# rubengooj/pl-svo

Measured on AMD Instinct MI355X. Metric: sparse-align+pose-opt frames/sec, 640×480, ~200 pts+80 lines; 1/2/4/8 GPU, higher is better.
Workload: dtype f64

## Files before the change

include/plsvo_hip.h:

```cpp
#ifndef PLSVO_HIP_H_
#define PLSVO_HIP_H_

#include <stddef.h>
#include <stdint.h>

#ifdef __cplusplus
extern "C" {
#endif

#define PLSVO_MAX_LEVELS 8
#define PLSVO_PATCH_SIZE 4
#define PLSVO_PATCH_AREA 16

#define PLSVO_OK              0
#define PLSVO_E_INVALID      -1
#define PLSVO_E_NODEVICE     -2
#define PLSVO_E_HIP          -3
#define PLSVO_E_CAPACITY     -4
#define PLSVO_E_STATE        -5
#define PLSVO_E_RCCL         -6

typedef struct plsvo_ctx plsvo_ctx;

typedef struct plsvo_pinhole {
  double fx, fy, cx, cy;
  int32_t width, height;
} plsvo_pinhole;


int plsvo_hip_create(int device_id, void* stream, plsvo_ctx** out);
int plsvo_hip_create_on_stream(int device_id, void* stream, plsvo_ctx** out);
void plsvo_hip_destroy(plsvo_ctx* ctx);
#define PLSVO_OPT_LDLT_FLAVOUR 1
#define PLSVO_OPT_ALIGN_THREADS 2
#define PLSVO_OPT_POSEOPT_THREADS 3
#define PLSVO_OPT_ALIGN_REORDER 4
#define PLSVO_OPT_POSEOPT_REORDER 5
int plsvo_hip_set_option(plsvo_ctx* ctx, int option, int value);
const char* plsvo_hip_last_error(const plsvo_ctx* ctx);
void* plsvo_hip_stream(plsvo_ctx* ctx);
int plsvo_hip_synchronize(plsvo_ctx* ctx);


int plsvo_hip_config_pyramids(plsvo_ctx* ctx, int n_slots, int width, int height, int n_levels);

int plsvo_hip_upload_pyramid(plsvo_ctx* ctx, int slot, int n_levels,
                             const uint8_t* const* level_ptr, const int* width, const int* height,
                             const int* stride_bytes);

int plsvo_hip_build_pyramid(plsvo_ctx* ctx, int slot, const uint8_t* level0, int stride_bytes,
                            int rounding);
int plsvo_hip_build_pyramids_dev(plsvo_ctx* ctx, int first_slot, int n, const void* d_level0,
                                 int stride_bytes, size_t image_pitch_bytes, int rounding);
int plsvo_hip_copy_slots(plsvo_ctx* ctx, int dst_first, int src_first, int n);
int plsvo_hip_download_level(plsvo_ctx* ctx, int slot, int level, uint8_t* out);


typedef struct plsvo_pinhole_radtan {
  plsvo_pinhole cam;
  double d[5];
} plsvo_pinhole_radtan;

#define PLSVO_MAX_RECTIFY_MAPS 8

int plsvo_rectify_map(const plsvo_pinhole_radtan* cam, int16_t* xy, uint16_t* frac);
int plsvo_hip_config_rectify(plsvo_ctx* ctx, const plsvo_pinhole_radtan* cam, int flip_vertical, int* map_id);
int plsvo_hip_rectify_build_pyramid(plsvo_ctx* ctx, int map_id, int slot, const uint8_t* raw, int stride_bytes, int rounding);
int plsvo_hip_rectify_build_pyramids_dev(plsvo_ctx* ctx, int map_id, int first_slot, int n, const void* d_raw,
                                         int stride_bytes, size_t image_pitch_bytes, int rounding);


typedef struct plsvo_corner { int32_t x, y; float score; int32_t level; } plsvo_corner;

typedef struct plsvo_detect_params {
  int32_t cell_size;
  int32_t n_levels;
  int32_t fast_threshold;
  int32_t reserved0;
  double  detection_threshold;
} plsvo_detect_params;

int plsvo_detect_grid(int width, int height, int cell_size, int* cols, int* rows);
int plsvo_detect_cell(int cols, int cell_size, double px_x, double px_y);
int plsvo_hip_detect_fast(plsvo_ctx* ctx, int first_slot, int n, const plsvo_detect_params* params, const uint8_t* occupancy,
                          plsvo_corner* corners, int32_t* counts);
int plsvo_hip_detect_fast_dev(plsvo_ctx* ctx, int first_slot, int n, const plsvo_detect_params* params, const uint8_t* d_occupancy,
                              plsvo_corner* d_corners, int32_t* d_counts);
int plsvo_hip_detect_stages(plsvo_ctx* ctx, int slot, int level, int fast_threshold, uint8_t* score, uint8_t* survives);


typedef struct plsvo_align_in {
  int32_t ref_slot, cur_slot;
  plsvo_pinhole cam;
  int32_t max_level, min_level;
  int32_t n_iter;
  int32_t reserved0;
  double eps;
  double T_cur_from_ref[7];
  int32_t n_pts, n_seg;
  const double* pt_px;
  const double* pt_xyz_ref;
  const double* seg_spx;
  const double* seg_epx;
  const double* seg_len;
  const double* seg_p_ref;
  const double* seg_q_ref;
  const uint8_t* seg_alive_in;
} plsvo_align_in;

typedef struct plsvo_align_out {
  double T_cur_from_ref[7];
  uint64_t n_meas;
  uint64_t n_tracked;
  double H[36];
  double chi2;
  uint8_t* seg_alive_out;
  int32_t iters_per_level[PLSVO_MAX_LEVELS];
  int32_t status;
  int32_t reserved0;
} plsvo_align_out;

typedef struct plsvo_align_iterlog {
  int32_t level, iter;
  int32_t accepted;
  int32_t stop;
  uint64_t n_meas;
  double new_chi2;
  double H[36], Jres[6], x[6];
  double T_after[7];
} plsvo_align_iterlog;

int plsvo_sparse_align(plsvo_ctx* ctx, const plsvo_align_in* in, plsvo_align_out* out);
int plsvo_sparse_align_batch(plsvo_ctx* ctx, int n, const plsvo_align_in* in, plsvo_align_out* out);

int plsvo_align_stage(plsvo_ctx* ctx, int n, const plsvo_align_in* in);
int plsvo_align_run(plsvo_ctx* ctx);
int plsvo_align_fetch(plsvo_ctx* ctx, int n, plsvo_align_out* out);

int plsvo_align_slot_layout(const plsvo_align_in* in, int level, int32_t* seg_code, int32_t* n_slots, int32_t* long_lines,
                            long long* n_patches);

int plsvo_align_set_trace(plsvo_ctx* ctx, int max_records_per_job);
int plsvo_align_fetch_trace(plsvo_ctx* ctx, int job, plsvo_align_iterlog* out, int max_records,
                            int* n_records);

const double* plsvo_align_poses_dev(plsvo_ctx* ctx);
int plsvo_align_copy_poses(plsvo_ctx* ctx, double* d_dst);

int plsvo_align_work(plsvo_ctx* ctx, uint64_t* patch_levels, uint64_t* patch_iters);
int plsvo_align_launch_order(plsvo_ctx* ctx, int n, int32_t* order);
int plsvo_align_work_points(plsvo_ctx* ctx, uint64_t* point_patch_iters);

int plsvo_align_chi2_ties(plsvo_ctx* ctx, uint64_t* iterations, uint64_t* ties, uint64_t* near_ties_without_terms);


typedef struct plsvo_poseopt_in {
  double T_f_w[7];
  double fx;
  double reproj_thresh;
  int32_t n_iter;
  int32_t n_iter_ref;
  int32_t n_pts, n_seg;
  const double* pt_f;
  const double* pt_pos;
  const int32_t* pt_level;
  const double* seg_line;
  const double* seg_spos;
  const double* seg_epos;
  const int32_t* seg_level;
} plsvo_poseopt_in;

typedef struct plsvo_poseopt_out {
  double T_f_w[7];
  double cov[36];
  double estimated_scale, error_init, error_final;
  uint64_t num_obs_pt, num_obs_ls;
  uint8_t* pt_keep;
  uint8_t* seg_keep;
  int32_t iters;
  int32_t iters_ref;
  int32_t status;
  int32_t reserved0;
} plsvo_poseopt_out;

typedef struct plsvo_poseopt_iterlog {
  int32_t phase;
  int32_t iter;
  int32_t accepted;
  int32_t reserved0;
  double new_chi2;
  double A[36], b[6], dT[6];
  double T_after[7];
} plsvo_poseopt_iterlog;

int plsvo_pose_optimize(plsvo_ctx* ctx, const plsvo_poseopt_in* in, plsvo_poseopt_out* out);
int plsvo_pose_optimize_batch(plsvo_ctx* ctx, int n, const plsvo_poseopt_in* in, plsvo_poseopt_out* out);
int plsvo_poseopt_stage(plsvo_ctx* ctx, int n, const plsvo_poseopt_in* in);
int plsvo_poseopt_run(plsvo_ctx* ctx);
int plsvo_poseopt_fetch(plsvo_ctx* ctx, int n, plsvo_poseopt_out* out);
int plsvo_poseopt_set_trace(plsvo_ctx* ctx, int max_records_per_job);
int plsvo_poseopt_fetch_trace(plsvo_ctx* ctx, int job, plsvo_poseopt_iterlog* out, int max_records,
                              int* n_records);
const double* plsvo_poseopt_poses_dev(plsvo_ctx* ctx);
int plsvo_poseopt_copy_poses(plsvo_ctx* ctx, double* d_dst);
int plsvo_poseopt_work(plsvo_ctx* ctx, uint64_t* pt_iters, uint64_t* seg_iters);


typedef struct plsvo_structopt_in {
  int32_t n_frames;
  int32_t n_iter_pts;
  int32_t n_iter_segs;
  int32_t n_pts, n_seg;
  int32_t reserved0;
  const double* frame_T;
  const double* pt_pos;
  const int32_t* pt_obs_off;
  const int32_t* pt_obs_frame;
  const double* pt_obs_f;
  const double* seg_spos;
  const double* seg_epos;
  const int32_t* seg_obs_off;
  const int32_t* seg_obs_frame;
  const double* seg_obs_sf;
  const double* seg_obs_ef;
} plsvo_structopt_in;

typedef struct plsvo_structopt_out {
  double* pt_pos;
  double* seg_spos;
  double* seg_epos;
  int32_t* pt_iters;
  int32_t* seg_iters;
} plsvo_structopt_out;

int plsvo_structure_optimize(plsvo_ctx* ctx, const plsvo_structopt_in* in, plsvo_structopt_out* out);


#define PLSVO_FTR_CORNER  0
#define PLSVO_FTR_EDGELET 1

typedef struct plsvo_match_in {
  plsvo_pinhole cam;
  int32_t n_pyr_levels;
  int32_t align_max_iter;
  int32_t n_frames;
  int32_t n;
  const double* frame_T;
  const int32_t* frame_slot;
  const int32_t* cur_frame;
  const int32_t* ref_frame;
  const double* ref_px;
  const double* ref_f;
  const int32_t* ref_level;
  const uint8_t* ref_type;
  const double* ref_grad;
  const double* pos;
  const double* px_cur;
} plsvo_match_in;

typedef struct plsvo_match_out {
  double* px_cur;
  uint8_t* found;
  int32_t* search_level;
  int32_t* n_iter;
} plsvo_match_out;

int plsvo_match_direct(plsvo_ctx* ctx, const plsvo_match_in* in, plsvo_match_out* out);

typedef struct plsvo_reproject_in {
  plsvo_pinhole cam;
  int32_t n_frames;
  int32_t n;
  int32_t cell_size;
  int32_t grid_n_cols;
  int32_t boundary;
  int32_t reserved0;
  const double* frame_T;
  const int32_t* frame;
  const double* pos;
} plsvo_reproject_in;

typedef struct plsvo_reproject_out {
  double* px;
  int32_t* cell;
} plsvo_reproject_out;

int plsvo_reproject(plsvo_ctx* ctx, const plsvo_reproject_in* in, plsvo_reproject_out* out);


typedef struct plsvo_chain_in {
  plsvo_align_in align;
  double T_prev_w[7];
  double T_kf_w[7];
  int32_t kf_slot;
  int32_t n_cand_pt, n_cand_seg;
  int32_t reserved0;
  const double* pos;
  const double* ref_px;
  const double* ref_f;
  const int32_t* ref_level;
  const uint8_t* ref_type;
  const double* ref_grad;
  const uint8_t* active;
// ... 134 lines not shown
```

pl-svo_amd/capi.py:

```python
import ctypes as C
import os
import sys

import numpy as np

from . import abi

_HERE = os.path.dirname(os.path.abspath(__file__))
LIB_PATH = os.environ.get("PLSVO_HIP_LIB", os.path.join(_HERE, "libplsvo_hip.so"))

SYMBOLS = [
    "plsvo_hip_create", "plsvo_hip_create_on_stream", "plsvo_hip_set_option", "plsvo_align_slot_layout", "plsvo_hip_destroy", "plsvo_hip_last_error", "plsvo_hip_stream", "plsvo_hip_synchronize",
    "plsvo_hip_config_pyramids", "plsvo_hip_upload_pyramid", "plsvo_hip_build_pyramid", "plsvo_hip_build_pyramids_dev",
    "plsvo_hip_download_level", "plsvo_hip_copy_slots",
    "plsvo_rectify_map", "plsvo_hip_config_rectify", "plsvo_hip_rectify_build_pyramid", "plsvo_hip_rectify_build_pyramids_dev",
    "plsvo_detect_grid", "plsvo_detect_cell", "plsvo_hip_detect_fast", "plsvo_hip_detect_fast_dev", "plsvo_hip_detect_stages",
    "plsvo_sparse_align", "plsvo_sparse_align_batch", "plsvo_align_stage", "plsvo_align_run", "plsvo_align_fetch",
    "plsvo_align_set_trace", "plsvo_align_fetch_trace", "plsvo_align_poses_dev", "plsvo_align_copy_poses", "plsvo_align_work", "plsvo_align_work_points", "plsvo_align_chi2_ties", "plsvo_align_launch_order",
    "plsvo_pose_optimize", "plsvo_pose_optimize_batch", "plsvo_poseopt_stage", "plsvo_poseopt_run", "plsvo_poseopt_fetch",
    "plsvo_poseopt_set_trace", "plsvo_poseopt_fetch_trace", "plsvo_poseopt_poses_dev", "plsvo_poseopt_copy_poses", "plsvo_poseopt_work",
    "plsvo_structure_optimize", "plsvo_match_direct", "plsvo_reproject", "plsvo_trajectory_record", "plsvo_update_seeds",
    "plsvo_chain_stage", "plsvo_chain_run", "plsvo_chain_fetch", "plsvo_frame_step_batch", "plsvo_chain_poses_dev",
    "plsvo_pack_pose_records", "plsvo_fetch_pose_records", "plsvo_gather_poses",
    "plsvo_hip_set_profiling", "plsvo_hip_kernel_time", "plsvo_hip_reset_profiling",
    "plsvo_hip_version", "plsvo_hip_build_flags", "plsvo_hip_device_info",
]


def rectify_map(cam):
    w, h = cam.cam.width, cam.cam.height
    xy = np.zeros((max(h, 0), max(w, 0), 2), dtype=np.int16)
    fr = np.zeros((max(h, 0), max(w, 0)), dtype=np.uint16)
    rc = lib().plsvo_rectify_map(C.byref(cam), xy.ctypes.data_as(C.POINTER(C.c_int16)), fr.ctypes.data_as(C.POINTER(C.c_uint16)))
    if rc != 0:
        raise PlsvoError(rc, "rectify_map: bad camera (non-finite or zero focal length, size outside 1..2046)")
    return xy, fr


def detect_grid(width, height, cell_size):
    cols, rows = C.c_int(0), C.c_int(0)
    rc = lib().plsvo_detect_grid(int(width), int(height), int(cell_size), C.byref(cols), C.byref(rows))
    if rc != 0:
        raise PlsvoError(rc, "detect_grid: width, height and cell_size must be >= 1")
    return cols.value, rows.value


def detect_cell(cols, cell_size, px_x, px_y):
    k = lib().plsvo_detect_cell(int(cols), int(cell_size), float(px_x), float(px_y))
    if k < 0:
        raise PlsvoError(k, "detect_cell: cols and cell_size must be >= 1, the pixel finite and not negative")
    return k


class PlsvoError(RuntimeError):
    def __init__(self, code, msg):
        super().__init__(f"plsvo_hip error {code}: {msg}")
        self.code = code


_lib = None


def lib():
    global _lib
    if _lib is not None:
        return _lib
    if not os.path.exists(LIB_PATH):
        raise ImportError(f"{LIB_PATH} not found: build it with `make -C pl-svo_amd/csrc` "
                          f"(or __graft_entry__.build()); plsvo_hip has no CPU fallback")
    L = C.CDLL(LIB_PATH)
    if hasattr(L, "plsvo_emu_build"):
        sys.stderr.write(f"pl-svo_amd: {LIB_PATH} is a HOST EMULATION build of the kernels (test infrastructure), not the gfx950 library\n")
    ctxp = C.c_void_p
    vp = C.c_void_p
    sig = {
        "plsvo_hip_create": (C.c_int, [C.c_int, vp, C.POINTER(ctxp)]),
        "plsvo_hip_create_on_stream": (C.c_int, [C.c_int, vp, C.POINTER(ctxp)]),
        "plsvo_hip_destroy": (None, [ctxp]),
        "plsvo_hip_set_option": (C.c_int, [ctxp, C.c_int, C.c_int]),
        "plsvo_hip_last_error": (C.c_char_p, [ctxp]),
        "plsvo_hip_stream": (vp, [ctxp]),
        "plsvo_hip_synchronize": (C.c_int, [ctxp]),
        "plsvo_hip_config_pyramids": (C.c_int, [ctxp, C.c_int, C.c_int, C.c_int, C.c_int]),
        "plsvo_hip_upload_pyramid": (C.c_int, [ctxp, C.c_int, C.c_int, C.POINTER(abi.c_u8_p), abi.c_i32_p, abi.c_i32_p, abi.c_i32_p]),
        "plsvo_hip_build_pyramid": (C.c_int, [ctxp, C.c_int, abi.c_u8_p, C.c_int, C.c_int]),
        "plsvo_hip_build_pyramids_dev": (C.c_int, [ctxp, C.c_int, C.c_int, vp, C.c_int, C.c_size_t, C.c_int]),
        "plsvo_hip_download_level": (C.c_int, [ctxp, C.c_int, C.c_int, abi.c_u8_p]),
        "plsvo_hip_copy_slots": (C.c_int, [ctxp, C.c_int, C.c_int, C.c_int]),
        "plsvo_rectify_map": (C.c_int, [C.POINTER(abi.PinholeRadtan), C.POINTER(C.c_int16), C.POINTER(C.c_uint16)]),
        "plsvo_hip_config_rectify": (C.c_int, [ctxp, C.POINTER(abi.PinholeRadtan), C.c_int, C.POINTER(C.c_int)]),
        "plsvo_hip_rectify_build_pyramid": (C.c_int, [ctxp, C.c_int, C.c_int, abi.c_u8_p, C.c_int, C.c_int]),
        "plsvo_hip_rectify_build_pyramids_dev": (C.c_int, [ctxp, C.c_int, C.c_int, C.c_int, vp, C.c_int, C.c_size_t, C.c_int]),
        "plsvo_detect_grid": (C.c_int, [C.c_int, C.c_int, C.c_int, C.POINTER(C.c_int), C.POINTER(C.c_int)]),
        "plsvo_detect_cell": (C.c_int, [C.c_int, C.c_int, C.c_double, C.c_double]),
        "plsvo_hip_detect_fast": (C.c_int, [ctxp, C.c_int, C.c_int, C.POINTER(abi.DetectParams), abi.c_u8_p, C.POINTER(abi.Corner), abi.c_i32_p]),
        "plsvo_hip_detect_fast_dev": (C.c_int, [ctxp, C.c_int, C.c_int, C.POINTER(abi.DetectParams), vp, vp, vp]),
        "plsvo_hip_detect_stages": (C.c_int, [ctxp, C.c_int, C.c_int, C.c_int, abi.c_u8_p, abi.c_u8_p]),
        "plsvo_sparse_align": (C.c_int, [ctxp, C.POINTER(abi.AlignIn), C.POINTER(abi.AlignOut)]),
        "plsvo_sparse_align_batch": (C.c_int, [ctxp, C.c_int, C.POINTER(abi.AlignIn), C.POINTER(abi.AlignOut)]),
        "plsvo_align_stage": (C.c_int, [ctxp, C.c_int, C.POINTER(abi.AlignIn)]),
        "plsvo_align_run": (C.c_int, [ctxp]),
        "plsvo_align_fetch": (C.c_int, [ctxp, C.c_int, C.POINTER(abi.AlignOut)]),
        "plsvo_align_set_trace": (C.c_int, [ctxp, C.c_int]),
        "plsvo_align_fetch_trace": (C.c_int, [ctxp, C.c_int, C.POINTER(abi.AlignIterLog), C.c_int, C.POINTER(C.c_int)]),
        "plsvo_align_poses_dev": (vp, [ctxp]),
        "plsvo_align_copy_poses": (C.c_int, [ctxp, vp]),
        "plsvo_poseopt_copy_poses": (C.c_int, [ctxp, vp]),
        "plsvo_align_work": (C.c_int, [ctxp, C.POINTER(C.c_uint64), C.POINTER(C.c_uint64)]),
        "plsvo_align_chi2_ties": (C.c_int, [ctxp, C.POINTER(C.c_uint64), C.POINTER(C.c_uint64), C.POINTER(C.c_uint64)]),
        "plsvo_align_work_points": (C.c_int, [ctxp, C.POINTER(C.c_uint64)]),
        "plsvo_align_launch_order": (C.c_int, [ctxp, C.c_int, C.POINTER(C.c_int32)]),
        "plsvo_pose_optimize": (C.c_int, [ctxp, C.POINTER(abi.PoseOptIn), C.POINTER(abi.PoseOptOut)]),
        "plsvo_pose_optimize_batch": (C.c_int, [ctxp, C.c_int, C.POINTER(abi.PoseOptIn), C.POINTER(abi.PoseOptOut)]),
        "plsvo_poseopt_stage": (C.c_int, [ctxp, C.c_int, C.POINTER(abi.PoseOptIn)]),
        "plsvo_poseopt_run": (C.c_int, [ctxp]),
        "plsvo_poseopt_fetch": (C.c_int, [ctxp, C.c_int, C.POINTER(abi.PoseOptOut)]),
        "plsvo_poseopt_set_trace": (C.c_int, [ctxp, C.c_int]),
        "plsvo_poseopt_fetch_trace": (C.c_int, [ctxp, C.c_int, C.POINTER(abi.PoseOptIterLog), C.c_int, C.POINTER(C.c_int)]),
        "plsvo_poseopt_poses_dev": (vp, [ctxp]),
        "plsvo_poseopt_work": (C.c_int, [ctxp, C.POINTER(C.c_uint64), C.POINTER(C.c_uint64)]),
        "plsvo_structure_optimize": (C.c_int, [ctxp, C.POINTER(abi.StructOptIn), C.POINTER(abi.StructOptOut)]),
        "plsvo_match_direct": (C.c_int, [ctxp, C.POINTER(abi.MatchIn), C.POINTER(abi.MatchOut)]),
        "plsvo_reproject": (C.c_int, [ctxp, C.POINTER(abi.ReprojectIn), C.POINTER(abi.ReprojectOut)]),
        "plsvo_update_seeds": (C.c_int, [ctxp, C.POINTER(abi.SeedsIn), C.POINTER(abi.SeedsOut)]),
        "plsvo_trajectory_record": (C.c_int, [abi.c_double_p, abi.c_double_p, abi.c_double_p]),
        "plsvo_chain_stage": (C.c_int, [ctxp, C.c_int, C.POINTER(abi.ChainIn), C.POINTER(abi.ChainParams)]),
        "plsvo_chain_run": (C.c_int, [ctxp]),
        "plsvo_chain_fetch": (C.c_int, [ctxp, C.c_int, C.POINTER(abi.ChainOut)]),
        "plsvo_frame_step_batch": (C.c_int, [ctxp, C.c_int, C.POINTER(abi.ChainIn), C.POINTER(abi.ChainParams), C.POINTER(abi.ChainOut)]),
        "plsvo_chain_poses_dev": (vp, [ctxp]),
        "plsvo_align_slot_layout": (C.c_int, [C.POINTER(abi.AlignIn), C.c_int, C.POINTER(C.c_int32), C.POINTER(C.c_int32), C.POINTER(C.c_int32),
                                              C.POINTER(C.c_longlong)]),
        "plsvo_pack_pose_records": (C.c_int, [ctxp, vp, C.POINTER(C.c_int)]),
        "plsvo_fetch_pose_records": (C.c_int, [ctxp, C.c_int, C.POINTER(abi.PoseRecord)]),
        "plsvo_gather_poses": (C.c_int, [ctxp, vp, vp, C.c_int, vp]),
        "plsvo_hip_set_profiling": (C.c_int, [ctxp, C.c_int]),
        "plsvo_hip_kernel_time": (C.c_int, [ctxp, C.c_int, C.POINTER(C.c_double), C.POINTER(C.c_int64)]),
        "plsvo_hip_reset_profiling": (C.c_int, [ctxp]),
        "plsvo_hip_version": (C.c_char_p, []),
        "plsvo_hip_build_flags": (C.c_char_p, []),
        "plsvo_hip_device_info": (C.c_int, [ctxp, C.c_char_p, C.c_int, C.POINTER(C.c_int), C.POINTER(C.c_size_t)]),
    }
    for name, (res, args) in sig.items():
        if "PLSVO_HIP_LIB" in os.environ and not hasattr(L, name):
            continue
        f = getattr(L, name)
        f.restype = res
        f.argtypes = args
    _lib = L
    return L


class Context:

    def __init__(self, device=0, stream=None):
        self.L = lib()
        h = C.c_void_p()
        if stream is None:
            rc = self.L.plsvo_hip_create(int(device), None, C.byref(h))
        else:
            rc = self.L.plsvo_hip_create_on_stream(int(device), C.c_void_p(int(stream)), C.byref(h))
        if rc != 0:
            raise PlsvoError(rc, (self.L.plsvo_hip_last_error(None) or b"").decode())
        self.h = h
        self._keep = None

    def set_ldlt_flavour(self, flavour):
        self._chk(self.L.plsvo_hip_set_option(self.h, 1, int(flavour)))

    def set_launch_shapes(self, align_threads=None, poseopt_threads=None):
        if align_threads is not None:
            self._chk(self.L.plsvo_hip_set_option(self.h, 2, int(align_threads)))
        if poseopt_threads is not None:
            self._chk(self.L.plsvo_hip_set_option(self.h, 3, int(poseopt_threads)))

    def set_launch_order_refresh(self, align=None, poseopt=None):
        if align is not None:
            self._chk(self.L.plsvo_hip_set_option(self.h, 4, 1 if align else 0))
        if poseopt is not None:
            self._chk(self.L.plsvo_hip_set_option(self.h, 5, 1 if poseopt else 0))

    def close(self):
        if getattr(self, "h", None):
            self.L.plsvo_hip_destroy(self.h)
            self.h = None

    def __del__(self):
        try:
            self.close()
        except Exception:
            pass

    def _chk(self, rc):
        if rc != 0:
            raise PlsvoError(rc, (self.L.plsvo_hip_last_error(self.h) or b"").decode())

    def device_info(self):
        name = C.create_string_buffer(256)
        cu = C.c_int(0)
        mem = C.c_size_t(0)
        self._chk(self.L.plsvo_hip_device_info(self.h, name, 256, C.byref(cu), C.byref(mem)))
        return name.value.decode(), cu.value, mem.value

    def stream(self):
        return self.L.plsvo_hip_stream(self.h)

    def synchronize(self):
        self._chk(self.L.plsvo_hip_synchronize(self.h))

    def set_profiling(self, on):
        self._chk(self.L.plsvo_hip_set_profiling(self.h, 1 if on else 0))

    def reset_profiling(self):
        self._chk(self.L.plsvo_hip_reset_profiling(self.h))

    def kernel_time(self, k):
        ms = C.c_double(0)
        n = C.c_int64(0)
        self._chk(self.L.plsvo_hip_kernel_time(self.h, k, C.byref(ms), C.byref(n)))
        return ms.value, n.value

    def config_pyramids(self, n_slots, width, height, n_levels):
        self._chk(self.L.plsvo_hip_config_pyramids(self.h, n_slots, width, height, n_levels))
        self.n_levels = n_levels
        self.width, self.height = width, height

    def upload_pyramid(self, slot, levels):
        keep = [np.ascontiguousarray(l, dtype=np.uint8) for l in levels]
        n = len(keep)
        ptrs = (abi.c_u8_p * n)(*[l.ctypes.data_as(abi.c_u8_p) for l in keep])
        w = (C.c_int32 * n)(*[l.shape[1] for l in keep])
        h = (C.c_int32 * n)(*[l.shape[0] for l in keep])
        s = (C.c_int32 * n)(*[l.strides[0] for l in keep])
        self._chk(self.L.plsvo_hip_upload_pyramid(self.h, slot, n, ptrs, w, h, s))

    def build_pyramid(self, slot, img0, rounding=0):
        img0 = np.ascontiguousarray(img0, dtype=np.uint8)
        self._chk(self.L.plsvo_hip_build_pyramid(self.h, slot, img0.ctypes.data_as(abi.c_u8_p), img0.strides[0], rounding))

    def build_pyramids_dev(self, first_slot, n, d_ptr, stride_bytes, image_pitch_bytes, rounding=0):
        self._chk(self.L.plsvo_hip_build_pyramids_dev(self.h, first_slot, n, C.c_void_p(d_ptr), stride_bytes,
                                                      image_pitch_bytes, rounding))

    def download_level(self, slot, level):
        w, h = self.width >> level, self.height >> level
        out = np.empty((h, w), dtype=np.uint8)
        self._chk(self.L.plsvo_hip_download_level(self.h, slot, level, out.ctypes.data_as(abi.c_u8_p)))
        return out

    def copy_slots(self, dst_first, src_first, n):
        self._chk(self.L.plsvo_hip_copy_slots(self.h, int(dst_first), int(src_first), int(n)))

    def download_pyramid(self, slot):
        return [self.download_level(slot, l) for l in range(self.n_levels)]

    def config_rectify(self, cam, flip_vertical=False):
        mid = C.c_int(-1)
        self._chk(self.L.plsvo_hip_config_rectify(self.h, C.byref(cam), 1 if flip_vertical else 0, C.byref(mid)))
        return mid.value

    def rectify_build_pyramid(self, map_id, slot, raw, rounding=0):
        raw = np.asarray(raw, dtype=np.uint8)
        if raw.ndim != 2 or raw.strides[1] != 1:
            raw = np.ascontiguousarray(raw)
        self._chk(self.L.plsvo_hip_rectify_build_pyramid(self.h, int(map_id), int(slot), raw.ctypes.data_as(abi.c_u8_p), raw.strides[0],
                                                         int(rounding)))

    def rectify_build_pyramids_dev(self, map_id, first_slot, n, d_ptr, stride_bytes, image_pitch_bytes, rounding=0):
        self._chk(self.L.plsvo_hip_rectify_build_pyramids_dev(self.h, int(map_id), int(first_slot), int(n), C.c_void_p(d_ptr),
                                                              int(stride_bytes), int(image_pitch_bytes), int(rounding)))

    def detect_fast(self, first_slot, n, cell_size=25, n_levels=3, fast_threshold=20, detection_threshold=20.0, occupancy=None):
        cols, rows = detect_grid(self.width, self.height, cell_size)
        cells = cols * rows
        pr = abi.detect_params(cell_size, n_levels, fast_threshold, detection_threshold)
        occ = None
        if occupancy is not None:
            occ = np.ascontiguousarray(np.asarray(occupancy).reshape(int(n), cells) != 0, dtype=np.uint8)
        out = np.zeros((max(int(n), 1), cells), dtype=abi.CORNER_DTYPE)
        counts = np.zeros(max(int(n), 1), dtype=np.int32)
        self._chk(self.L.plsvo_hip_detect_fast(self.h, int(first_slot), int(n), C.byref(pr), None if occ is None else occ.ctypes.data_as(abi.c_u8_p),
                                               out.ctypes.data_as(C.POINTER(abi.Corner)), counts.ctypes.data_as(abi.c_i32_p)))
        return [out[i, :counts[i]].copy() for i in range(int(n))]

    def detect_fast_dev(self, first_slot, n, d_corners, d_counts, cell_size=25, n_levels=3, fast_threshold=20, detection_threshold=20.0,
                        d_occupancy=None):
        pr = abi.detect_params(cell_size, n_levels, fast_threshold, detection_threshold)
        self._chk(self.L.plsvo_hip_detect_fast_dev(self.h, int(first_slot), int(n), C.byref(pr), C.c_void_p(d_occupancy), C.c_void_p(d_corners),
                                                   C.c_void_p(d_counts)))

    def detect_stages(self, slot, level, fast_threshold=20):
        w, h = self.width >> level, self.height >> level
        score = np.zeros((max(h, 0), max(w, 0)), dtype=np.uint8)
        surv = np.zeros_like(score)
        self._chk(self.L.plsvo_hip_detect_stages(self.h, int(slot), int(level), int(fast_threshold), score.ctypes.data_as(abi.c_u8_p),
                                                 surv.ctypes.data_as(abi.c_u8_p)))
        return score, surv

    def align_set_trace(self, max_records):
        self._chk(self.L.plsvo_align_set_trace(self.h, max_records))
        self._align_trace = max_records

    def align_stage(self, jobs):
        arr = (abi.AlignIn * len(jobs))(*[j.c for j in jobs])
        self._chk(self.L.plsvo_align_stage(self.h, len(jobs), arr))
        self._align_jobs = jobs

    def align_run(self):
        self._chk(self.L.plsvo_align_run(self.h))

    def align_fetch(self):
        jobs = self._align_jobs
        n = len(jobs)
        outs = (abi.AlignOut * n)()
        alive = [np.ones(max(j.n_seg, 1), dtype=np.uint8) for j in jobs]
        for o, a in zip(outs, alive):
            o.seg_alive_out = a.ctypes.data_as(abi.c_u8_p)
        self._chk(self.L.plsvo_align_fetch(self.h, n, outs))
        return [abi.AlignResult(o, a[:j.n_seg].copy()) for o, a, j in zip(outs, alive, jobs)]

    def align_fetch_trace(self, job):
        cap = getattr(self, "_align_trace", 0)
        log = (abi.AlignIterLog * max(cap, 1))()
        n = C.c_int(0)
        self._chk(self.L.plsvo_align_fetch_trace(self.h, job, log, cap, C.byref(n)))
        return abi.align_log_to_dicts(log, n.value)

    def sparse_align_batch(self, jobs):
        self.align_stage(jobs)
        self.align_run()
        return self.align_fetch()

    def sparse_align(self, job):
        return self.sparse_align_batch([job])[0]

    def align_work(self):
        a = C.c_uint64(0)
        b = C.c_uint64(0)
        self._chk(self.L.plsvo_align_work(self.h, C.byref(a), C.byref(b)))
        return a.value, b.value

    def align_work_points(self):
        a = C.c_uint64(0)
        self._chk(self.L.plsvo_align_work_points(self.h, C.byref(a)))
        return a.value

    def align_launch_order(self, n):
        out = np.zeros(n, dtype=np.int32)
        self._chk(self.L.plsvo_align_launch_order(self.h, n, out.ctypes.data_as(C.POINTER(C.c_int32))))
        return out

    def align_chi2_ties(self):
        a = C.c_uint64(0)
        b = C.c_uint64(0)
        c = C.c_uint64(0)
        self._chk(self.L.plsvo_align_chi2_ties(self.h, C.byref(a), C.byref(b), C.byref(c)))
        return a.value, b.value, c.value

    def align_poses_dev(self):
        return self.L.plsvo_align_poses_dev(self.h)

    def align_copy_poses(self, d_dst):
        self._chk(self.L.plsvo_align_copy_poses(self.h, C.c_void_p(d_dst)))

    def poseopt_copy_poses(self, d_dst):
        self._chk(self.L.plsvo_poseopt_copy_poses(self.h, C.c_void_p(d_dst)))

    def poseopt_set_trace(self, max_records):
        self._chk(self.L.plsvo_poseopt_set_trace(self.h, max_records))
        self._pose_trace = max_records

    def poseopt_stage(self, jobs):
        arr = (abi.PoseOptIn * len(jobs))(*[j.c for j in jobs])
        self._chk(self.L.plsvo_poseopt_stage(self.h, len(jobs), arr))
        self._pose_jobs = jobs

    def poseopt_run(self):
        self._chk(self.L.plsvo_poseopt_run(self.h))

    def poseopt_fetch(self):
        jobs = self._pose_jobs
        n = len(jobs)
        outs = (abi.PoseOptOut * n)()
        pk = [np.ones(max(j.n_pts, 1), dtype=np.uint8) for j in jobs]
        sk = [np.ones(max(j.n_seg, 1), dtype=np.uint8) for j in jobs]
        for o, a, b in zip(outs, pk, sk):
            o.pt_keep = a.ctypes.data_as(abi.c_u8_p)
            o.seg_keep = b.ctypes.data_as(abi.c_u8_p)
        self._chk(self.L.plsvo_poseopt_fetch(self.h, n, outs))
        return [abi.PoseOptResult(o, a[:j.n_pts].copy(), b[:j.n_seg].copy()) for o, a, b, j in zip(outs, pk, sk, jobs)]

    def poseopt_fetch_trace(self, job):
        cap = getattr(self, "_pose_trace", 0)
        log = (abi.PoseOptIterLog * max(cap, 1))()
        n = C.c_int(0)
        self._chk(self.L.plsvo_poseopt_fetch_trace(self.h, job, log, cap, C.byref(n)))
        return abi.poseopt_log_to_dicts(log, n.value)

    def pose_optimize_batch(self, jobs):
        self.poseopt_stage(jobs)
        self.poseopt_run()
        return self.poseopt_fetch()

    def pose_optimize(self, job):
        return self.pose_optimize_batch([job])[0]

    def poseopt_work(self):
        a = C.c_uint64(0)
        b = C.c_uint64(0)
        self._chk(self.L.plsvo_poseopt_work(self.h, C.byref(a), C.byref(b)))
        return a.value, b.value

    def poseopt_poses_dev(self):
        return self.L.plsvo_poseopt_poses_dev(self.h)

    def chain_stage(self, jobs, cam, n_pyr_levels=3, align_max_iter=10, cell_size=30, cell_rule=False, max_fts=120, cell_order=None,
                    reproj_thresh=2.0, poseopt_n_iter=10, seg_cell_size=0, max_fts_segs=100, seg_cell_order=None):
        n = len(jobs)
        arr = (abi.ChainIn * n)(*[j.c for j in jobs])
        pr = abi.ChainParams()
        pr.cam = cam if isinstance(cam, abi.Pinhole) else abi.Pinhole(*cam)
        pr.n_pyr_levels, pr.align_max_iter, pr.cell_size, pr.cell_rule = int(n_pyr_levels), int(align_max_iter), int(cell_size), int(bool(cell_rule))
        pr.max_fts, pr.poseopt_n_iter, pr.reproj_thresh = int(max_fts), int(poseopt_n_iter), float(reproj_thresh)
        self._chain_order = None if cell_order is None else np.ascontiguousarray(cell_order, dtype=np.int32)
        pr.cell_order = C.cast(None, abi.c_i32_p) if self._chain_order is None else self._chain_order.ctypes.data_as(abi.c_i32_p)
        pr.seg_cell_size, pr.max_fts_segs = int(seg_cell_size), int(max_fts_segs)
        self._chain_seg_order = None if seg_cell_order is None else np.ascontiguousarray(seg_cell_order, dtype=np.int32)
        pr.seg_cell_order = C.cast(None, abi.c_i32_p) if self._chain_seg_order is None else self._chain_seg_order.ctypes.data_as(abi.c_i32_p)
        self._chain_seg_mult = 2 if (cell_rule and seg_cell_size > 0) else 1
        self._chk(self.L.plsvo_chain_stage(self.h, n, arr, C.byref(pr)))
        self._chain_jobs = list(jobs)
        self._align_jobs = [j.align_job for j in jobs]

    def chain_run(self):
        self._chk(self.L.plsvo_chain_run(self.h))

    def chain_fetch(self):
        jobs = self._chain_jobs
        n = len(jobs)
        outs = (abi.ChainOut * n)()
        bufs = []
        for o, j in zip(outs, jobs):
            b = dict(alive=np.ones(max(j.align_job.n_seg, 1), np.uint8), pk=np.zeros(max(j.n_cand_pt, 1), np.uint8), sk=np.zeros(max(self._chain_seg_mult * j.n_cand_seg, 1), np.uint8),
                     found=np.zeros(max(j.n_cand, 1), np.uint8), px=np.zeros((max(j.n_cand, 1), 2)), level=np.zeros(max(j.n_cand, 1), np.int32),
                     sel_pt=np.zeros(max(j.n_cand_pt, 1), np.int32), sel_seg=np.zeros(max(self._chain_seg_mult * j.n_cand_seg, 1), np.int32))
            o.align.seg_alive_out = b["alive"].ctypes.data_as(abi.c_u8_p)
            o.pose.pt_keep = b["pk"].ctypes.data_as(abi.c_u8_p)
            o.pose.seg_keep = b["sk"].ctypes.data_as(abi.c_u8_p)
            o.found = b["found"].ctypes.data_as(abi.c_u8_p)
            o.px = b["px"].ctypes.data_as(abi.c_double_p)
            o.search_level = b["level"].ctypes.data_as(abi.c_i32_p)
            o.sel_pt = b["sel_pt"].ctypes.data_as(abi.c_i32_p)
            o.sel_seg = b["sel_seg"].ctypes.data_as(abi.c_i32_p)
            bufs.append(b)
        self._chk(self.L.plsvo_chain_fetch(self.h, n, outs))
        return [abi.ChainResult(o, j, b["alive"][:j.align_job.n_seg].copy(), b["pk"], b["sk"], b["found"], b["px"], b["level"], b["sel_pt"], b["sel_seg"])
                for o, j, b in zip(outs, jobs, bufs)]

    def frame_step_batch(self, jobs, cam, **params):
        self.chain_stage(jobs, cam, **params)
        self.chain_run()
        return self.chain_fetch()

    def chain_poses_dev(self):
        return self.L.plsvo_chain_poses_dev(self.h)

    def structure_optimize(self, job):
        out, bufs = job.make_out()
        self._chk(self.L.plsvo_structure_optimize(self.h, C.byref(job.c), C.byref(out)))
        return job.trim(bufs)

    def match_direct(self, job):
        out, bufs = job.make_out()
        self._chk(self.L.plsvo_match_direct(self.h, C.byref(job.c), C.byref(out)))
        return job.trim(bufs)

    def reproject(self, job):
        out, bufs = job.make_out()
        self._chk(self.L.plsvo_reproject(self.h, C.byref(job.c), C.byref(out)))
        return job.trim(bufs)

    def update_seeds(self, job):
        out, bufs = job.make_out()
        self._chk(self.L.plsvo_update_seeds(self.h, C.byref(job.c), C.byref(out)))
        return job.trim(bufs)

    def pack_pose_records(self, d_dst):
        n = C.c_int(0)
        self._chk(self.L.plsvo_pack_pose_records(self.h, C.c_void_p(d_dst), C.byref(n)))
        return int(n.value)

    def fetch_pose_records(self, n):
        out = np.zeros(n, dtype=abi.POSE_RECORD_DTYPE)
        self._chk(self.L.plsvo_fetch_pose_records(self.h, n, out.ctypes.data_as(C.POINTER(abi.PoseRecord))))
        return out

    def gather_poses(self, rccl_comm, d_local, n_local, d_all):
        self._chk(self.L.plsvo_gather_poses(self.h, C.c_void_p(rccl_comm), C.c_void_p(d_local), n_local, C.c_void_p(d_all)))


def trajectory_record(T_f_w, cov):
    T = np.ascontiguousarray(T_f_w, dtype=np.float64)
    Cv = np.ascontiguousarray(cov, dtype=np.float64).reshape(36)
# ... 18 lines not shown
```

pl-svo_amd/csrc/align_kernels.hip:

```cpp
#include <hip/hip_runtime.h>

#include <type_traits>

#include "plsvo_dev.hpp"
#include "plsvo_math.hpp"
#include "plsvo_wave.hpp"
#include "align_refpatch.hpp"
#include "robust_weight.hpp"

namespace plsvo_hip {

__device__ __forceinline__ float robust_weight(float a) { return robust_weight_f64(a); }

template <bool TILED>
__device__ __forceinline__ uint2 load_row8_raw(const uint8_t* img, int pitch, int x, int y) {
  uint32_t d0, d1, d2, sh;
  if constexpr (TILED) {
    const int a = x & ~3;
    sh = (uint32_t)(x & 3);
    const int row = tiled_row_offset(pitch, y);
    d0 = *reinterpret_cast<const uint32_t*>(img + (row + tiled_col_offset(a)));
    d1 = *reinterpret_cast<const uint32_t*>(img + (row + tiled_col_offset(a + 4)));
    d2 = *reinterpret_cast<const uint32_t*>(img + (row + tiled_col_offset(a + 8)));
  } else {
    const int off = y * pitch + x, a = off & ~3;
    sh = (uint32_t)(off & 3);
    d0 = *reinterpret_cast<const uint32_t*>(img + a);
    d1 = *reinterpret_cast<const uint32_t*>(img + a + 4);
    d2 = *reinterpret_cast<const uint32_t*>(img + a + 8);
  }
  return make_uint2(__builtin_amdgcn_alignbyte(d1, d0, sh), __builtin_amdgcn_alignbyte(d2, d1, sh));
}
#ifdef PLSVO_TIMING
#define TICK_RAW(slot) do { if (tid == 0) { const unsigned long long t__ = __builtin_amdgcn_s_memtime(); s_time[slot] += t__ - s_tlast; s_tlast = t__; } } while (0)
#if PLSVO_TIMING == 3
#define TICK(slot) do { if ((slot) == 0) TICK_RAW(5); } while (0)
#define TICKS(slot) TICK_RAW(slot)
#else
#define TICK(slot) TICK_RAW(slot)
#define TICKS(slot) do { } while (0)
#endif
#else
#define TICK(slot) do { } while (0)
#define TICKS(slot) do { } while (0)
#endif

#define SLOT_HOLE ((int)0x80000000)

template <int T>
__device__ __forceinline__ void block_sync() {
  if constexpr (T == 64) wave_lds_fence(); else __syncthreads();
}

constexpr int kTiledMaxThreads = 64;
constexpr float kChiBand = 1.5f;

__host__ __device__ inline size_t align_chi_window_offset(int threads, int cap, int scap) {
  size_t o = sizeof(double) * 32 * (threads / 16) + sizeof(double) * 64 + sizeof(int) * 32;
  o += (size_t)cap * (sizeof(int2) + sizeof(float)) + (size_t)scap * sizeof(int) + ((size_t)2 * scap + 2) * sizeof(float);
  return (o + 15) & ~(size_t)15;
}
__host__ __device__ inline size_t align_quad_offset(int threads, int cap, int scap, int chi_lds_pts) {
  const size_t window = 1024 * sizeof(float), planes = (size_t)2 * chi_lds_pts * 16 * sizeof(float);
  return (align_chi_window_offset(threads, cap, scap) + (planes > window ? planes : window) + 15) & ~(size_t)15;
}
__host__ __device__ inline size_t align_lds_used(int threads, int cap, int scap, int chi_lds_pts) {
  const size_t quad = threads >= kQuadMinThreads ? (size_t)cap * 32 : 0;
  return align_quad_offset(threads, cap, scap, chi_lds_pts) + quad + 16;
}
#define PLSVO_LDS __attribute__((address_space(3)))
#define PLSVO_GLOBAL __attribute__((address_space(1)))
typedef float plsvo_v4f __attribute__((ext_vector_type(4)));
__device__ __forceinline__ float chain4(float s, plsvo_v4f v) {
  s = __fadd_rn(s, v.x); s = __fadd_rn(s, v.y); s = __fadd_rn(s, v.z); return __fadd_rn(s, v.w);
}
__device__ __forceinline__ double half_scan_incl(double v) {
  v += dpp_bcast_f64<DPP_ROW_SHR(1), 0xF>(v);
  v += dpp_bcast_f64<DPP_ROW_SHR(2), 0xF>(v);
  v += dpp_bcast_f64<DPP_ROW_SHR(4), 0xF>(v);
  v += dpp_bcast_f64<DPP_ROW_SHR(8), 0xF>(v);
  v += dpp_bcast_f64<DPP_ROW_BCAST15, 0xA>(v);
  return v;
}
__device__ __forceinline__ double half_readlane(double v, int la, int lb) {
  const double a = readlane_f64(v, la), b = readlane_f64(v, 32 + lb);
  return (threadIdx.x & 32) ? b : a;
}
__device__ __forceinline__ float half_readlane(float v, int la, int lb) {
  const float a = __int_as_float(__builtin_amdgcn_readlane(__float_as_int(v), la)), b = __int_as_float(__builtin_amdgcn_readlane(__float_as_int(v), 32 + lb));
  return (threadIdx.x & 32) ? b : a;
}

__device__ __forceinline__ void exact_round32(const float (&t)[16], float& s, double& base) {
  const int lane = threadIdx.x & 63, l32 = lane & 31;
  double d = 0.0;
#pragma unroll
  for (int i = 0; i < 16; ++i) d += (double)t[i];
  const double inc = half_scan_incl(d);
  const double excl = inc - d;
  const double tot = half_readlane(inc, 31, 31);
  const double lo = base + excl, hi = lo + d;
  int e = (int)((__double2hiint(lo) >> 20) & 0x7ff) - 1023;
  bool safe = lo > 0.0 && hi < 1.7976931348623157e308 && e - 24 >= -126 && e <= 126;
  e = min(max(e, -100), 126);
  const double two_e = __hiloint2double((e + 1023) << 20, 0), two_e1 = __hiloint2double((e + 1024) << 20, 0);
  safe = safe && lo * (1.0 - 0.0009765625) >= two_e && hi * (1.0 + 0.0009765625) < two_e1;
  const int e_top = (int)((__double2hiint(base + tot) >> 20) & 0x7ff) - 1023;
  safe = safe && e >= e_top - 26;
  const float C = __int_as_float((e + 127) << 23), half_q = __int_as_float((e - 24 + 127) << 23);
  double delta = 0.0;
  bool half_hit = false;
#pragma unroll
  for (int i = 0; i < 16; ++i) {
    const float r = __fsub_rn(__fadd_rn(C, t[i]), C);
    half_hit = half_hit || fabsf(__fsub_rn(t[i], r)) == half_q;
    delta += (double)r;
  }
  safe = safe && !half_hit;
  if (!safe) delta = 0.0;
  const double dinc = half_scan_incl(delta);
  const double dex = dinc - delta;
  const double dlast = half_readlane(dinc, 31, 31);
  int start = 0;
  double s0 = (double)s, off = 0.0;
  bool done = false;
  for (;;) {
    const double sl = s0 + (dex - off);
    bool ok = safe && sl > 0.0 && two_e <= sl && sl + delta < two_e1;
    if (l32 < start || done) ok = true;
    const unsigned long long m = __ballot(!ok);
    const unsigned ba = (unsigned)m, bb = (unsigned)(m >> 32);
    const int fa = ba ? __builtin_ctz(ba) : 32, fb = bb ? __builtin_ctz(bb) : 32;
    const int f = (lane & 32) ? fb : fa;
    const double dex_f = half_readlane(dex, fa & 31, fb & 31), delta_f = half_readlane(delta, fa & 31, fb & 31);
    float sf = (float)(s0 + (dex_f - off));
    if (!done && l32 == f) {
#pragma unroll
      for (int i = 0; i < 16; ++i) sf = __fadd_rn(sf, t[i]);
    }
    sf = half_readlane(sf, fa & 31, fb & 31);
    if (!done) {
      if (f == 32) { s0 = s0 + (dlast - off); done = true; }
      else { s0 = (double)sf; start = f + 1; off = dex_f + delta_f; if (start == 32) done = true; }
    }
    if (!__any(!done)) break;
  }
  s = (float)s0;
  base += tot;
}

__device__ __noinline__ void exact_chi2_pair(const PLSVO_GLOBAL float* bufA, const PLSVO_GLOBAL float* bufB, int n_pts, int n_seg, int iter,
                                             const PLSVO_LDS int* s_dead, PLSVO_LDS float* s_win, const PLSVO_LDS float* s_lterm, int scap,
                                             PLSVO_LDS float* s_out) {
  const int lane = threadIdx.x & 63;
  const plsvo_v4f z4 = { 0.f, 0.f, 0.f, 0.f };
  auto load_win = [&](int r, plsvo_v4f* v) {
    const size_t f0 = (size_t)r * 512;
#pragma unroll
    for (int h = 0; h < 2; ++h) {
      const int q = lane + 64 * h;
      const bool ok = 32 * r + (q >> 2) < n_pts;
      v[h] = ok ? reinterpret_cast<const PLSVO_GLOBAL plsvo_v4f*>(bufA + f0)[q] : z4;
      v[2 + h] = ok ? reinterpret_cast<const PLSVO_GLOBAL plsvo_v4f*>(bufB + f0)[q] : z4;
    }
  };
  float sum = 0.0f;
  double base = 0.0;
  const int n_rounds = (n_pts + 31) >> 5;
  plsvo_v4f nxt[4] = { z4, z4, z4, z4 };
  if (n_rounds > 0) load_win(0, nxt);
  for (int r = 0; r < n_rounds; ++r) {
    const plsvo_v4f c0 = nxt[0], c1 = nxt[1], c2 = nxt[2], c3 = nxt[3];
    if (r + 1 < n_rounds) load_win(r + 1, nxt);
    wave_lds_fence();
    PLSVO_LDS plsvo_v4f* const w4 = reinterpret_cast<PLSVO_LDS plsvo_v4f*>(s_win);
    w4[lane] = c0; w4[lane + 64] = c1; w4[128 + lane] = c2; w4[128 + lane + 64] = c3;
    wave_lds_fence();
    {
      const PLSVO_LDS plsvo_v4f* w = w4 + 128 * (lane >> 5) + 4 * (lane & 31);
      const plsvo_v4f q0 = w[0], q1 = w[1], q2 = w[2], q3 = w[3];
      const float t[16] = { q0.x, q0.y, q0.z, q0.w, q1.x, q1.y, q1.z, q1.w, q2.x, q2.y, q2.z, q2.w, q3.x, q3.y, q3.z, q3.w };
      exact_round32(t, sum, base);
    }
  }
  if ((lane & 31) == 0) {
    const int h = lane >> 5;
    float seg_sum = 0.0f;
    for (int sg = 0; sg < n_seg; ++sg) {
      const int dead = s_dead[sg];
      const float t = s_lterm[((iter - h) & 1) * scap + sg];
      seg_sum = __fadd_rn(seg_sum, (dead == 0 || dead > iter - h + 1) ? t : 0.0f);
    }
    s_out[h] = __fadd_rn(sum, seg_sum);
  }
  wave_lds_fence();
}

__device__ __noinline__ void exact_chi2_pair_lds(const PLSVO_LDS float* planeA, const PLSVO_LDS float* planeB, int n_pts, int n_seg, int iter,
                                                 const PLSVO_LDS int* s_dead, const PLSVO_LDS float* s_lterm, int scap, PLSVO_LDS float* s_out) {
  const int lane = threadIdx.x & 63, h = lane >> 5, l32 = lane & 31;
  const PLSVO_LDS plsvo_v4f* plane = reinterpret_cast<const PLSVO_LDS plsvo_v4f*>(h ? planeB : planeA);
  float sum = 0.0f;
  double base = 0.0;
  for (int p0 = 0; p0 < n_pts; p0 += 32) {
    const int p = p0 + l32;
    const plsvo_v4f z4 = { 0.f, 0.f, 0.f, 0.f };
    plsvo_v4f q0 = z4, q1 = z4, q2 = z4, q3 = z4;
    if (p < n_pts) { q0 = plane[4 * p]; q1 = plane[4 * p + 1]; q2 = plane[4 * p + 2]; q3 = plane[4 * p + 3]; }
    const float t[16] = { q0.x, q0.y, q0.z, q0.w, q1.x, q1.y, q1.z, q1.w, q2.x, q2.y, q2.z, q2.w, q3.x, q3.y, q3.z, q3.w };
    exact_round32(t, sum, base);
  }
  if (l32 == 0) {
    float seg_sum = 0.0f;
    for (int sg = 0; sg < n_seg; ++sg) {
      const int dead = s_dead[sg];
      const float t = s_lterm[((iter - h) & 1) * scap + sg];
      seg_sum = __fadd_rn(seg_sum, (dead == 0 || dead > iter - h + 1) ? t : 0.0f);
    }
    s_out[h] = __fadd_rn(sum, seg_sum);
  }
  wave_lds_fence();
}

constexpr int kMinWavesPerSimd = 2;
template <int T>
__global__ __launch_bounds__(T, kMinWavesPerSimd) void align_fused_kernel(AlignBatchDev b, int cap, int scap, int level_hi, int level_lo, int do_init) {
  const bool pair = T >= kQuadMinThreads && b.pair != 0;
  const int rank = pair ? (int)((blockIdx.x >> 3) & 1u) : 0;
  const int wg_index = pair ? (int)((blockIdx.x >> 4) * 8u + (blockIdx.x & 7u)) : (int)blockIdx.x;
  if (wg_index >= b.n_jobs) return;
  const bool lead = rank == 0;
  const bool own_pts = !pair || rank == 0, own_segs = !pair || rank == 1;
  const int job_id = b.order ? b.order[wg_index] : wg_index;
  const AlignJobDev job = b.jobs[job_id];
  AlignStateDev* st = b.state + job_id;
  const int tid = threadIdx.x, lane = tid & 63, wave = tid >> 6;
  const int grp = tid >> 2, row = tid & 3;
  constexpr int ROWS = T / 16;

  extern __shared__ __align__(16) unsigned char smem[];
  double* s_red = reinterpret_cast<double*>(smem);
  double* s_pose = s_red + ROWS * 32;
  double* s_tot = s_pose + 32;
  int* s_ctl = reinterpret_cast<int*>(s_tot + 32);
  int2* s_meta = reinterpret_cast<int2*>(s_ctl + 32);
  float* s_abs = reinterpret_cast<float*>(s_meta + cap);
  int* s_dead = reinterpret_cast<int*>(s_abs + cap);
  float* s_lterm = reinterpret_cast<float*>(s_dead + scap);
  float* s_win = reinterpret_cast<float*>(smem + align_chi_window_offset(T, cap, scap));
  constexpr bool kQuad = T >= kQuadMinThreads;
  double* const s_xyz = reinterpret_cast<double*>(kQuad ? smem + align_quad_offset(T, cap, scap, b.chi_lds_pts) : smem);
  float* const s_uvr = reinterpret_cast<float*>(s_xyz + 3 * (kQuad ? cap : 0));

#ifdef PLSVO_TIMING
  __shared__ unsigned long long s_time[8];
  __shared__ unsigned long long s_tlast;
  if (tid == 0) { for (int k = 0; k < 8; ++k) s_time[k] = 0; s_tlast = __builtin_amdgcn_s_memtime(); }
#endif
  const int lv_first = min(job.max_level, level_hi), lv_last = max(job.min_level, level_lo);
  const bool nothing = job.skip || lv_first < lv_last;
  if (do_init && own_segs) {
    for (int s = tid; s < job.n_seg; s += T)
      b.seg_alive[job.seg_off + s] = b.seg_alive_in ? (b.seg_alive_in[job.seg_off + s] != 0) : 1;
  }
  if (tid == 0) {
    double T_in[7], chi_in = 1e10; int stop_in = 0;
    if (do_init) {
#pragma unroll
      for (int k = 0; k < 7; ++k) T_in[k] = b.T0[7 * job_id + k];
      if (lead) {
#pragma unroll
      for (int k = 0; k < 7; ++k) st->T[k] = T_in[k];
      st->chi2 = 1e10; st->n_meas = 0; st->stop = 0; st->log_count = 0; st->error = 0;
      for (int k = 0; k < 36; ++k) st->H[k] = 0.0;
      for (int k = 0; k < PLSVO_MAX_LEVELS; ++k) st->iters[k] = 0;
      st->patch_levels = 0; st->patch_iters = 0; st->patch_iters_pt = 0; st->chi2_ties = 0; st->chi2_unarmed = 0;
      for (int k = 0; k < 8; ++k) st->phase_ticks[k] = 0;
      if (nothing && b.poses) for (int k = 0; k < 7; ++k) b.poses[7 * job_id + k] = T_in[k];
      if (nothing && b.work_key) b.work_key[job_id] = 0;
      }
    } else if (!nothing) {
#pragma unroll
      for (int k = 0; k < 7; ++k) T_in[k] = st->T[k];
      chi_in = st->chi2; stop_in = st->stop;
    }
    if (!nothing) {
#pragma unroll
      for (int k = 0; k < 7; ++k) { s_pose[12 + k] = T_in[k]; s_pose[19 + k] = T_in[k]; }
      s_pose[26] = chi_in; s_pose[28] = 0.0; s_pose[29] = 0.0; s_pose[31] = 0.0;
      for (int k = 0; k < 32; ++k) s_tot[k] = 0.0;
      s_ctl[1] = stop_in; s_ctl[3] = 0; s_ctl[6] = 0; s_ctl[9] = 0;
      s_ctl[10] = 0;
    }
  }
  if (nothing) return;
  block_sync<T>();
  if (b.chi_lds_pts > 0) {
    const int tail0 = job.n_pts * 16, tail1 = ((job.n_pts + 3) & ~3) * 16;
    for (int k = tail0 + tid; k < tail1; k += T) { s_win[k] = 0.0f; s_win[b.chi_lds_pts * 16 + k] = 0.0f; }
  }
  const size_t pbase = (size_t)job.patch_off;
  const int nfeat = job.n_pts + job.n_seg;
  double* const pxyz = b.patch_xyz + 3 * pbase;
  const int line0 = pair ? ((job.n_pts + 63) & ~63) : 0;
  unsigned long long* const xb = pair ? b.xbuf + (size_t)job_id * 256 : nullptr;
  unsigned xseq = b.xseq0;
  bool x_lost = false;

  for (int level = lv_first; level >= lv_last; --level) {
    const int W = job.width >> level, Hh = job.height >> level;
    constexpr bool kTiled = T <= kTiledMaxThreads;
    const unsigned int lvl_off = kTiled ? pyr_tiled_level_offset(job.width, job.height, level) : pyr_level_offset(job.width, job.height, level);
    const uint8_t* const pyr_base = kTiled ? b.pyr.tbase : b.pyr.base;
    const unsigned long long pyr_slot = kTiled ? b.pyr.tslot_bytes : b.pyr.slot_bytes;
    const uint8_t* ref_img = pyr_base + (size_t)job.ref_slot * pyr_slot + lvl_off;
    const uint8_t* cur_img = pyr_base + (size_t)job.cur_slot * pyr_slot + lvl_off;
    const int pitch = kTiled ? (W + 15) >> 4 : W;
    int n_slots = 0; bool long_lines = false;
#pragma unroll
    for (int l = 0; l < PLSVO_MAX_LEVELS; ++l) if (l == level) { n_slots = job.n_slots[l]; long_lines = ((job.long_mask >> l) & 1) != 0; }
    if (n_slots > cap || n_slots > job.patch_cap) {
      if (tid == 0 && lead) { st->error = 1; if (b.work_key) b.work_key[job_id] = 0; }
      return;
    }
    const int slot_lo = (pair && rank == 1) ? min(line0, n_slots) : 0, slot_hi = (pair && rank == 0) ? min(line0, n_slots) : n_slots;
    block_sync<T>();
    TICKS(0);

    if (tid == 0) { s_ctl[0] = 0; s_ctl[2] = 0; s_ctl[5] = 0; s_ctl[7] = 0; s_ctl[8] = 0; s_pose[27] = 0.0; }
    for (int p = tid; p < n_slots; p += T) s_meta[p] = make_int2(SLOT_HOLE, 0);
    block_sync<T>();
    TICKS(1);

    const double scale = 1.0 / (double)(1 << level);
    int my_patches = 0;
    for (int f = (own_pts ? 0 : job.n_pts) + tid; f < (own_segs ? nfeat : job.n_pts); f += T) {
      if (f < job.n_pts) {
        const int i = job.pt_off + f;
        if constexpr (kQuad) {
          s_xyz[3 * f] = b.pt_xyz[3 * i]; s_xyz[3 * f + 1] = b.pt_xyz[3 * i + 1]; s_xyz[3 * f + 2] = b.pt_xyz[3 * i + 2];
        }
        const float u = (float)(b.pt_px[2 * i] * scale), v = (float)(b.pt_px[2 * i + 1] * scale);
        if constexpr (kQuad) { s_uvr[2 * f] = u; s_uvr[2 * f + 1] = v; }
        if (u >= 3.0f && v >= 3.0f && u < (float)(W - 3) && v < (float)(Hh - 3)) {
          s_meta[f] = make_int2(f, f | (1 << 20));
          if constexpr (kQuad) {
          } else {
          b.patch_uvref[2 * (pbase + f)] = u;
          b.patch_uvref[2 * (pbase + f) + 1] = v;
          pxyz[3 * f] = b.pt_xyz[3 * i];
          pxyz[3 * f + 1] = b.pt_xyz[3 * i + 1];
          pxyz[3 * f + 2] = b.pt_xyz[3 * i + 2];
          }
          ++my_patches;
        }
      } else {
        const int sl = f - job.n_pts, s = job.seg_off + sl;
        s_dead[sl] = 0; s_lterm[sl] = 0.0f; s_lterm[scap + sl] = 0.0f;
        double g_s[2] = { 0.0, 0.0 }, g_e[2] = { 0.0, 0.0 }, g_p[3] = { 0.0, 0.0, 0.0 }, g_q[3] = { 0.0, 0.0, 0.0 };
        if constexpr (kQuad) {
          g_s[0] = b.seg_spx[2 * s]; g_s[1] = b.seg_spx[2 * s + 1]; g_e[0] = b.seg_epx[2 * s]; g_e[1] = b.seg_epx[2 * s + 1];
#pragma unroll
          for (int c = 0; c < 3; ++c) { g_p[c] = b.seg_p[3 * s + c]; g_q[c] = b.seg_q[3 * s + c]; }
        }
        const int code = b.seg_slot[(size_t)(level - b.slot_level0) * b.slot_stride + s];
        if (code >= 0 && b.seg_alive[s]) {
          const int p0 = code & 0xfffff, N = code >> 20;
          const double sx = kQuad ? g_s[0] : b.seg_spx[2 * s], sy = kQuad ? g_s[1] : b.seg_spx[2 * s + 1];
          double inc2x = ((kQuad ? g_e[0] : b.seg_epx[2 * s]) - sx) * scale / (double)(N - 1);
          double inc2y = ((kQuad ? g_e[1] : b.seg_epx[2 * s + 1]) - sy) * scale / (double)(N - 1);
          double px = sx * scale, py = sy * scale;
          double xr[3], inc3[3];
          for (int c = 0; c < 3; ++c) {
            const double pr = kQuad ? g_p[c] : b.seg_p[3 * s + c];
            inc3[c] = ((kQuad ? g_q[c] : b.seg_q[3 * s + c]) - pr) / (double)(N - 1);
            xr[c] = pr;
          }
          for (int n = 0; n < N; ++n) {
            const int p = p0 + n;
            s_meta[p] = make_int2(-1 - sl, p0 | (N << 20));
            if constexpr (kQuad) {
              s_uvr[2 * p] = (float)px; s_uvr[2 * p + 1] = (float)py;
              s_xyz[3 * p] = xr[0]; s_xyz[3 * p + 1] = xr[1]; s_xyz[3 * p + 2] = xr[2];
            } else {
            b.patch_uvref[2 * (pbase + p)] = (float)px;
            b.patch_uvref[2 * (pbase + p) + 1] = (float)py;
            pxyz[3 * p] = xr[0];
            pxyz[3 * p + 1] = xr[1];
            pxyz[3 * p + 2] = xr[2];
            }
            px += inc2x; py += inc2y;
            xr[0] += inc3[0]; xr[1] += inc3[1]; xr[2] += inc3[2];
          }
          my_patches += N;
        }
      }
    }
    if constexpr (kQuad) {
      const int wave_patches = wave_sum_i32_to_lane63(my_patches);
      if (lane == 63 && wave_patches) atomicAdd(&s_ctl[5], wave_patches);
    } else {
    if (my_patches) atomicAdd(&s_ctl[5], my_patches);
    }
    TICKS(2);
    block_sync<T>();
    TICKS(3);

    if constexpr (kQuad) {
      for (int pb = slot_lo + wave * 64; pb < slot_hi; pb += T) {
        const int p = pb + lane;
        if (p < slot_hi && s_meta[p].x != SLOT_HOLE) {
          const float u = s_uvr[2 * p], v = s_uvr[2 * p + 1];
          const PatchW pw = patch_weights(u, v);
          uint32_t d[7][3]; int shf[7];
#pragma unroll
          for (int k = 0; k < 7; ++k) {
            const int off = (pw.vi - 3 + k) * pitch + (pw.ui - 3), a = off & ~3;
            shf[k] = off & 3;
            d[k][0] = *reinterpret_cast<const uint32_t*>(ref_img + a);
            d[k][1] = *reinterpret_cast<const uint32_t*>(ref_img + a + 4);
            d[k][2] = *reinterpret_cast<const uint32_t*>(ref_img + a + 8);
          }
          uint32_t lo[7], hi[7];
#pragma unroll
          for (int k = 0; k < 7; ++k) {
            lo[k] = __builtin_amdgcn_alignbyte(d[k][1], d[k][0], (uint32_t)shf[k]);
            hi[k] = __builtin_amdgcn_alignbyte(d[k][2], d[k][1], (uint32_t)shf[k]);
          }
          uint4 q[4];
          q[0] = make_uint4(lo[0], hi[0], lo[1], hi[1]); q[1] = make_uint4(lo[2], hi[2], lo[3], hi[3]); q[2] = make_uint4(lo[4], hi[4], lo[5], hi[5]);
          q[3] = make_uint4(lo[6], hi[6], __float_as_uint(u - floorf(u)), __float_as_uint(v - floorf(v)));
          float4* const dst = reinterpret_cast<float4*>(b.cache_ref) + (pbase + p) * 12;
          RecordRows rec;
          rec.start(q);
          float4 vr, vx, vy;
          rec.template row<0>(vr, vx, vy); dst[0] = vr; dst[1] = vx; dst[2] = vy;
          rec.template row<1>(vr, vx, vy); dst[3] = vr; dst[4] = vx; dst[5] = vy;
          rec.template row<2>(vr, vx, vy); dst[6] = vr; dst[7] = vx; dst[8] = vy;
          rec.template row<3>(vr, vx, vy); dst[9] = vr; dst[10] = vx; dst[11] = vy;
        }
      }
    } else {
    for (int pb = 0; pb < n_slots; pb += T / 4) {
      const int p = pb + grp;
      if (p < n_slots && s_meta[p].x != SLOT_HOLE) {
        const float u = b.patch_uvref[2 * (pbase + p)], v = b.patch_uvref[2 * (pbase + p) + 1];
        const PatchW pw = patch_weights(u, v);
        unsigned char* const rec = reinterpret_cast<unsigned char*>(b.cache_ref) + ((pbase + p) << 6);
        const int cx = pw.ui - 3, ry = pw.vi - 3 + row;
        *reinterpret_cast<uint2*>(rec + 8 * row) = load_row8_raw<kTiled>(ref_img, pitch, cx, ry);
        if (row < 3) *reinterpret_cast<uint2*>(rec + 8 * (row + 4)) = load_row8_raw<kTiled>(ref_img, pitch, cx, ry + 4);
        else *reinterpret_cast<float2*>(rec + 56) = make_float2(u - floorf(u), v - floorf(v));
      }
    }
    }
    TICKS(4);
    if (tid == 0) { SE3d m = se3_load(s_pose + 12); quat_to_matrix(m.q, s_pose); s_pose[9] = m.t[0]; s_pose[10] = m.t[1]; s_pose[11] = m.t[2]; }
    block_sync<T>();
    TICK(0);

    const double fs = fabs(job.fx) / (double)(1 << level);
    const float colmax = (float)(W - 2), rowmax = (float)(Hh - 2);

    for (int iter = 0; iter < job.n_iter; ++iter) {
     int redo_mask = 0;
     for (int stage = 0; stage < 3; ++stage) {
      if (stage > 0 && !(redo_mask & stage)) continue;
      const bool terms_only = stage > 0;
      const int last_stage = (redo_mask & 2) ? 2 : ((redo_mask & 1) ? 1 : 0);
      const double* const pose_rt = (stage == 2) ? s_red : s_pose;

      const bool store_chi = terms_only || b.chi_lds_pts > 0 || s_ctl[7] != 0;
      const int chi_par = (stage == 2) ? ((iter & 1) ^ 1) : (iter & 1);
      float* const chi_it = b.chi_terms + (size_t)chi_par * b.chi_plane + (size_t)job.pt_off * 16;

      double acc[32];
#pragma unroll
      for (int k = 0; k < 32; ++k) acc[k] = 0.0;

      for (int pass = (long_lines && !terms_only) ? 0 : 1; pass < 2; ++pass) {
        const bool write_abs = (!long_lines || pass == 0) && !terms_only;
        const bool accumulate = pass == 1 && !terms_only;
        const int n_rounds_slots = terms_only ? min(n_slots, job.n_pts) : (kQuad ? slot_hi : n_slots);

        if constexpr (kQuad) {
        struct PixSums { double A, B, C, D, E, Chi; float Abs; };
        auto unpack5 = [](uint32_t lo, uint32_t hi, int sh, float* o) {
          const uint32_t w0 = __builtin_amdgcn_alignbyte(hi, lo, (uint32_t)sh);
          o[0] = (float)(w0 & 0xffu); o[1] = (float)((w0 >> 8) & 0xffu); o[2] = (float)((w0 >> 16) & 0xffu); o[3] = (float)(w0 >> 24);
          o[4] = (float)((hi >> (8 * sh)) & 0xffu);
        };
        auto row4 = [&](auto WEIGHTED, bool is_point, const PatchW& pw, const float* top, const float* bot, const float4& r4, const float4& x4,
                        const float4& y4, float4& tv4, PixSums& ps) {
          constexpr bool weighted = decltype(WEIGHTED)::value;
          const float* pr = reinterpret_cast<const float*>(&r4);
          const float* pxp = reinterpret_cast<const float*>(&x4);
          const float* pyp = reinterpret_cast<const float*>(&y4);
          float* tv = reinterpret_cast<float*>(&tv4);
#pragma unroll
          for (int x = 0; x < 4; ++x) {
            const float c = bilinear(pw.wTL, pw.wTR, pw.wBL, pw.wBR, top[x], top[x + 1], bot[x], bot[x + 1]);
            const float res = __fsub_rn(c, pr[x]);
            const float ares = fabsf(res);
            const double rd = (double)res, dx = (double)pxp[x], dy = (double)pyp[x];
            if (weighted) {
              const float w = is_point ? robust_weight(ares) : 1.0f;
              const double wd = (double)w;
              const double wdx = wd * dx, wdy = wd * dy;
              ps.A += wdx * dx; ps.B += wdx * dy; ps.C += wdy * dy;
              ps.D += wdx * rd; ps.E += wdy * rd;
              const float term = __fmul_rn(__fmul_rn(res, res), w);
              ps.Chi += (double)term;
              tv[x] = is_point ? term : ares;
            } else {
              ps.A += dx * dx; ps.B += dx * dy; ps.C += dy * dy;
              ps.D += dx * rd; ps.E += dy * rd;
              tv[x] = ares;
            }
            ps.Abs += ares;
          }
        };
        auto chi_store = [&](int p_, int r, const float4& t) {
          const plsvo_v4f t4 = { t.x, t.y, t.z, t.w };
          if (b.chi_lds_pts > 0) ((PLSVO_LDS plsvo_v4f*)(s_win + (iter & 1) * b.chi_lds_pts * 16 + p_ * 16))[r] = t4;
          else ((PLSVO_GLOBAL plsvo_v4f*)(chi_it + (unsigned)(p_ * 16)))[r] = t4;
        };
        auto slot_finish = [&](int p, const int2& meta, bool is_line, bool cand, bool live, double X, double Y, double Z, double z_inv, const PixSums& ps) {
          double wh = 0.0, wj = 0.0;
          if (__any(is_line && cand)) {
            if (write_abs) {
              if (is_line && cand) s_abs[p] = live ? ps.Abs : -1.0f;
              wave_lds_fence();
            }
            if (accumulate && is_line && cand) {
              const int first = meta.y & 0xfffff, N = meta.y >> 20;
              bool good = true; float sum = 0.0f;
              for (int n = 0; n < N; ++n) { const float a = s_abs[first + n]; good = good && (a >= 0.0f); sum += a; }
              const float res_ = (float)((double)sum / (double)N);
              if (good && (double)res_ < 200.0) {
                const float w = (float)(1.0 / (1.0 + (double)res_));
                wh = (double)w / (double)res_;
                wj = (double)w;
                if (p == first) {
                  const float term = __fmul_rn(__fmul_rn(res_, res_), w);
                  acc[27] += (double)term; acc[28] += 1.0;
                  s_lterm[(iter & 1) * scap + (-1 - meta.x)] = term;
                }
              } else if (p == first) {
                s_dead[-1 - meta.x] = iter + 1;
                b.seg_alive[job.seg_off + (-1 - meta.x)] = 0;
              }
            }
          }
          if (accumulate) {
            if (!is_line && live) {
              wh = 1.0; wj = 1.0;
              acc[27] += ps.Chi; acc[28] += (double)PLSVO_PATCH_AREA;
            }
            if (live) { acc[29] += 1.0; if (!is_line && store_chi && b.chi_lds_pts == 0) acc[30] += 1.0; }
            if (wh != 0.0 || wj != 0.0) {
              double J[12];
              {
                const double z_inv_2 = z_inv * z_inv;
                J[0] = -z_inv; J[1] = 0.0; J[2] = X * z_inv_2; J[3] = Y * J[2]; J[4] = -(1.0 + X * J[2]); J[5] = Y * z_inv;
                J[6] = 0.0; J[7] = -z_inv; J[8] = Y * z_inv_2; J[9] = 1.0 + Y * J[8]; J[10] = -J[3]; J[11] = -X * z_inv;
              }
              const double hs = wh * fs * fs, js = wj * fs;
              const double hA = ps.A * hs, hB = ps.B * hs, hC = ps.C * hs, jD = ps.D * js, jE = ps.E * js;
              double v0[6], v1[6];
#pragma unroll
              for (int k = 0; k < 6; ++k) { v0[k] = hA * J[k] + hB * J[6 + k]; v1[k] = hB * J[k] + hC * J[6 + k]; }
              int k = 0;
#pragma unroll
              for (int i = 0; i < 6; ++i)
#pragma unroll
                for (int jj = i; jj < 6; ++jj) { acc[k] += J[i] * v0[jj] + J[6 + i] * v1[jj]; ++k; }
#pragma unroll
              for (int i = 0; i < 6; ++i) acc[21 + i] -= jD * J[i] + jE * J[6 + i];
            }
          }
        };
        auto project = [&](bool cand_, double X, double Y, double Z, float& u, float& v) -> bool {
          const PLSVO_LDS double* const pq = (const PLSVO_LDS double*)pose_rt;
          const double x_cam = pq[0] * X + pq[1] * Y + pq[2] * Z + pq[9];
          const double y_cam = pq[3] * X + pq[4] * Y + pq[5] * Z + pq[10];
          const double z_cam = pq[6] * X + pq[7] * Y + pq[8] * Z + pq[11];
          u = (float)((job.fx * (x_cam / z_cam) + job.cx) * scale);
          v = (float)((job.fy * (y_cam / z_cam) + job.cy) * scale);
          return cand_ && (u >= 2.0f) && (v >= 2.0f) && (u < colmax) && (v < rowmax);
        };

          const float4* const cache_f = reinterpret_cast<const float4*>(b.cache_ref);
          for (int pb = (terms_only ? 0 : slot_lo) + wave * 64; pb < n_rounds_slots; pb += T) {
            const int p = pb + lane;
            struct Rows3 { float4 r4, x4, y4; };
            auto load_row = [&](int r) -> Rows3 {
              Rows3 c;
              c.r4 = make_float4(0.f, 0.f, 0.f, 0.f); c.x4 = c.r4; c.y4 = c.r4;
              if (p < n_rounds_slots) {
                const float4* const cf = cache_f + ((pbase + p) * 4 + r) * 3;
                c.r4 = cf[0]; c.x4 = cf[1]; c.y4 = cf[2];
              }
              return c;
            };
            Rows3 row_cur = load_row(0);
            int2 meta = make_int2(SLOT_HOLE, 0);
            if (p < n_slots) meta = s_meta[p];
            const bool hole = meta.x == SLOT_HOLE;
            const bool is_line = !hole && meta.x < 0;
            bool cand = !hole && p < n_rounds_slots;
            if (cand && is_line && s_dead[-1 - meta.x]) cand = false;
            double X = 0.0, Y = 0.0, Z = 1.0;
            if (cand) { X = s_xyz[3 * p]; Y = s_xyz[3 * p + 1]; Z = s_xyz[3 * p + 2]; }
            float u, v;
            const bool live = project(cand, X, Y, Z, u, v);
            uint32_t wlo[5], whi[5]; int wsh[5];
#pragma unroll
            for (int r = 0; r < 5; ++r) { wlo[r] = 0u; whi[r] = 0u; wsh[r] = 0; }
            PatchW pw = { 0, 0, 0.f, 0.f, 0.f, 0.f };
            if (live) {
              pw = patch_weights(u, v);
#pragma unroll
              for (int r = 0; r < 5; ++r) {
                const int off = (pw.vi - 2 + r) * pitch + (pw.ui - 2);
                wsh[r] = off & 3;
                wlo[r] = *reinterpret_cast<const uint32_t*>(cur_img + (off & ~3)); whi[r] = *reinterpret_cast<const uint32_t*>(cur_img + (off & ~3) + 4);
              }
            }
            const double z_inv = 1.0 / Z;
            PixSums ps = { 0.0, 0.0, 0.0, 0.0, 0.0, 0.0, 0.0f };
            const bool any_point = __any(live && !is_line) != 0;
            const bool chi_out = (accumulate || terms_only) && store_chi && p < job.n_pts;
            if (chi_out && !live) {
#pragma unroll
              for (int r = 0; r < 4; ++r) chi_store(p, r, make_float4(0.f, 0.f, 0.f, 0.f));
            }
            if (__any(live)) {
              float ra[5], rb[5];
              unpack5(wlo[0], whi[0], wsh[0], ra);
#pragma unroll
              for (int r = 0; r < 4; ++r) {
                const Rows3 c = row_cur;
                if (r < 3) row_cur = load_row(r + 1);
                float* const top = (r & 1) ? rb : ra;
                float* const bot = (r & 1) ? ra : rb;
                unpack5(wlo[r + 1], whi[r + 1], wsh[r + 1], bot);
                if (live) {
                  float4 chi_t = make_float4(0.f, 0.f, 0.f, 0.f);
                  if (any_point) row4(std::true_type{}, !is_line, pw, top, bot, c.r4, c.x4, c.y4, chi_t, ps);
                  else row4(std::false_type{}, !is_line, pw, top, bot, c.r4, c.x4, c.y4, chi_t, ps);
                  if (chi_out) chi_store(p, r, chi_t);
                }
              }
            }
            if (!terms_only) slot_finish(p, meta, is_line, cand, live, X, Y, Z, z_inv, ps);
          }
        } else {
        struct SlotA { int2 meta; bool cand; double X, Y, Z; };
        auto stage_a = [&](int pb_) -> SlotA {
          SlotA f;
          const int p_ = pb_ + tid;
          f.meta = make_int2(SLOT_HOLE, 0);
          if (p_ < n_slots) f.meta = s_meta[p_];
          f.cand = f.meta.x != SLOT_HOLE;
          if (f.cand && f.meta.x < 0 && s_dead[-1 - f.meta.x]) f.cand = false;
          f.X = 0.0; f.Y = 0.0; f.Z = 1.0;
          if (f.cand) { f.X = pxyz[3 * p_]; f.Y = pxyz[3 * p_ + 1]; f.Z = pxyz[3 * p_ + 2]; }
          return f;
        };
        struct SlotC { uint4 q[4]; };
        auto stage_c = [&](int pb_, bool cand_) -> SlotC {
          SlotC c;
#pragma unroll
          for (int r = 0; r < 4; ++r) c.q[r] = make_uint4(0u, 0u, 0u, 0u);
          if (cand_) {
            const uint4* const rec = reinterpret_cast<const uint4*>(b.cache_ref) + (pbase + pb_ + tid) * 4;
#pragma unroll
            for (int r = 0; r < 4; ++r) c.q[r] = rec[r];
          }
          return c;
        };
        struct SlotB { bool live; float u, v; uint32_t wlo[5], whi[5]; int wsh[5]; };
        auto stage_b = [&](const SlotA& a_) -> SlotB {
          SlotB g;
          const PLSVO_LDS double* const pq = (const PLSVO_LDS double*)pose_rt;
          const double x_cam = pq[0] * a_.X + pq[1] * a_.Y + pq[2] * a_.Z + pq[9];
          const double y_cam = pq[3] * a_.X + pq[4] * a_.Y + pq[5] * a_.Z + pq[10];
          const double z_cam = pq[6] * a_.X + pq[7] * a_.Y + pq[8] * a_.Z + pq[11];
          g.u = (float)((job.fx * (x_cam / z_cam) + job.cx) * scale);
          g.v = (float)((job.fy * (y_cam / z_cam) + job.cy) * scale);
          g.live = a_.cand && (g.u >= 2.0f) && (g.v >= 2.0f) && (g.u < colmax) && (g.v < rowmax);
#pragma unroll
          for (int r = 0; r < 5; ++r) { g.wlo[r] = 0u; g.whi[r] = 0u; g.wsh[r] = 0; }
          if (g.live) {
            const int ui = (int)floorf(g.u), vi = (int)floorf(g.v);
            const int x0 = ui - 2, y0 = vi - 2;
            if constexpr (kTiled) {
              const int ca = tiled_col_offset(x0 & ~3), cb = tiled_col_offset((x0 & ~3) + 4);
#pragma unroll
              for (int r = 0; r < 5; ++r) {
                const int q = tiled_row_offset(pitch, y0 + r);
                g.wsh[r] = x0 & 3;
                g.wlo[r] = *reinterpret_cast<const uint32_t*>(cur_img + (q + ca)); g.whi[r] = *reinterpret_cast<const uint32_t*>(cur_img + (q + cb));
              }
            } else {
#pragma unroll
              for (int r = 0; r < 5; ++r) {
                const int off = (y0 + r) * pitch + x0;
                g.wsh[r] = off & 3;
                g.wlo[r] = *reinterpret_cast<const uint32_t*>(cur_img + (off & ~3)); g.whi[r] = *reinterpret_cast<const uint32_t*>(cur_img + (off & ~3) + 4);
              }
            }
          }
          return g;
        };
        SlotA a_nxt = stage_a(0);
        SlotC c_nxt = stage_c(0, a_nxt.cand);
        for (int pb = 0; pb < n_rounds_slots; pb += T) {
          const int p = pb + tid;
          const SlotA sa = a_nxt;
          const SlotC sc = c_nxt;
          const SlotB sb = stage_b(sa);
          a_nxt = stage_a(pb + T);
          const bool next_cand = a_nxt.cand;
          const int2 meta = sa.meta;
          const bool hole = meta.x == SLOT_HOLE;
          const bool is_line = !hole && meta.x < 0;
          const bool cand = sa.cand;
          const double X = sa.X, Y = sa.Y, Z = sa.Z;
          const float u = sb.u, v = sb.v;
          const bool live = sb.live;
          const uint32_t* const wlo = sb.wlo; const uint32_t* const whi = sb.whi; const int* const wsh = sb.wsh;

          double sA = 0, sB = 0, sC = 0, sD = 0, sE = 0, sChi = 0;
          float sAbs = 0.0f;
          const bool any_point = __any(live && !is_line) != 0;
          const bool chi_out = (accumulate || terms_only) && store_chi && p < job.n_pts;
          PLSVO_LDS plsvo_v4f* const chi_lds = (PLSVO_LDS plsvo_v4f*)(s_win + (iter & 1) * b.chi_lds_pts * 16 + p * 16);
          PLSVO_GLOBAL plsvo_v4f* const chi_glb = (PLSVO_GLOBAL plsvo_v4f*)(chi_it + (unsigned)(p * 16));
          auto chi_store = [&](int r, const float4& t) {
            const plsvo_v4f t4 = { t.x, t.y, t.z, t.w };
            if (b.chi_lds_pts > 0) chi_lds[r] = t4; else chi_glb[r] = t4;
          };
          if (chi_out && !live) {
#pragma unroll
            for (int r = 0; r < 4; ++r) chi_store(r, make_float4(0.f, 0.f, 0.f, 0.f));
          }
          if (live) {
            const PatchW pw = patch_weights(u, v);
            auto unpack5 = [](uint32_t lo, uint32_t hi, int sh, float* o) {
              const uint32_t w0 = __builtin_amdgcn_alignbyte(hi, lo, (uint32_t)sh);
              o[0] = (float)(w0 & 0xffu); o[1] = (float)((w0 >> 8) & 0xffu); o[2] = (float)((w0 >> 16) & 0xffu); o[3] = (float)(w0 >> 24);
              o[4] = (float)((hi >> (8 * sh)) & 0xffu);
            };
            const bool is_point = !is_line;
            auto row4 = [&](auto WEIGHTED, const float* top, const float* bot, const float4& r4, const float4& x4, const float4& y4, float4& tv4) {
              constexpr bool weighted = decltype(WEIGHTED)::value;
              const float* pr = reinterpret_cast<const float*>(&r4);
              const float* pxp = reinterpret_cast<const float*>(&x4);
              const float* pyp = reinterpret_cast<const float*>(&y4);
              float* tv = reinterpret_cast<float*>(&tv4);
#pragma unroll
              for (int x = 0; x < 4; ++x) {
                const float c = bilinear(pw.wTL, pw.wTR, pw.wBL, pw.wBR, top[x], top[x + 1], bot[x], bot[x + 1]);
                const float res = __fsub_rn(c, pr[x]);
                const float ares = fabsf(res);
                const double rd = (double)res, dx = (double)pxp[x], dy = (double)pyp[x];
                if (weighted) {
                  const float w = is_point ? robust_weight(ares) : 1.0f;
                  const double wd = (double)w;
                  const double wdx = wd * dx, wdy = wd * dy;
                  sA += wdx * dx; sB += wdx * dy; sC += wdy * dy;
                  sD += wdx * rd; sE += wdy * rd;
                  const float term = __fmul_rn(__fmul_rn(res, res), w);
                  sChi += (double)term;
                  tv[x] = is_point ? term : ares;
                } else {
                  sA += dx * dx; sB += dx * dy; sC += dy * dy;
                  sD += dx * rd; sE += dy * rd;
                  tv[x] = ares;
                }
                sAbs += ares;
              }
            };
            float ra[5], rb[5];
            unpack5(wlo[0], whi[0], wsh[0], ra);
            RecordRows rec;
            rec.start(sc.q);
            auto patch_row = [&](auto RI) {
              constexpr int r = decltype(RI)::value;
              float* const top = (r & 1) ? rb : ra;
              float* const bot = (r & 1) ? ra : rb;
              unpack5(wlo[r + 1], whi[r + 1], wsh[r + 1], bot);
              float4 chi_t = make_float4(0.f, 0.f, 0.f, 0.f);
              float4 r4, x4, y4;
              rec.template row<r>(r4, x4, y4);
              if (any_point) row4(std::true_type{}, top, bot, r4, x4, y4, chi_t);
              else row4(std::false_type{}, top, bot, r4, x4, y4, chi_t);
              if (chi_out) chi_store(r, chi_t);
            };
            patch_row(std::integral_constant<int, 0>{}); patch_row(std::integral_constant<int, 1>{});
            patch_row(std::integral_constant<int, 2>{}); patch_row(std::integral_constant<int, 3>{});
          }
          c_nxt = stage_c(pb + T, next_cand);

          double wh = 0.0, wj = 0.0;
          if (__any(is_line && cand)) {
            if (write_abs) {
              if (is_line && cand) s_abs[p] = live ? sAbs : -1.0f;
              wave_lds_fence();
            }
            if (accumulate && is_line && cand) {
              const int first = meta.y & 0xfffff, N = meta.y >> 20;
              bool good = true; float sum = 0.0f;
              for (int n = 0; n < N; ++n) { const float a = s_abs[first + n]; good = good && (a >= 0.0f); sum += a; }
              const float res_ = (float)((double)sum / (double)N);
              if (good && (double)res_ < 200.0) {
                const float w = (float)(1.0 / (1.0 + (double)res_));
                wh = (double)w / (double)res_;
                wj = (double)w;
                if (p == first) {
                  const float term = __fmul_rn(__fmul_rn(res_, res_), w);
                  acc[27] += (double)term; acc[28] += 1.0;
                  s_lterm[(iter & 1) * scap + (-1 - meta.x)] = term;
                }
              } else if (p == first) {
                s_dead[-1 - meta.x] = iter + 1;
                b.seg_alive[job.seg_off + (-1 - meta.x)] = 0;
              }
            }
          }
          if (accumulate) {
            if (!is_line && live) {
              wh = 1.0; wj = 1.0;
              acc[27] += sChi; acc[28] += (double)PLSVO_PATCH_AREA;
            }
            if (live) { acc[29] += 1.0; if (!is_line && store_chi && b.chi_lds_pts == 0) acc[30] += 1.0; }
            if (wh != 0.0 || wj != 0.0) {
              const double xyz[3] = { X, Y, Z };
              double J[12];
              jacobian_xyz2uv(xyz, J);
              const double hs = wh * fs * fs, js = wj * fs;
              const double hA = sA * hs, hB = sB * hs, hC = sC * hs, jD = sD * js, jE = sE * js;
              double v0[6], v1[6];
#pragma unroll
              for (int k = 0; k < 6; ++k) { v0[k] = hA * J[k] + hB * J[6 + k]; v1[k] = hB * J[k] + hC * J[6 + k]; }
              int k = 0;
#pragma unroll
              for (int i = 0; i < 6; ++i)
#pragma unroll
                for (int jj = i; jj < 6; ++jj) { acc[k] += J[i] * v0[jj] + J[6 + i] * v1[jj]; ++k; }
#pragma unroll
              for (int i = 0; i < 6; ++i) acc[21 + i] -= jD * J[i] + jE * J[6 + i];
            }
          }
        }
        }
        if (long_lines && pass == 0) block_sync<T>();
      }
      TICK(1);

      if (!terms_only) {
        double out2[2];
        row_reduce_scatter32(acc, out2);
        const int k0 = row_reduce_scatter32_index(lane);
        *reinterpret_cast<double2*>(s_red + (tid >> 4) * 32 + k0) = make_double2(out2[0], out2[1]);
      }
      block_sync<T>();
      TICK(2);

      if (wave == 0 && stage == last_stage) {
        double tot = terms_only ? s_tot[lane & 31] : reduce_rows_finish<ROWS>(s_red);
        if constexpr (kQuad) {
          if (pair) {
            if ((lane & 31) == 31) tot = (double)s_ctl[5];
            const double theirs = pair_allgather32(xb, rank, xseq, tot, x_lost);
            ++xseq;
            tot = rank == 0 ? tot + theirs : theirs + tot;
          }
        }
        if (lane < 32 && !terms_only) s_tot[lane] = tot;
        TICK(3);
        double x[6];
        wave_solve6_reg(tot, x, job.ldlt_flavour, kQuad);
        TICK(4);
        const double chi_sum = readlane_f64(tot, 27), nm_d = readlane_f64(tot, 28), ev_d = readlane_f64(tot, 29), ev_pt = readlane_f64(tot, 30);
        const unsigned long long nm = (unsigned long long)(nm_d + 0.5);
        double new_chi2 = (double)((float)chi_sum / (float)nm);
        double old_chi2 = s_pose[26];
        const float band = kChiBand * __fsqrt_rn((float)nm_d) * 5.9604644775390625e-8f;
        const bool near = iter > 0 && !s_ctl[1] && !isnan(x[0]) && fabs(new_chi2 - old_chi2) <= (double)band * old_chi2;
        const bool have_terms = terms_only || b.chi_lds_pts > 0 || (s_ctl[7] != 0 && s_ctl[8] != 0);
        const bool tie = near && have_terms;
        const bool defer = near && !have_terms;
        if (defer && lane == 0) {
          s_ctl[10] = (s_ctl[7] != 0 ? 0 : 1) | (s_ctl[8] != 0 ? 0 : 2);
          if (s_ctl[8] == 0) {
            const SE3d om = se3_load(s_pose + 19);
            quat_to_matrix(om.q, s_red); s_red[9] = om.t[0]; s_red[10] = om.t[1]; s_red[11] = om.t[2];
          }
        }
        if (tie) {
          if (b.chi_lds_pts > 0)
            exact_chi2_pair_lds((const PLSVO_LDS float*)(s_win + (iter & 1) * b.chi_lds_pts * 16), (const PLSVO_LDS float*)(s_win + ((iter & 1) ^ 1) * b.chi_lds_pts * 16),
                                own_pts ? job.n_pts : 0, own_segs ? job.n_seg : 0, iter, (const PLSVO_LDS int*)s_dead, (const PLSVO_LDS float*)s_lterm, scap, (PLSVO_LDS float*)s_lterm + 2 * scap);
          else
            exact_chi2_pair((const PLSVO_GLOBAL float*)(b.chi_terms + (size_t)(iter & 1) * b.chi_plane + (size_t)job.pt_off * 16),
                            (const PLSVO_GLOBAL float*)(b.chi_terms + (size_t)((iter & 1) ^ 1) * b.chi_plane + (size_t)job.pt_off * 16),
                            job.n_pts, job.n_seg, iter, (const PLSVO_LDS int*)s_dead, (PLSVO_LDS float*)s_win, (const PLSVO_LDS float*)s_lterm, scap,
                            (PLSVO_LDS float*)s_lterm + 2 * scap);
          float FA = s_lterm[2 * scap], FB = s_lterm[2 * scap + 1];
          if constexpr (kQuad) {
            if (pair) {
              const double mine = (lane & 31) == 0 ? (double)FA : ((lane & 31) == 1 ? (double)FB : 0.0);
              const double theirs = pair_allgather32(xb, rank, xseq, mine, x_lost);
              ++xseq;
              const float TA = (float)readlane_f64(theirs, 0), TB = (float)readlane_f64(theirs, 1);
              FA = rank == 0 ? __fadd_rn(FA, TA) : __fadd_rn(TA, FA);
              FB = rank == 0 ? __fadd_rn(FB, TB) : __fadd_rn(TB, FB);
            }
          }
          new_chi2 = (double)(FA / (float)nm);
          old_chi2 = (double)(FB / (float)(unsigned long long)(s_pose[30] + 0.5));
        }
        TICK(7);
        if (x_lost && lane == 0) s_ctl[3] = 2;
        if (lane == 0 && !defer) {
          s_ctl[10] = 0;
          s_pose[27] += ev_d;
          s_pose[31] += ev_pt;
          s_pose[30] = nm_d;
          s_ctl[2] += 1;
          if (tie) s_ctl[6] += 1;
          if (near && !have_terms) s_ctl[9] += 1;
          int stop = s_ctl[1];
          if (isnan(x[0]) || x_lost) stop = 1;
          SE3d model = se3_load(s_pose + 12);
          int accepted, brk = 0;
          if ((iter > 0 && new_chi2 > old_chi2) || stop) {
            model = se3_load(s_pose + 19);
            accepted = 0; brk = 1;
          } else {
            double mx[6];
            for (int k = 0; k < 6; ++k) mx[k] = -x[k];
            const SE3d nm_ = se3_mul_dev(model, se3_exp_dev(mx));
            se3_store(model, s_pose + 19);
            model = nm_;
            s_pose[26] = new_chi2;
            accepted = 1;
            if (norm_max6(x) <= job.eps) brk = 1;
          }
          s_ctl[8] = s_ctl[7];
          s_ctl[7] = (accepted && norm_max6(x) < 1e-3) ? 1 : 0;
          se3_store(model, s_pose + 12);
          quat_to_matrix(model.q, s_pose); s_pose[9] = model.t[0]; s_pose[10] = model.t[1]; s_pose[11] = model.t[2];
          s_ctl[1] = stop; s_ctl[0] = brk;
          if (b.log && lead) {
            const int lc = st->log_count;
            if (lc < b.log_cap) {
              plsvo_align_iterlog* r = b.log + (size_t)job_id * b.log_cap + lc;
              r->level = level; r->iter = iter; r->accepted = accepted; r->stop = stop; r->n_meas = nm; r->new_chi2 = new_chi2;
              for (int k = 0; k < 6; ++k) r->x[k] = x[k];
              se3_store(model, r->T_after);
            }
            st->log_count = lc + 1;
          }
        }
      }
      TICK(5);
      block_sync<T>();
      if (stage == 0) redo_mask = s_ctl[10];
     }
      if (b.log && tid == 0 && lead) {
        const int lc = st->log_count - 1;
        if (lc >= 0 && lc < b.log_cap) {
          plsvo_align_iterlog* r = b.log + (size_t)job_id * b.log_cap + lc;
          for (int i = 0; i < 6; ++i) for (int jj = 0; jj < 6; ++jj) r->H[i * 6 + jj] = s_tot[sym6_index(i, jj)];
          for (int k = 0; k < 6; ++k) r->Jres[k] = s_tot[21 + k];
        }
      }
#if defined(PLSVO_TIMING) && PLSVO_TIMING == 3
      if (iter == 0) TICK_RAW(7); else TICK_RAW(6);
#endif
      TICK(6);
      if (s_ctl[0]) break;
    }

    if (tid == 0) {
      if (lead) st->iters[level] = s_ctl[2];
      s_pose[28] += pair ? s_tot[31] : (double)s_ctl[5];
      s_pose[29] += s_pose[27];
    }
  }

  block_sync<T>();
  if (tid == 0 && lead) {
    for (int k = 0; k < 7; ++k) st->T[k] = s_pose[12 + k];
    if (b.poses) for (int k = 0; k < 7; ++k) b.poses[7 * job_id + k] = s_pose[12 + k];
    st->chi2 = s_pose[26];
    st->patch_levels += (unsigned long long)(s_pose[28] + 0.5);
    st->patch_iters += (unsigned long long)(s_pose[29] + 0.5);
    if (b.work_key) b.work_key[job_id] = (int)fmin(s_pose[29] + 0.5, 2147483647.0);
    st->patch_iters_pt += (unsigned long long)(s_pose[31] + 0.5);
    st->stop = s_ctl[1];
    if (s_ctl[3]) st->error = s_ctl[3];
    st->chi2_ties += s_ctl[6];
    st->chi2_unarmed += s_ctl[9];
    st->n_meas = (unsigned long long)(s_tot[28] + 0.5);
    for (int i = 0; i < 6; ++i) for (int jj = 0; jj < 6; ++jj) st->H[i * 6 + jj] = s_tot[sym6_index(i, jj)];
#ifdef PLSVO_TIMING
    for (int k = 0; k < 8; ++k) st->phase_ticks[k] += s_time[k];
#endif
  }
}


size_t align_level_lds_bytes(int threads, int cap, int scap, int chi_lds_pts) { return align_lds_used(threads, cap, scap, chi_lds_pts); }

}
extern "C" const char* plsvo_hip_build_flags(void) { return ""; }
namespace plsvo_hip {

template <int T>
static hipError_t launch_fused_T(const AlignBatchDev& b, int cap, int scap, int level_hi, int level_lo, int do_init, size_t lds, hipStream_t stream) {
  hipError_t e = hipFuncSetAttribute(reinterpret_cast<const void*>(align_fused_kernel<T>), hipFuncAttributeMaxDynamicSharedMemorySize, (int)lds);
  if (e != hipSuccess) return e;
  const unsigned grid = (T >= kQuadMinThreads && b.pair) ? (unsigned)((b.n_jobs + 7) / 8) * 16u : (unsigned)b.n_jobs;
#ifdef PLSVO_WAVE_EMU
  wave_emu::pair_stride() = (T >= kQuadMinThreads && b.pair) ? 8 : 0;
#endif
  hipLaunchKernelGGL((align_fused_kernel<T>), dim3(grid), dim3(T), lds, stream, b, cap, scap, level_hi, level_lo, do_init);
#ifdef PLSVO_WAVE_EMU
  wave_emu::pair_stride() = 0;
#endif
  return hipGetLastError();
}

__global__ __launch_bounds__(1024) void align_reorder_kernel(const int* work_key, int n, int* order_out, int shift) {
  __shared__ int s_hist[1024];
  __shared__ int s_scan[1024];
  const int tid = threadIdx.x;
  auto bin_of = [&](int j) -> int {
    const int b_ = work_key[j] >> shift;
    return 1023 - (b_ > 1023 ? 1023 : (b_ < 0 ? 0 : b_));
  };
  s_hist[tid] = 0;
  __syncthreads();
  for (int j = tid; j < n; j += 1024) atomicAdd(&s_hist[bin_of(j)], 1);
  __syncthreads();
  int v = s_hist[tid];
  s_scan[tid] = v;
  __syncthreads();
  for (int d = 1; d < 1024; d <<= 1) {
    const int add = tid >= d ? s_scan[tid - d] : 0;
    __syncthreads();
    s_scan[tid] += add;
    __syncthreads();
  }
  s_hist[tid] = s_scan[tid] - v;
  __syncthreads();
  for (int j = tid; j < n; j += 1024) order_out[atomicAdd(&s_hist[bin_of(j)], 1)] = j;
}
hipError_t launch_align_reorder(const int* work_key, int n, int* order_out, int shift, hipStream_t stream) {
  hipLaunchKernelGGL(align_reorder_kernel, dim3(1), dim3(1024), 0, stream, work_key, n, order_out, shift);
  return hipGetLastError();
}

hipError_t launch_align_levels(const AlignBatchDev& b, int cap, int scap, int level_hi, int level_lo, int do_init, int threads, size_t lds,
                               hipStream_t stream) {
  switch (threads) {
    case 64: return launch_fused_T<64>(b, cap, scap, level_hi, level_lo, do_init, lds, stream);
    case 128: return launch_fused_T<128>(b, cap, scap, level_hi, level_lo, do_init, lds, stream);
    case 256: return launch_fused_T<256>(b, cap, scap, level_hi, level_lo, do_init, lds, stream);
    case 512: return launch_fused_T<512>(b, cap, scap, level_hi, level_lo, do_init, lds, stream);
    default: return hipErrorInvalidValue;
  }
}

}
```

pl-svo_amd/csrc/plsvo_capi.hip:

```cpp
#include <hip/hip_runtime.h>
#include <dlfcn.h>
#include <rccl/rccl.h>

#include <algorithm>
#include <chrono>
#include <cmath>
#include <cstdio>
#include <cstdlib>
#include <cstring>
#include <string>
#include <vector>

#include "../../include/plsvo_hip.h"
#include "plsvo_dev.hpp"
#include "plsvo_math.hpp"

namespace plsvo_hip {
size_t align_level_lds_bytes(int threads, int cap, int scap, int chi_lds_pts);
hipError_t launch_align_reorder(const int* work_key, int n, int* order_out, int shift, hipStream_t stream);
hipError_t launch_align_levels(const AlignBatchDev& b, int cap, int scap, int level_hi, int level_lo, int do_init, int threads, size_t lds,
                               hipStream_t stream);
hipError_t launch_pose_opt(const PoseBatchDev& b, double* d_poses, int threads, hipStream_t stream);
hipError_t launch_structopt(const StructBatchDev& s, hipStream_t stream);
hipError_t launch_match_direct(const MatchBatchDev& b, hipStream_t stream);
hipError_t launch_reproject(const ReprojBatchDev& b, hipStream_t stream);
hipError_t launch_update_seeds(const SeedsBatchDev& b, hipStream_t stream);
hipError_t launch_halfsample(const uint8_t* src, size_t src_pitch, int in_w, int in_h, int in_stride, uint8_t* dst,
                             size_t dst_pitch, int n_slots, int rounding, hipStream_t stream);
hipError_t launch_copy_level0(const uint8_t* src, size_t src_pitch, int w, int h, int stride, uint8_t* dst, size_t dst_pitch,
                              int n_slots, hipStream_t stream);
hipError_t launch_chain_pose(const ChainBatchDev& b, hipStream_t stream);
hipError_t launch_pack_pose_records(const AlignStateDev* ast, const PoseStateDev* pst, int n, plsvo_pose_record* dst, hipStream_t stream);
hipError_t launch_chain_active(const ChainBatchDev& b, hipStream_t stream);
hipError_t launch_chain_select(const ChainBatchDev& b, hipStream_t stream);
hipError_t launch_tile_level(const uint8_t* src, size_t src_pitch, int w, int h, uint8_t* dst, size_t dst_pitch, int n_slots, hipStream_t stream);
hipError_t launch_rectify(const uint8_t* raw, size_t raw_pitch, int stride, int flip, const uint32_t* map, int w, int h, uint8_t* dst,
                          size_t dst_pitch, int n_slots, hipStream_t stream);
hipError_t launch_detect_fast(const DetectLaunch& a, int n_slots, hipStream_t stream);
hipError_t launch_detect_stages(const DetectLaunch& a, hipStream_t stream);
hipError_t launch_detect_compact(unsigned long long* keys, int n_cells, plsvo_corner* corners, int32_t* counts, int n_slots, hipStream_t stream);
}

using namespace plsvo_hip;

static thread_local std::string g_create_error;

namespace {

struct DevBuf {
  void* p = nullptr;
  size_t cap = 0;
  hipError_t ensure(size_t bytes) {
    if (bytes <= cap) return hipSuccess;
    if (p) { hipError_t e = hipFree(p); p = nullptr; cap = 0; if (e != hipSuccess) return e; }
    size_t want = std::max(bytes, (size_t)256);
    hipError_t e = hipMalloc(&p, want);
    if (e == hipSuccess) cap = want;
    return e;
  }
  void release() { if (p) (void)hipFree(p); p = nullptr; cap = 0; }
  template <typename T> T* as() const { return reinterpret_cast<T*>(p); }
};

struct EventPair { hipEvent_t a, b; };

struct Blob {
  std::vector<uint8_t> host;
  template <typename T> size_t add(const std::vector<T>& v) {
    const size_t off = (host.size() + 255) & ~(size_t)255;
    host.resize(off + std::max(v.size() * sizeof(T), (size_t)16));
    if (!v.empty()) memcpy(host.data() + off, v.data(), v.size() * sizeof(T));
    return off;
  }
};

}

struct plsvo_ctx {
  int device = 0;
  hipStream_t stream = nullptr;
  bool own_stream = false;
  std::string err;
  int cu_count = 0;
  size_t lds_per_block = 65536;
  int env_align_threads = 0, env_align_lds_pad = 0, env_poseopt_threads = 0;
  bool env_align_per_level = false, env_align_no_lpt = false, env_host_timing = false;
  int ldlt_flavour = 320;

  DevBuf pyr_tiled;
  DevBuf pyr_slab;
  PyrDesc pyr{};
  DevBuf pyr_upload;
  struct RectifyMap { DevBuf map; int w = 0, h = 0; bool identity = false, flip = false; };
  RectifyMap rect[PLSVO_MAX_RECTIFY_MAPS];
  int rect_n = 0;
  DevBuf det_keys, det_occ, det_corners, det_counts, det_stage;

  int a_n = 0;
  bool a_staged = false;
  std::vector<AlignJobDev> a_jobs;
  std::vector<int> a_nseg_off;
  int a_total_seg = 0;
  int a_gmax = -1, a_gmin = 99;
  int a_cap[PLSVO_MAX_LEVELS]{};
  int a_scap = 4;
  int a_trace_cap = 0;
  DevBuf a_d_state, a_d_alive;
  DevBuf a_d_pxyz, a_d_puv, a_d_cref, a_d_chi, a_d_log, a_d_poses;
  size_t a_patch_total = 0;
  int a_seg_align = 32;
  DevBuf a_d_workkey;
  DevBuf a_d_order[2];
  int a_order_next = 0;
  bool env_align_no_reorder = false;
  const int* a_stage_order = nullptr;
  bool a_one_shot = false, p_one_shot = false;
  int env_align_reorder_min = 0;
  DevBuf a_d_xbuf;
  unsigned int x_launch = 0;
  bool env_align_no_pair = false;
  AlignBatchDev a_b{};

  int p_n = 0;
  bool p_staged = false;
  std::vector<PoseJobDev> p_jobs;
  int p_total_pt = 0, p_total_seg = 0;
  int p_trace_cap = 0;
  DevBuf p_d_state, p_d_ptkeep, p_d_segkeep;
  DevBuf p_d_s32, p_d_s64, p_d_log, p_d_poses;
  PoseBatchDev p_b{};
  DevBuf p_d_workkey, p_d_order[2];
  int p_order_next = 0, p_key_shift = 0;
  bool env_poseopt_no_reorder = false;
  int env_poseopt_reorder_min = 0;

  bool ch_staged = false;
  int ch_n = 0, ch_ncand = 0, ch_npt_cap = 0, ch_nseg_cap = 0;
  std::vector<ChainJobDev> ch_jobs;
  DevBuf ch_d_blob, ch_d_work, ch_d_po;
  ChainBatchDev ch_b{};
  MatchBatchDev ch_match{};
  ReprojBatchDev ch_reproj{};
  PoseBatchDev ch_pose{};
  DevBuf ch_d_state, ch_d_ptkeep, ch_d_segkeep, ch_d_s32, ch_d_s64, ch_d_poses;
  DevBuf rec_d;
  unsigned long long run_seq = 0, a_run_seq = 0, p_run_seq = 0, ch_run_seq = 0;

  DevBuf s_d_in, s_d_out;

  DevBuf a_d_blob, p_d_blob;
  void* pinned[2] = { nullptr, nullptr };
  size_t pinned_cap[2] = { 0, 0 };
  hipEvent_t pinned_done[2] = { nullptr, nullptr };
  int pinned_next = 0;
  void* pyr_pinned[2] = { nullptr, nullptr };
  size_t pyr_pinned_cap[2] = { 0, 0 };
  hipEvent_t pyr_pinned_done[2] = { nullptr, nullptr };
  int pyr_pinned_next = 0;
  std::vector<uint8_t> tiled_stale;
  int tiled_stale_count = 0;
  void* dl_pinned = nullptr;
  size_t dl_pinned_cap = 0;

  bool profiling = false;
  std::vector<EventPair> ev[PLSVO_K_COUNT];
  std::vector<EventPair> ev_pool;
  double ev_ms[PLSVO_K_COUNT]{};
  int64_t ev_launches[PLSVO_K_COUNT]{};
};

#define CTX_CHECK(ctx) do { if (!(ctx)) return PLSVO_E_INVALID; } while (0)
#define HIP_TRY(ctx, expr)                                                                      \
  do {                                                                                          \
    hipError_t e__ = (expr);                                                                    \
    if (e__ != hipSuccess) {                                                                    \
      (ctx)->err = std::string(#expr) + ": " + hipGetErrorString(e__);                          \
      return PLSVO_E_HIP;                                                                       \
    }                                                                                           \
  } while (0)
static int fail(plsvo_ctx* ctx, int code, const std::string& msg) { ctx->err = msg; return code; }

static void prof_begin(plsvo_ctx* c, int k, EventPair* ep) {
  if (!c->profiling) return;
  if (!c->ev_pool.empty()) { *ep = c->ev_pool.back(); c->ev_pool.pop_back(); }
  else { (void)hipEventCreate(&ep->a); (void)hipEventCreate(&ep->b); }
  (void)hipEventRecord(ep->a, c->stream);
  (void)k;
}
static void prof_end(plsvo_ctx* c, int k, EventPair* ep) {
  if (!c->profiling) return;
  (void)hipEventRecord(ep->b, c->stream);
  c->ev[k].push_back(*ep);
}
static void prof_collect(plsvo_ctx* c) {
  for (int k = 0; k < PLSVO_K_COUNT; ++k) {
    for (auto& ep : c->ev[k]) {
      float ms = 0.f;
      if (hipEventSynchronize(ep.b) == hipSuccess && hipEventElapsedTime(&ms, ep.a, ep.b) == hipSuccess) {
        c->ev_ms[k] += (double)ms; c->ev_launches[k] += 1;
      }
      c->ev_pool.push_back(ep);
    }
    c->ev[k].clear();
  }
}

extern "C" const char* plsvo_hip_version(void) { return "plsvo_hip 0.1 (gfx950)"; }

static int create_ctx(int device_id, void* stream, bool use_given_stream, plsvo_ctx** out);
static bool env_flag(const char* name) { const char* s = getenv(name); return s && *s && strcmp(s, "0") != 0; }
extern "C" int plsvo_hip_create(int device_id, void* stream, plsvo_ctx** out) { return create_ctx(device_id, stream, stream != nullptr, out); }
extern "C" int plsvo_hip_create_on_stream(int device_id, void* stream, plsvo_ctx** out) { return create_ctx(device_id, stream, true, out); }

static int create_ctx(int device_id, void* stream, bool use_given_stream, plsvo_ctx** out) {
  if (!out) return PLSVO_E_INVALID;
  *out = nullptr;
  int n = 0;
  hipError_t e = hipGetDeviceCount(&n);
  if (e != hipSuccess || n <= 0) {
    g_create_error = std::string("no HIP device available (") + (e != hipSuccess ? hipGetErrorString(e) : "count=0") +
                     "); plsvo_hip has no CPU fallback";
    return PLSVO_E_NODEVICE;
  }
  if (device_id < 0 || device_id >= n) { g_create_error = "device_id out of range"; return PLSVO_E_INVALID; }
  if ((e = hipSetDevice(device_id)) != hipSuccess) { g_create_error = hipGetErrorString(e); return PLSVO_E_HIP; }
  plsvo_ctx* c = new plsvo_ctx();
  c->device = device_id;
  hipDeviceProp_t prop;
  if (hipGetDeviceProperties(&prop, device_id) == hipSuccess) {
    c->cu_count = prop.multiProcessorCount;
    c->lds_per_block = prop.sharedMemPerBlock;
    int optin = 0;
    if (hipDeviceGetAttribute(&optin, hipDeviceAttributeMaxSharedMemoryPerBlock, device_id) == hipSuccess && optin > 0)
      c->lds_per_block = std::max(c->lds_per_block, (size_t)optin);
  }
  if (use_given_stream) { c->stream = reinterpret_cast<hipStream_t>(stream); c->own_stream = false; }
  else {
    if ((e = hipStreamCreateWithFlags(&c->stream, hipStreamNonBlocking)) != hipSuccess) {
      g_create_error = hipGetErrorString(e); delete c; return PLSVO_E_HIP;
    }
    c->own_stream = true;
  }
  if (const char* s = getenv("PLSVO_LDS_LIMIT")) c->lds_per_block = (size_t)atol(s);
  if (const char* s = getenv("PLSVO_ALIGN_THREADS")) { const int v = atoi(s); if (v == 64 || v == 128 || v == 256 || v == 512) c->env_align_threads = v; }
  if (const char* s = getenv("PLSVO_ALIGN_LDS_PAD")) c->env_align_lds_pad = std::max(0, atoi(s));
  if (const char* s = getenv("PLSVO_POSEOPT_THREADS")) { const int v = atoi(s); if (v == 16 || v == 64 || v == 256 || v == 512) c->env_poseopt_threads = v; }
  if (const char* s = getenv("PLSVO_ALIGN_PER_LEVEL")) c->env_align_per_level = atoi(s) != 0;
  c->env_align_no_lpt = env_flag("PLSVO_ALIGN_NO_LPT");
  c->env_align_no_pair = env_flag("PLSVO_ALIGN_NO_PAIR");
  c->env_align_no_reorder = env_flag("PLSVO_ALIGN_NO_REORDER");
  if (const char* s = getenv("PLSVO_ALIGN_REORDER_MIN")) c->env_align_reorder_min = atoi(s);
  c->env_poseopt_no_reorder = env_flag("PLSVO_POSEOPT_NO_REORDER");
  if (const char* s = getenv("PLSVO_POSEOPT_REORDER_MIN")) c->env_poseopt_reorder_min = atoi(s);
  c->env_host_timing = getenv("PLSVO_HOST_TIMING") != nullptr;
  *out = c;
  return PLSVO_OK;
}

extern "C" void plsvo_hip_destroy(plsvo_ctx* c) {
  if (!c) return;
  (void)hipSetDevice(c->device);
  (void)hipStreamSynchronize(c->stream);
  prof_collect(c);
  for (auto& ep : c->ev_pool) { (void)hipEventDestroy(ep.a); (void)hipEventDestroy(ep.b); }
  c->a_d_xbuf.release(); c->a_d_order[0].release(); c->a_d_order[1].release(); c->a_d_workkey.release(); c->p_d_workkey.release(); c->p_d_order[0].release(); c->p_d_order[1].release();
  DevBuf* bufs[] = { &c->pyr_slab, &c->pyr_tiled, &c->pyr_upload, &c->a_d_blob, &c->a_d_state, &c->a_d_alive, &c->a_d_pxyz, &c->a_d_puv, &c->a_d_cref,
                     &c->a_d_chi, &c->a_d_log, &c->a_d_poses, &c->p_d_blob, &c->p_d_state, &c->p_d_ptkeep, &c->p_d_segkeep, &c->p_d_s32, &c->p_d_s64,
                     &c->p_d_log, &c->p_d_poses, &c->s_d_in, &c->s_d_out, &c->ch_d_blob, &c->ch_d_work, &c->ch_d_po, &c->ch_d_state,
                     &c->ch_d_ptkeep, &c->ch_d_segkeep, &c->ch_d_s32, &c->ch_d_s64, &c->ch_d_poses, &c->rec_d };
  for (DevBuf* b : bufs) b->release();
  for (auto& r : c->rect) r.map.release();
  c->det_keys.release(); c->det_occ.release(); c->det_corners.release(); c->det_counts.release(); c->det_stage.release();
  for (int k = 0; k < 2; ++k) { if (c->pinned[k]) (void)hipHostFree(c->pinned[k]); if (c->pinned_done[k]) (void)hipEventDestroy(c->pinned_done[k]); }
  for (int k = 0; k < 2; ++k) { if (c->pyr_pinned[k]) (void)hipHostFree(c->pyr_pinned[k]); if (c->pyr_pinned_done[k]) (void)hipEventDestroy(c->pyr_pinned_done[k]); }
  if (c->dl_pinned) (void)hipHostFree(c->dl_pinned);
  if (c->own_stream) (void)hipStreamDestroy(c->stream);
  delete c;
}

extern "C" int plsvo_hip_set_option(plsvo_ctx* c, int option, int value) {
  CTX_CHECK(c);
  if (option == PLSVO_OPT_LDLT_FLAVOUR) {
    if (value != 320 && value != 330) return fail(c, PLSVO_E_INVALID, "set_option: the LDLT flavour is 320 (Eigen 3.1 ... 3.2.1) or 330 (Eigen 3.2.2 and later)");
    c->ldlt_flavour = value;
    c->a_staged = false; c->p_staged = false;
    return PLSVO_OK;
  }
  if (option == PLSVO_OPT_ALIGN_THREADS) {
    if (value != 0 && value != 64 && value != 128 && value != 256 && value != 512) return fail(c, PLSVO_E_INVALID, "set_option: alignment launch shape is 0 (automatic), 64, 128, 256 or 512 threads per frame");
    c->env_align_threads = value;
    return PLSVO_OK;
  }
  if (option == PLSVO_OPT_POSEOPT_THREADS) {
    if (value != 0 && value != 16 && value != 64 && value != 256 && value != 512) return fail(c, PLSVO_E_INVALID, "set_option: pose-optimiser launch shape is 0 (automatic), 16 (a 16-lane row per frame, four frames per wave), 64, 256 or 512 threads per frame");
    c->env_poseopt_threads = value;
    return PLSVO_OK;
  }
  if (option == PLSVO_OPT_ALIGN_REORDER || option == PLSVO_OPT_POSEOPT_REORDER) {
    if (value != 0 && value != 1) return fail(c, PLSVO_E_INVALID, "set_option: the launch-order refresh is 0 (keep the stage order) or 1 (refresh from the last launch's measured work)");
    if (option == PLSVO_OPT_ALIGN_REORDER) {
      c->env_align_no_reorder = value == 0;
      if (value == 0 && c->a_staged && c->a_d_blob.p) c->a_b.order = c->a_stage_order;
    } else {
      c->env_poseopt_no_reorder = value == 0;
    }
    return PLSVO_OK;
  }
  return fail(c, PLSVO_E_INVALID, "set_option: unknown option");
}

extern "C" const char* plsvo_hip_last_error(const plsvo_ctx* c) { return c ? c->err.c_str() : g_create_error.c_str(); }
extern "C" void* plsvo_hip_stream(plsvo_ctx* c) { return c ? reinterpret_cast<void*>(c->stream) : nullptr; }
extern "C" int plsvo_hip_synchronize(plsvo_ctx* c) { CTX_CHECK(c); HIP_TRY(c, hipStreamSynchronize(c->stream)); return PLSVO_OK; }

extern "C" int plsvo_hip_device_info(plsvo_ctx* c, char* name, int name_len, int* cu_count, size_t* hbm_bytes) {
  CTX_CHECK(c);
  hipDeviceProp_t prop;
  HIP_TRY(c, hipGetDeviceProperties(&prop, c->device));
  if (name && name_len > 0) { snprintf(name, (size_t)name_len, "%s (%s)", prop.name, prop.gcnArchName); }
  if (cu_count) *cu_count = prop.multiProcessorCount;
  if (hbm_bytes) *hbm_bytes = prop.totalGlobalMem;
  return PLSVO_OK;
}

extern "C" int plsvo_hip_config_pyramids(plsvo_ctx* c, int n_slots, int width, int height, int n_levels) {
  CTX_CHECK(c);
  if (n_slots <= 0 || width <= 0 || height <= 0 || n_levels <= 0 || n_levels > PLSVO_MAX_LEVELS) return fail(c, PLSVO_E_INVALID, "config_pyramids: bad arguments");
  HIP_TRY(c, hipSetDevice(c->device));
  PyrDesc d{};
  size_t off = 0;
  for (int l = 0; l < n_levels; ++l) {
    d.w[l] = width >> l; d.h[l] = height >> l;
    if (d.w[l] <= 0 || d.h[l] <= 0) return fail(c, PLSVO_E_INVALID, "config_pyramids: too many levels for this image size");
    d.off[l] = pyr_level_offset(width, height, l);
    off = (size_t)pyr_level_offset(width, height, l + 1);
  }
  d.slot_bytes = off; d.n_slots = n_slots; d.n_levels = n_levels;
  d.tslot_bytes = pyr_tiled_level_offset(width, height, n_levels);
  HIP_TRY(c, hipStreamSynchronize(c->stream));
  HIP_TRY(c, c->pyr_slab.ensure((size_t)n_slots * off + 256));
  HIP_TRY(c, hipMemsetAsync(c->pyr_slab.p, 0, (size_t)n_slots * off + 256, c->stream));
  HIP_TRY(c, c->pyr_tiled.ensure((size_t)n_slots * d.tslot_bytes + 256));
  HIP_TRY(c, hipMemsetAsync(c->pyr_tiled.p, 0, (size_t)n_slots * d.tslot_bytes + 256, c->stream));
  d.base = c->pyr_slab.as<uint8_t>();
  d.tbase = c->pyr_tiled.as<uint8_t>();
  c->pyr = d;
  c->tiled_stale.assign((size_t)n_slots, 0); c->tiled_stale_count = 0;
  c->a_staged = false;
  c->ch_staged = false;
  return PLSVO_OK;
}

static int check_slot(plsvo_ctx* c, int slot) {
  if (!c->pyr.base) return fail(c, PLSVO_E_STATE, "pyramids not configured");
  if (slot < 0 || slot >= c->pyr.n_slots) return fail(c, PLSVO_E_CAPACITY, "pyramid slot out of range");
  return PLSVO_OK;
}

static int retile(plsvo_ctx* c, int first_slot, int n, int n_levels) {
  const uint8_t* src = c->pyr_slab.as<uint8_t>() + (size_t)first_slot * c->pyr.slot_bytes;
  uint8_t* dst = c->pyr_tiled.as<uint8_t>() + (size_t)first_slot * c->pyr.tslot_bytes;
  for (int l = 0; l < n_levels; ++l)
    HIP_TRY(c, launch_tile_level(src + c->pyr.off[l], c->pyr.slot_bytes, c->pyr.w[l], c->pyr.h[l],
                                 dst + pyr_tiled_level_offset(c->pyr.w[0], c->pyr.h[0], l), c->pyr.tslot_bytes, n, c->stream));
  return PLSVO_OK;
}

static void mark_tiled_fresh(plsvo_ctx* c, int first, int n) {
  if (c->tiled_stale_count == 0) return;
  for (int s = first; s < first + n && s < (int)c->tiled_stale.size(); ++s)
    if (c->tiled_stale[(size_t)s]) { c->tiled_stale[(size_t)s] = 0; --c->tiled_stale_count; }
}
static int retile_stale(plsvo_ctx* c, const std::vector<int>& slots) {
  if (c->tiled_stale_count == 0) return PLSVO_OK;
  for (int sl : slots) {
    if (sl < 0 || sl >= (int)c->tiled_stale.size() || !c->tiled_stale[(size_t)sl]) continue;
    int rc = retile(c, sl, 1, c->pyr.n_levels); if (rc) return rc;
    c->tiled_stale[(size_t)sl] = 0; --c->tiled_stale_count;
    if (c->tiled_stale_count == 0) break;
  }
  return PLSVO_OK;
}

extern "C" int plsvo_hip_upload_pyramid(plsvo_ctx* c, int slot, int n_levels, const uint8_t* const* level_ptr, const int* width,
                                        const int* height, const int* stride_bytes) {
  CTX_CHECK(c);
  int rc = check_slot(c, slot); if (rc) return rc;
  if (!level_ptr || !width || !height || !stride_bytes || n_levels <= 0 || n_levels > c->pyr.n_levels) return fail(c, PLSVO_E_INVALID, "upload_pyramid: bad arguments");
  HIP_TRY(c, hipSetDevice(c->device));
  for (int l = 0; l < n_levels; ++l) {
    if (!level_ptr[l] || width[l] != c->pyr.w[l] || height[l] != c->pyr.h[l] || stride_bytes[l] < width[l])
      return fail(c, PLSVO_E_INVALID, "upload_pyramid: level size does not match the configured pyramid");
  }
  uint8_t* const slot_dst = c->pyr_slab.as<uint8_t>() + (size_t)slot * c->pyr.slot_bytes;
  const size_t image_bytes = (size_t)c->pyr.off[n_levels - 1] + (size_t)width[n_levels - 1] * (size_t)height[n_levels - 1];
  const int k = c->pyr_pinned_next;
  if (!c->pyr_pinned_done[k] && hipEventCreate(&c->pyr_pinned_done[k]) != hipSuccess) c->pyr_pinned_done[k] = nullptr;
  bool packed = false;
  if (c->pyr_pinned_done[k]) {
    HIP_TRY(c, hipEventSynchronize(c->pyr_pinned_done[k]));
    if (c->pyr_pinned_cap[k] < image_bytes) {
      if (c->pyr_pinned[k]) (void)hipHostFree(c->pyr_pinned[k]);
      c->pyr_pinned[k] = nullptr; c->pyr_pinned_cap[k] = 0;
      if (hipHostMalloc(&c->pyr_pinned[k], (size_t)c->pyr.slot_bytes, hipHostMallocDefault) == hipSuccess) {
        c->pyr_pinned_cap[k] = (size_t)c->pyr.slot_bytes;
        memset(c->pyr_pinned[k], 0, c->pyr_pinned_cap[k]);
      }
    }
    if (c->pyr_pinned[k]) {
      uint8_t* const img = static_cast<uint8_t*>(c->pyr_pinned[k]);
      for (int l = 0; l < n_levels; ++l) {
        uint8_t* d = img + c->pyr.off[l];
        const size_t w = (size_t)width[l];
        if ((size_t)stride_bytes[l] == w) memcpy(d, level_ptr[l], w * (size_t)height[l]);
        else for (int y = 0; y < height[l]; ++y) memcpy(d + (size_t)y * w, level_ptr[l] + (size_t)y * (size_t)stride_bytes[l], w);
      }
      HIP_TRY(c, hipMemcpyAsync(slot_dst, img, image_bytes, hipMemcpyHostToDevice, c->stream));
      HIP_TRY(c, hipEventRecord(c->pyr_pinned_done[k], c->stream));
      c->pyr_pinned_next = k ^ 1;
      packed = true;
    }
  }
  if (!packed) {
    for (int l = 0; l < n_levels; ++l)
      HIP_TRY(c, hipMemcpy2DAsync(slot_dst + c->pyr.off[l], (size_t)width[l], level_ptr[l], (size_t)stride_bytes[l], (size_t)width[l], (size_t)height[l],
                                  hipMemcpyHostToDevice, c->stream));
    HIP_TRY(c, hipStreamSynchronize(c->stream));
  }
  if (!c->tiled_stale[(size_t)slot]) { c->tiled_stale[(size_t)slot] = 1; ++c->tiled_stale_count; }
  return PLSVO_OK;
}

static int build_levels(plsvo_ctx* c, int first_slot, int n, int rounding) {
  uint8_t* base = c->pyr_slab.as<uint8_t>() + (size_t)first_slot * c->pyr.slot_bytes;
  for (int l = 1; l < c->pyr.n_levels; ++l) {
    EventPair ep{}; prof_begin(c, PLSVO_K_HALFSAMPLE, &ep);
    HIP_TRY(c, launch_halfsample(base + c->pyr.off[l - 1], c->pyr.slot_bytes, c->pyr.w[l - 1], c->pyr.h[l - 1], c->pyr.w[l - 1],
                                 base + c->pyr.off[l], c->pyr.slot_bytes, n, rounding, c->stream));
    prof_end(c, PLSVO_K_HALFSAMPLE, &ep);
  }
  const int rc_t = retile(c, first_slot, n, c->pyr.n_levels);
  if (rc_t) {
    for (int s = first_slot; s < first_slot + n && s < (int)c->tiled_stale.size(); ++s)
      if (!c->tiled_stale[(size_t)s]) { c->tiled_stale[(size_t)s] = 1; ++c->tiled_stale_count; }
    return rc_t;
  }
  mark_tiled_fresh(c, first_slot, n);
  return PLSVO_OK;
}

extern "C" int plsvo_hip_build_pyramid(plsvo_ctx* c, int slot, const uint8_t* level0, int stride_bytes, int rounding) {
  CTX_CHECK(c);
  int rc = check_slot(c, slot); if (rc) return rc;
  if (!level0 || stride_bytes < c->pyr.w[0]) return fail(c, PLSVO_E_INVALID, "build_pyramid: bad arguments");
  HIP_TRY(c, hipSetDevice(c->device));
  uint8_t* dst = c->pyr_slab.as<uint8_t>() + (size_t)slot * c->pyr.slot_bytes + c->pyr.off[0];
  HIP_TRY(c, hipMemcpy2DAsync(dst, (size_t)c->pyr.w[0], level0, (size_t)stride_bytes, (size_t)c->pyr.w[0], (size_t)c->pyr.h[0],
                              hipMemcpyHostToDevice, c->stream));
// ... 392 lines not shown
  if (!pinned) fallback.resize(std::max(total, (size_t)64));
  uint8_t* const base = pinned ? static_cast<uint8_t*>(c->dl_pinned) : fallback.data();
  for (int k = 0; k < n_ranges; ++k) {
    void* to = static_cast<void*>(base + off[k]);
    h[k] = static_cast<const uint8_t*>(to);
    if (bytes[k]) HIP_TRY(c, hipMemcpyAsync(to, src[k], bytes[k], hipMemcpyDeviceToHost, c->stream));
  }
  HIP_TRY(c, hipStreamSynchronize(c->stream));
  return PLSVO_OK;
}

static const size_t kPinnedMax = (size_t)8 << 20;
static int upload_blob(plsvo_ctx* c, DevBuf& buf, const Blob& blob) {
  const size_t bytes = std::max(blob.host.size(), (size_t)256);
  HIP_TRY(c, buf.ensure(bytes));
  if (blob.host.empty()) return PLSVO_OK;
  if (blob.host.size() <= kPinnedMax) {
    const int k = c->pinned_next;
    if (!c->pinned_done[k] && hipEventCreate(&c->pinned_done[k]) != hipSuccess) c->pinned_done[k] = nullptr;
    if (c->pinned_done[k]) {
      HIP_TRY(c, hipEventSynchronize(c->pinned_done[k]));
      if (c->pinned_cap[k] < blob.host.size()) {
        if (c->pinned[k]) (void)hipHostFree(c->pinned[k]);
        c->pinned[k] = nullptr; c->pinned_cap[k] = 0;
        const size_t want = std::max(blob.host.size() * 2, (size_t)1 << 20);
        if (hipHostMalloc(&c->pinned[k], want, hipHostMallocDefault) == hipSuccess) c->pinned_cap[k] = want; else c->pinned[k] = nullptr;
      }
      if (c->pinned[k]) {
        memcpy(c->pinned[k], blob.host.data(), blob.host.size());
        HIP_TRY(c, hipMemcpyAsync(buf.p, c->pinned[k], blob.host.size(), hipMemcpyHostToDevice, c->stream));
        HIP_TRY(c, hipEventRecord(c->pinned_done[k], c->stream));
        c->pinned_next = k ^ 1;
        return PLSVO_OK;
      }
    }
  }
  HIP_TRY(c, hipMemcpyAsync(buf.p, blob.host.data(), blob.host.size(), hipMemcpyHostToDevice, c->stream));
  HIP_TRY(c, hipStreamSynchronize(c->stream));
  return PLSVO_OK;
}

extern "C" int plsvo_align_stage(plsvo_ctx* c, int n, const plsvo_align_in* in) {
  CTX_CHECK(c);
  if (n <= 0 || !in) return fail(c, PLSVO_E_INVALID, "align_stage: bad arguments");
  if (!c->pyr.base) return fail(c, PLSVO_E_STATE, "align_stage: pyramids not configured");
  HIP_TRY(c, hipSetDevice(c->device));
  c->a_staged = false;
  c->ch_staged = false;
  std::vector<AlignJobDev> jobs((size_t)n);
  std::vector<double> T0((size_t)n * 7), ptpx, ptxyz, spx, epx, len, sp, sq;
  std::vector<uint8_t> alive;
  int gmax = -1, gmin = 99;
  const int cus_stage = c->cu_count > 0 ? c->cu_count : 256;
  const int seg_align = (2 * n <= cus_stage) ? 64 : 32;
  int caps[PLSVO_MAX_LEVELS] = { 0 };
  std::vector<long long> work((size_t)n, 0);
  std::vector<int> seg_slot[PLSVO_MAX_LEVELS];
  size_t patch_total = 0;
  for (int j = 0; j < n; ++j) {
    const plsvo_align_in& a = in[j];
    if (a.n_pts < 0 || a.n_seg < 0 || a.max_level < a.min_level || a.min_level < 0 || a.max_level >= c->pyr.n_levels || a.n_iter < 0)
      return fail(c, PLSVO_E_INVALID, "align_stage: bad job parameters (levels must exist in the configured pyramid)");
    if (a.ref_slot < 0 || a.ref_slot >= c->pyr.n_slots || a.cur_slot < 0 || a.cur_slot >= c->pyr.n_slots)
      return fail(c, PLSVO_E_CAPACITY, "align_stage: pyramid slot out of range");
    if (a.cam.width != c->pyr.w[0] || a.cam.height != c->pyr.h[0])
      return fail(c, PLSVO_E_INVALID, "align_stage: camera size does not match the configured pyramid");
    if ((a.n_pts > 0 && (!a.pt_px || !a.pt_xyz_ref)) || (a.n_seg > 0 && (!a.seg_spx || !a.seg_epx || !a.seg_len || !a.seg_p_ref || !a.seg_q_ref)))
      return fail(c, PLSVO_E_INVALID, "align_stage: null feature array");
    AlignJobDev& J = jobs[(size_t)j];
    J.ref_slot = a.ref_slot; J.cur_slot = a.cur_slot;
    J.fx = a.cam.fx; J.fy = a.cam.fy; J.cx = a.cam.cx; J.cy = a.cam.cy; J.width = a.cam.width; J.height = a.cam.height;
    J.max_level = a.max_level; J.min_level = a.min_level; J.n_iter = a.n_iter; J.eps = a.eps;
    J.skip = (a.n_pts == 0 && a.n_seg == 0) ? 1 : 0;
    J.pt_off = (int)(ptpx.size() / 2); J.n_pts = a.n_pts; J.seg_off = (int)len.size(); J.n_seg = a.n_seg;
    for (int k = 0; k < 7; ++k) T0[(size_t)j * 7 + k] = a.T_cur_from_ref[k];
    ptpx.insert(ptpx.end(), a.pt_px, a.pt_px + 2 * (size_t)a.n_pts);
    ptxyz.insert(ptxyz.end(), a.pt_xyz_ref, a.pt_xyz_ref + 3 * (size_t)a.n_pts);
    spx.insert(spx.end(), a.seg_spx, a.seg_spx + 2 * (size_t)a.n_seg);
    epx.insert(epx.end(), a.seg_epx, a.seg_epx + 2 * (size_t)a.n_seg);
    len.insert(len.end(), a.seg_len, a.seg_len + (size_t)a.n_seg);
    sp.insert(sp.end(), a.seg_p_ref, a.seg_p_ref + 3 * (size_t)a.n_seg);
    sq.insert(sq.end(), a.seg_q_ref, a.seg_q_ref + 3 * (size_t)a.n_seg);
    for (int s = 0; s < a.n_seg; ++s) alive.push_back(a.seg_alive_in ? (a.seg_alive_in[s] ? 1 : 0) : 1);
    int ub_max = 0;
    long long ub_sum = 0;
    J.long_mask = 0; J.ldlt_flavour = c->ldlt_flavour;
    for (int l = 0; l < PLSVO_MAX_LEVELS; ++l) J.n_slots[l] = 0;
    std::vector<int> codes((size_t)std::max(a.n_seg, 1));
    for (int l = a.max_level; l >= a.min_level; --l) {
      int n_slots = 0, long_lines = 0; long long n_real = 0;
      const int lrc = slot_layout(&a, l, seg_align, codes.data(), &n_slots, &long_lines, &n_real);
      if (lrc == PLSVO_E_CAPACITY) return fail(c, PLSVO_E_CAPACITY, "align_stage: a segment with more than 2047 samples or more than 2^20 patch slots in one job");
      if (lrc != PLSVO_OK) return fail(c, lrc, "align_stage: slot layout failed");
      seg_slot[(size_t)l].insert(seg_slot[(size_t)l].end(), codes.begin(), codes.begin() + a.n_seg);
      if (long_lines) J.long_mask |= 1 << l;
      const int slots4 = (n_slots + 3) & ~3;
      J.n_slots[l] = n_slots;
      ub_sum += n_real;
      if (!J.skip) caps[l] = std::max(caps[l], slots4);
      ub_max = std::max(ub_max, slots4);
    }
    J.patch_off = (int)patch_total; J.patch_cap = ub_max;
    work[(size_t)j] = J.skip ? 0 : ub_sum;
    patch_total += (size_t)ub_max;
    if (patch_total > (size_t)0x7fffffff / 16) return fail(c, PLSVO_E_CAPACITY, "align_stage: batch too large (patch index overflow)");
    if (!J.skip) { gmax = std::max(gmax, a.max_level); gmin = std::min(gmin, a.min_level); }
    for (int l = 0; l < PLSVO_MAX_LEVELS; ++l)
      if (l > a.max_level || l < a.min_level) seg_slot[(size_t)l].insert(seg_slot[(size_t)l].end(), (size_t)a.n_seg, -1);
  }
  std::vector<int> order((size_t)n);
  for (int j = 0; j < n; ++j) order[(size_t)j] = j;
  if (!c->env_align_no_lpt) std::stable_sort(order.begin(), order.end(), [&](int x, int y) { return work[(size_t)x] > work[(size_t)y]; });
  int rc;
  const int slot_level0 = (gmax >= gmin && gmax >= 0) ? gmin : 0;
  const size_t total_seg = len.size();
  std::vector<int> slot_table;
  for (int l = slot_level0; l <= std::max(gmax, slot_level0); ++l) slot_table.insert(slot_table.end(), seg_slot[(size_t)l].begin(), seg_slot[(size_t)l].end());
  if (slot_table.empty()) slot_table.push_back(-1);
  Blob blob;
  const size_t o_slot = blob.add(slot_table), o_order = blob.add(order), o_jobs = blob.add(jobs), o_T0 = blob.add(T0), o_ptpx = blob.add(ptpx),
               o_ptxyz = blob.add(ptxyz), o_spx = blob.add(spx), o_epx = blob.add(epx), o_len = blob.add(len), o_sp = blob.add(sp),
               o_sq = blob.add(sq), o_alive = blob.add(alive);
  if ((rc = upload_blob(c, c->a_d_blob, blob))) return rc;
  HIP_TRY(c, c->a_d_alive.ensure(std::max(alive.size(), (size_t)1)));
  HIP_TRY(c, c->a_d_state.ensure((size_t)n * sizeof(AlignStateDev)));
  HIP_TRY(c, c->a_d_poses.ensure((size_t)n * 7 * sizeof(double)));
  const size_t pt = std::max(patch_total, (size_t)4);
  HIP_TRY(c, c->a_d_pxyz.ensure(pt * 3 * sizeof(double)));
  HIP_TRY(c, c->a_d_puv.ensure(pt * 2 * sizeof(float)));
  HIP_TRY(c, c->a_d_cref.ensure(pt * 64));
  c->a_patch_total = pt;
  const size_t npt_total = ptpx.size() / 2 + 32;
  HIP_TRY(c, c->a_d_chi.ensure(2 * npt_total * 16 * sizeof(float)));
  if (c->a_trace_cap > 0) HIP_TRY(c, c->a_d_log.ensure((size_t)n * c->a_trace_cap * sizeof(plsvo_align_iterlog)));

  AlignBatchDev& b = c->a_b;
  uint8_t* const base = c->a_d_blob.as<uint8_t>();
  b.jobs = reinterpret_cast<const AlignJobDev*>(base + o_jobs); b.state = c->a_d_state.as<AlignStateDev>();
  b.T0 = reinterpret_cast<const double*>(base + o_T0);
  b.pt_px = reinterpret_cast<const double*>(base + o_ptpx); b.pt_xyz = reinterpret_cast<const double*>(base + o_ptxyz);
  b.seg_spx = reinterpret_cast<const double*>(base + o_spx); b.seg_epx = reinterpret_cast<const double*>(base + o_epx);
  b.seg_len = reinterpret_cast<const double*>(base + o_len);
  b.seg_p = reinterpret_cast<const double*>(base + o_sp); b.seg_q = reinterpret_cast<const double*>(base + o_sq);
  b.seg_alive_in = base + o_alive; b.seg_alive = c->a_d_alive.as<uint8_t>();
  b.patch_xyz = c->a_d_pxyz.as<double>(); b.patch_uvref = c->a_d_puv.as<float>();
  b.cache_ref = c->a_d_cref.as<float>();
  b.chi_terms = c->a_d_chi.as<float>(); b.chi_plane = (unsigned long long)npt_total * 16;
  b.seg_slot = reinterpret_cast<const int*>(base + o_slot); b.slot_level0 = slot_level0; b.slot_stride = (int)total_seg;
  b.poses = c->a_d_poses.as<double>();
  b.pyr = c->pyr;
  b.log = c->a_trace_cap > 0 ? c->a_d_log.as<plsvo_align_iterlog>() : nullptr;
  b.log_cap = c->a_trace_cap;
  b.n_jobs = n;
  b.pair = 0; b.xseq0 = 0; b.xbuf = nullptr; b.work_key = nullptr;
  b.order = reinterpret_cast<const int*>(base + o_order);
  c->a_stage_order = b.order;
  c->a_jobs.swap(jobs);
  c->a_n = n; c->a_total_seg = (int)alive.size(); c->a_gmax = gmax; c->a_gmin = gmin;
  for (int l = 0; l < PLSVO_MAX_LEVELS; ++l) c->a_cap[l] = caps[l];
  c->a_scap = 4;
  for (int j = 0; j < n; ++j) c->a_scap = std::max(c->a_scap, in[j].n_seg);
  c->a_seg_align = seg_align;
  c->a_staged = true; c->a_run_seq = 0;
  return PLSVO_OK;
}

static void pick_align_config(const plsvo_ctx* c, int n_jobs, int cap, int scap, int max_pts, int* threads, size_t* lds, int* chi_lds_pts) {
  const int cus = c->cu_count > 0 ? c->cu_count : 256;
  int t = 64;
  if (n_jobs <= cus) t = 512;
  else if (n_jobs <= 4 * cus) t = 256;
  else if (n_jobs < 64 * cus) t = 128;
  if (c->env_align_threads) t = c->env_align_threads;
  int pts = t >= 256 ? ((max_pts + 3) & ~3) : 0;
  if (pts > 0 && align_level_lds_bytes(t, cap, scap, pts) > c->lds_per_block) pts = 0;
  *chi_lds_pts = pts;
  *threads = t; *lds = align_level_lds_bytes(t, cap, scap, pts);
  *lds += (size_t)c->env_align_lds_pad;
}

namespace {
struct Roctx {
  int (*push)(const char*) = nullptr;
  int (*pop)() = nullptr;
  Roctx() {
    void* h = dlopen("librocprofiler-sdk-roctx.so", RTLD_LAZY | RTLD_GLOBAL);
    if (!h) h = dlopen("librocprofiler-sdk-roctx.so.1", RTLD_LAZY | RTLD_GLOBAL);
    if (!h) return;
    push = reinterpret_cast<int (*)(const char*)>(dlsym(h, "roctxRangePushA"));
    pop = reinterpret_cast<int (*)()>(dlsym(h, "roctxRangePop"));
    if (!push || !pop) { push = nullptr; pop = nullptr; }
  }
};
const Roctx& roctx() { static const Roctx r; return r; }
struct RoctxRange {
  explicit RoctxRange(const char* name) { if (roctx().push) roctx().push(name); }
  ~RoctxRange() { if (roctx().pop) roctx().pop(); }
};
}

extern "C" int plsvo_align_run(plsvo_ctx* c) {
  CTX_CHECK(c);
  RoctxRange range("sparse_img_align");
  if (!c->a_staged) return fail(c, PLSVO_E_STATE, "align_run: no staged batch");
  HIP_TRY(c, hipSetDevice(c->device));
  int cap = 4;
  const bool have_levels = c->a_gmax >= c->a_gmin && c->a_gmax >= 0;
  if (have_levels) for (int l = c->a_gmin; l <= c->a_gmax; ++l) cap = std::max(cap, c->a_cap[l]);
  int threads; size_t lds;
  const int scap = (c->a_scap + 3) & ~3;
  int max_pts = 0, chi_lds_pts = 0;
  for (const AlignJobDev& J : c->a_jobs) max_pts = std::max(max_pts, J.n_pts);
  pick_align_config(c, c->a_n, cap, scap, max_pts, &threads, &lds, &chi_lds_pts);
  c->a_b.chi_lds_pts = chi_lds_pts;
  if (lds > c->lds_per_block) return fail(c, PLSVO_E_CAPACITY, "align_run: slot tables do not fit in LDS (too many features in one job)");
  if (threads <= 64 && c->tiled_stale_count > 0) {
    std::vector<int> slots;
    slots.reserve(2 * c->a_jobs.size());
    for (const AlignJobDev& J : c->a_jobs) { slots.push_back(J.ref_slot); slots.push_back(J.cur_slot); }
    const int rc_t = retile_stale(c, slots); if (rc_t) return rc_t;
  }
  const int cus_run = c->cu_count > 0 ? c->cu_count : 256;
  int max_iter = 0;
  for (const AlignJobDev& J : c->a_jobs) max_iter = std::max(max_iter, J.n_iter);
  const long long max_exchanges = have_levels ? (long long)(c->a_gmax - c->a_gmin + 1) * (long long)max_iter * 2 : 0;
  const bool pair = threads >= kQuadMinThreads && chi_lds_pts > 0 && c->a_seg_align == 64 && 2 * c->a_n <= cus_run && !c->env_align_no_pair &&
                    !c->env_align_per_level && have_levels && max_exchanges < 1024;
  c->a_b.pair = pair ? 1 : 0;
  if (pair) {
    const size_t xbytes = (size_t)c->a_n * 256 * sizeof(unsigned long long);
    if (c->a_d_xbuf.cap < xbytes) {
      HIP_TRY(c, c->a_d_xbuf.ensure(std::max(xbytes, (size_t)128 * 2048)));
      HIP_TRY(c, hipMemsetAsync(c->a_d_xbuf.p, 0, c->a_d_xbuf.cap, c->stream));
    }
    c->a_b.xbuf = c->a_d_xbuf.as<unsigned long long>();
    c->x_launch = (c->x_launch + 1u) & 0x3fffffu;
    if (c->x_launch == 0) {
      HIP_TRY(c, hipMemsetAsync(c->a_d_xbuf.p, 0, c->a_d_xbuf.cap, c->stream));
      c->x_launch = 1;
    }
    c->a_b.xseq0 = c->x_launch << 10;
  }
  if (threads >= kQuadMinThreads) {
    HIP_TRY(c, c->a_d_cref.ensure(c->a_patch_total * 192));
    c->a_b.cache_ref = c->a_d_cref.as<float>();
  }
  const bool per_level = c->env_align_per_level;
  const bool reorder = have_levels && !per_level && c->a_n > (c->env_align_reorder_min > 0 ? c->env_align_reorder_min - 1 : cus_run * 512 / threads) &&
                       !c->env_align_no_reorder && !c->env_align_no_lpt && !c->a_one_shot;
  c->a_b.work_key = nullptr;
  if (reorder) {
    if (c->a_d_workkey.cap < (size_t)c->a_n * sizeof(int)) {
      HIP_TRY(c, c->a_d_workkey.ensure((size_t)c->a_n * sizeof(int)));
      HIP_TRY(c, hipMemsetAsync(c->a_d_workkey.p, 0, c->a_d_workkey.cap, c->stream));
    }
    c->a_b.work_key = c->a_d_workkey.as<int>();
  }
  if (!per_level || !have_levels) {
    EventPair ep{}; prof_begin(c, PLSVO_K_ALIGN_LEVEL, &ep);
    HIP_TRY(c, launch_align_levels(c->a_b, cap, scap, have_levels ? c->a_gmax : 0, have_levels ? c->a_gmin : 0, 1, threads, lds, c->stream));
    prof_end(c, PLSVO_K_ALIGN_LEVEL, &ep);
    if (reorder) {
      DevBuf& ob = c->a_d_order[c->a_order_next];
      HIP_TRY(c, ob.ensure((size_t)c->a_n * sizeof(int)));
      HIP_TRY(c, launch_align_reorder(c->a_b.work_key, c->a_n, ob.as<int>(), 7, c->stream));
      c->a_b.order = ob.as<int>();
      c->a_order_next ^= 1;
    }
  } else {
    for (int level = c->a_gmax; level >= c->a_gmin; --level) {
      EventPair ep{}; prof_begin(c, PLSVO_K_ALIGN_LEVEL, &ep);
      HIP_TRY(c, launch_align_levels(c->a_b, cap, scap, level, level, level == c->a_gmax ? 1 : 0, threads, lds, c->stream));
      prof_end(c, PLSVO_K_ALIGN_LEVEL, &ep);
    }
  }
  c->a_run_seq = ++c->run_seq;
  return PLSVO_OK;
}

extern "C" int plsvo_align_fetch(plsvo_ctx* c, int n, plsvo_align_out* out) {
  CTX_CHECK(c);
  if (!c->a_staged) return fail(c, PLSVO_E_STATE, "align_fetch: no staged batch");
  if (n != c->a_n || !out) return fail(c, PLSVO_E_INVALID, "align_fetch: n does not match the staged batch");
  HIP_TRY(c, hipSetDevice(c->device));
  std::vector<uint8_t> big;
  const size_t rb[2] = { (size_t)n * sizeof(AlignStateDev), (size_t)std::max(c->a_total_seg, 0) };
  const void* const rs[2] = { c->a_d_state.p, c->a_d_alive.p };
  const uint8_t* rh[2] = { nullptr, nullptr };
  { const int rc_d = download_ranges(c, 2, rs, rb, big, rh); if (rc_d) return rc_d; }
  const AlignStateDev* const st = reinterpret_cast<const AlignStateDev*>(rh[0]);
  const uint8_t* const alive = rh[1];
  int dev_err = 0;
  for (int j = 0; j < n; ++j) {
    const AlignStateDev& s = st[(size_t)j];
    plsvo_align_out& o = out[j];
    uint8_t* alive_out = o.seg_alive_out;
    memset(&o, 0, sizeof(o));
    o.seg_alive_out = alive_out;
    for (int k = 0; k < 7; ++k) o.T_cur_from_ref[k] = s.T[k];
    o.n_meas = s.n_meas; o.n_tracked = s.n_meas / PLSVO_PATCH_AREA;
    for (int k = 0; k < 36; ++k) o.H[k] = s.H[k];
    o.chi2 = s.chi2;
    for (int l = 0; l < PLSVO_MAX_LEVELS; ++l) o.iters_per_level[l] = s.iters[l];
    o.status = s.stop ? 1 : 0;
    if (alive_out && c->a_jobs[(size_t)j].n_seg > 0)
      memcpy(alive_out, alive + c->a_jobs[(size_t)j].seg_off, (size_t)c->a_jobs[(size_t)j].n_seg);
    if (s.error) dev_err = s.error;
  }
  if (dev_err) return fail(c, PLSVO_E_CAPACITY, "align: device-side capacity check failed (code " + std::to_string(dev_err) + ")");
  return PLSVO_OK;
}

extern "C" int plsvo_sparse_align_batch(plsvo_ctx* c, int n, const plsvo_align_in* in, plsvo_align_out* out) {
  const bool host_timing = c && c->env_host_timing;
  const auto t0 = std::chrono::steady_clock::now();
  int rc = plsvo_align_stage(c, n, in); if (rc) return rc;
  const auto t1 = std::chrono::steady_clock::now();
  c->a_one_shot = true;
  rc = plsvo_align_run(c);
  c->a_one_shot = false;
  if (rc) return rc;
  const auto t2 = std::chrono::steady_clock::now();
  rc = plsvo_align_fetch(c, n, out);
  if (host_timing) {
    const auto t3 = std::chrono::steady_clock::now();
    fprintf(stderr, "[plsvo_hip] sparse_align_batch n=%d: stage %.1f us, run (enqueue) %.1f us, fetch (incl. wait) %.1f us\n", n,
            std::chrono::duration<double, std::micro>(t1 - t0).count(), std::chrono::duration<double, std::micro>(t2 - t1).count(),
            std::chrono::duration<double, std::micro>(t3 - t2).count());
  }
  return rc;
}
extern "C" int plsvo_sparse_align(plsvo_ctx* c, const plsvo_align_in* in, plsvo_align_out* out) {
  return plsvo_sparse_align_batch(c, 1, in, out);
}

extern "C" int plsvo_align_set_trace(plsvo_ctx* c, int max_records_per_job) {
  CTX_CHECK(c);
  if (max_records_per_job < 0) return fail(c, PLSVO_E_INVALID, "set_trace: negative capacity");
  c->a_trace_cap = max_records_per_job;
  c->a_staged = false;
  return PLSVO_OK;
}

extern "C" int plsvo_align_fetch_trace(plsvo_ctx* c, int job, plsvo_align_iterlog* out, int max_records, int* n_records) {
  CTX_CHECK(c);
  if (!c->a_staged || c->a_trace_cap <= 0) return fail(c, PLSVO_E_STATE, "fetch_trace: tracing not enabled for the staged batch");
  if (job < 0 || job >= c->a_n || !out || !n_records) return fail(c, PLSVO_E_INVALID, "fetch_trace: bad arguments");
  HIP_TRY(c, hipSetDevice(c->device));
  AlignStateDev s;
  HIP_TRY(c, hipMemcpyAsync(&s, c->a_d_state.as<AlignStateDev>() + job, sizeof(s), hipMemcpyDeviceToHost, c->stream));
  HIP_TRY(c, hipStreamSynchronize(c->stream));
  const int have = std::min(s.log_count, c->a_trace_cap);
  const int nrec = std::min(have, max_records);
  if (nrec > 0) {
    HIP_TRY(c, hipMemcpyAsync(out, c->a_d_log.as<plsvo_align_iterlog>() + (size_t)job * c->a_trace_cap, (size_t)nrec * sizeof(plsvo_align_iterlog),
                              hipMemcpyDeviceToHost, c->stream));
    HIP_TRY(c, hipStreamSynchronize(c->stream));
  }
  *n_records = nrec;
  return PLSVO_OK;
}

extern "C" const double* plsvo_align_poses_dev(plsvo_ctx* c) { return (c && c->a_staged) ? c->a_d_poses.as<double>() : nullptr; }

extern "C" int plsvo_align_phase_ticks(plsvo_ctx* c, unsigned long long* out8) {
  CTX_CHECK(c);
  if (!c->a_staged || !out8) return fail(c, PLSVO_E_STATE, "phase_ticks: no staged batch");
  std::vector<AlignStateDev> st((size_t)c->a_n);
  HIP_TRY(c, hipMemcpyAsync(st.data(), c->a_d_state.p, (size_t)c->a_n * sizeof(AlignStateDev), hipMemcpyDeviceToHost, c->stream));
  HIP_TRY(c, hipStreamSynchronize(c->stream));
  for (int k = 0; k < 8; ++k) { out8[k] = 0; for (auto& s : st) out8[k] += s.phase_ticks[k]; }
  return PLSVO_OK;
}

extern "C" int plsvo_poseopt_phase_ticks(plsvo_ctx* c, unsigned long long* out8) {
  CTX_CHECK(c);
  if (!c->p_staged || !out8) return fail(c, PLSVO_E_STATE, "phase_ticks: no staged batch");
  std::vector<PoseStateDev> st((size_t)c->p_n);
  HIP_TRY(c, hipMemcpyAsync(st.data(), c->p_d_state.p, (size_t)c->p_n * sizeof(PoseStateDev), hipMemcpyDeviceToHost, c->stream));
  HIP_TRY(c, hipStreamSynchronize(c->stream));
  for (int k = 0; k < 8; ++k) { out8[k] = 0; for (auto& s : st) out8[k] += s.phase_ticks[k]; }
  return PLSVO_OK;
}

extern "C" int plsvo_align_copy_poses(plsvo_ctx* c, double* d_dst) {
  CTX_CHECK(c);
  if (!c->a_staged || !d_dst) return fail(c, PLSVO_E_STATE, "align_copy_poses: no staged batch / null destination");
  HIP_TRY(c, hipSetDevice(c->device));
  HIP_TRY(c, hipMemcpyAsync(d_dst, c->a_d_poses.p, (size_t)c->a_n * 7 * sizeof(double), hipMemcpyDeviceToDevice, c->stream));
  return PLSVO_OK;
}

extern "C" int plsvo_align_work(plsvo_ctx* c, uint64_t* patch_levels, uint64_t* patch_iters) {
  CTX_CHECK(c);
  if (!c->a_staged) return fail(c, PLSVO_E_STATE, "align_work: no staged batch");
  HIP_TRY(c, hipSetDevice(c->device));
  std::vector<AlignStateDev> st((size_t)c->a_n);
  HIP_TRY(c, hipMemcpyAsync(st.data(), c->a_d_state.p, (size_t)c->a_n * sizeof(AlignStateDev), hipMemcpyDeviceToHost, c->stream));
  HIP_TRY(c, hipStreamSynchronize(c->stream));
  uint64_t pl = 0, pi = 0;
  for (auto& s : st) { pl += s.patch_levels; pi += s.patch_iters; }
  if (patch_levels) *patch_levels = pl;
  if (patch_iters) *patch_iters = pi;
  return PLSVO_OK;
}

extern "C" int plsvo_align_work_points(plsvo_ctx* c, uint64_t* point_patch_iters) {
  CTX_CHECK(c);
  if (!c->a_staged) return fail(c, PLSVO_E_STATE, "align_work_points: no staged batch");
  HIP_TRY(c, hipSetDevice(c->device));
  std::vector<AlignStateDev> st((size_t)c->a_n);
  HIP_TRY(c, hipMemcpyAsync(st.data(), c->a_d_state.p, (size_t)c->a_n * sizeof(AlignStateDev), hipMemcpyDeviceToHost, c->stream));
  HIP_TRY(c, hipStreamSynchronize(c->stream));
  uint64_t n = 0;
  for (auto& s : st) n += s.patch_iters_pt;
  if (point_patch_iters) *point_patch_iters = n;
  return PLSVO_OK;
}

extern "C" int plsvo_align_launch_order(plsvo_ctx* c, int n, int32_t* order) {
  CTX_CHECK(c);
  if (!c->a_staged) return fail(c, PLSVO_E_STATE, "align_launch_order: no staged batch");
  if (n != c->a_n || !order) return fail(c, PLSVO_E_INVALID, "align_launch_order: n does not match the staged batch");
  HIP_TRY(c, hipSetDevice(c->device));
  if (!c->a_b.order) { for (int j = 0; j < n; ++j) order[j] = j; return PLSVO_OK; }
  HIP_TRY(c, hipMemcpyAsync(order, c->a_b.order, (size_t)n * sizeof(int32_t), hipMemcpyDeviceToHost, c->stream));
  HIP_TRY(c, hipStreamSynchronize(c->stream));
  return PLSVO_OK;
}

extern "C" int plsvo_align_chi2_ties(plsvo_ctx* c, uint64_t* iterations, uint64_t* ties, uint64_t* near_ties_without_terms) {
  CTX_CHECK(c);
  if (!c->a_staged) return fail(c, PLSVO_E_STATE, "align_chi2_ties: no staged batch");
  HIP_TRY(c, hipSetDevice(c->device));
  std::vector<AlignStateDev> st((size_t)c->a_n);
  HIP_TRY(c, hipMemcpyAsync(st.data(), c->a_d_state.p, (size_t)c->a_n * sizeof(AlignStateDev), hipMemcpyDeviceToHost, c->stream));
  HIP_TRY(c, hipStreamSynchronize(c->stream));
  uint64_t it = 0, t = 0, un = 0;
  for (auto& s : st) { t += (uint64_t)s.chi2_ties; un += (uint64_t)s.chi2_unarmed; for (int l = 0; l < PLSVO_MAX_LEVELS; ++l) it += (uint64_t)s.iters[l]; }
  if (iterations) *iterations = it;
  if (ties) *ties = t;
  if (near_ties_without_terms) *near_ties_without_terms = un;
  return PLSVO_OK;
}

extern "C" int plsvo_poseopt_stage(plsvo_ctx* c, int n, const plsvo_poseopt_in* in) {
  CTX_CHECK(c);
  if (n <= 0 || !in) return fail(c, PLSVO_E_INVALID, "poseopt_stage: bad arguments");
  HIP_TRY(c, hipSetDevice(c->device));
  c->p_staged = false;
  std::vector<PoseJobDev> jobs((size_t)n);
  std::vector<double> f, pos, line, spos, epos;
  std::vector<int> plev, slev;
  for (int j = 0; j < n; ++j) {
    const plsvo_poseopt_in& a = in[j];
    if (a.n_pts < 0 || a.n_seg < 0 || a.n_iter < 0) return fail(c, PLSVO_E_INVALID, "poseopt_stage: bad job parameters");
    if ((a.n_pts > 0 && (!a.pt_f || !a.pt_pos || !a.pt_level)) || (a.n_seg > 0 && (!a.seg_line || !a.seg_spos || !a.seg_epos || !a.seg_level)))
      return fail(c, PLSVO_E_INVALID, "poseopt_stage: null feature array");
    PoseJobDev& J = jobs[(size_t)j];
    for (int k = 0; k < 7; ++k) J.T0[k] = a.T_f_w[k];
    J.fx = a.fx; J.reproj_thresh = a.reproj_thresh; J.n_iter = a.n_iter; J.n_iter_ref = a.n_iter_ref; J.ldlt_flavour = c->ldlt_flavour; J.reserved0 = 0;
    J.pt_off = (int)plev.size(); J.n_pts = a.n_pts; J.seg_off = (int)slev.size(); J.n_seg = a.n_seg;
    f.insert(f.end(), a.pt_f, a.pt_f + 3 * (size_t)a.n_pts);
    pos.insert(pos.end(), a.pt_pos, a.pt_pos + 3 * (size_t)a.n_pts);
    plev.insert(plev.end(), a.pt_level, a.pt_level + (size_t)a.n_pts);
    line.insert(line.end(), a.seg_line, a.seg_line + 3 * (size_t)a.n_seg);
    spos.insert(spos.end(), a.seg_spos, a.seg_spos + 3 * (size_t)a.n_seg);
    epos.insert(epos.end(), a.seg_epos, a.seg_epos + 3 * (size_t)a.n_seg);
    slev.insert(slev.end(), a.seg_level, a.seg_level + (size_t)a.n_seg);
    for (int i = 0; i < a.n_pts; ++i) if (a.pt_level[i] < 0 || a.pt_level[i] > 30) return fail(c, PLSVO_E_INVALID, "poseopt_stage: feature level out of range");
    for (int i = 0; i < a.n_seg; ++i) if (a.seg_level[i] < 0 || a.seg_level[i] > 30) return fail(c, PLSVO_E_INVALID, "poseopt_stage: feature level out of range");
  }
  int rc;
  Blob blob;
  const size_t o_jobs = blob.add(jobs), o_f = blob.add(f), o_pos = blob.add(pos), o_plev = blob.add(plev), o_line = blob.add(line),
               o_spos = blob.add(spos), o_epos = blob.add(epos), o_slev = blob.add(slev);
  if ((rc = upload_blob(c, c->p_d_blob, blob))) return rc;
  const size_t npt = plev.size(), nsg = slev.size(), nft = std::max(npt + nsg, (size_t)1);
  HIP_TRY(c, c->p_d_ptkeep.ensure(std::max(npt, (size_t)1)));
  HIP_TRY(c, c->p_d_segkeep.ensure(std::max(nsg, (size_t)1)));
  HIP_TRY(c, c->p_d_s32.ensure(nft * sizeof(float)));
  HIP_TRY(c, c->p_d_s64.ensure(nft * 5 * sizeof(double)));
  HIP_TRY(c, c->p_d_state.ensure((size_t)n * sizeof(PoseStateDev)));
  HIP_TRY(c, c->p_d_poses.ensure((size_t)n * 7 * sizeof(double)));
  if (c->p_trace_cap > 0) HIP_TRY(c, c->p_d_log.ensure((size_t)n * c->p_trace_cap * sizeof(plsvo_poseopt_iterlog)));
  PoseBatchDev& b = c->p_b;
  uint8_t* const base = c->p_d_blob.as<uint8_t>();
  b.jobs = reinterpret_cast<const PoseJobDev*>(base + o_jobs); b.state = c->p_d_state.as<PoseStateDev>();
  b.pt_f = reinterpret_cast<const double*>(base + o_f); b.pt_pos = reinterpret_cast<const double*>(base + o_pos);
  b.pt_level = reinterpret_cast<const int*>(base + o_plev);
  b.seg_line = reinterpret_cast<const double*>(base + o_line); b.seg_spos = reinterpret_cast<const double*>(base + o_spos);
  b.seg_epos = reinterpret_cast<const double*>(base + o_epos); b.seg_level = reinterpret_cast<const int*>(base + o_slev);
  b.pt_keep = c->p_d_ptkeep.as<uint8_t>(); b.seg_keep = c->p_d_segkeep.as<uint8_t>();
  b.scratch_f32 = c->p_d_s32.as<float>(); b.scratch_f64 = c->p_d_s64.as<double>();
  b.log = c->p_trace_cap > 0 ? c->p_d_log.as<plsvo_poseopt_iterlog>() : nullptr;
  b.log_cap = c->p_trace_cap; b.n_jobs = n;
  b.order = nullptr; b.work_key = nullptr;
  {
    long key_max = 1;
    for (int j = 0; j < n; ++j) key_max = std::max(key_max, (long)(jobs[j].n_pts + jobs[j].n_seg) * (long)(std::max(jobs[j].n_iter, 0) + std::max(jobs[j].n_iter_ref, 0)));
    c->p_key_shift = 0;
    while ((key_max >> c->p_key_shift) > 1023) ++c->p_key_shift;
  }
  c->p_jobs.swap(jobs);
  c->p_n = n; c->p_total_pt = (int)npt; c->p_total_seg = (int)nsg;
  c->p_staged = true; c->p_run_seq = 0;
  return PLSVO_OK;
}

extern "C" int plsvo_poseopt_run(plsvo_ctx* c) {
  CTX_CHECK(c);
  RoctxRange range("pose_optimizer");
  if (!c->p_staged) return fail(c, PLSVO_E_STATE, "poseopt_run: no staged batch");
  HIP_TRY(c, hipSetDevice(c->device));
  const int cus = c->cu_count > 0 ? c->cu_count : 256;
  const long feats = (long)c->p_total_pt + (long)c->p_total_seg;
  int threads = c->p_n <= 2 * cus ? 256 : (feats <= 580l * c->p_n ? 16 : 64);
  if (c->env_poseopt_threads) threads = c->env_poseopt_threads;
  const bool reorder = threads != 256 && !c->env_poseopt_no_reorder && !c->p_one_shot &&
                       c->p_n > (c->env_poseopt_reorder_min > 0 ? c->env_poseopt_reorder_min - 1 : (threads == 16 ? 4 : 8) * cus);
  c->p_b.work_key = nullptr;
  if (reorder) {
    if (c->p_d_workkey.cap < (size_t)c->p_n * sizeof(int)) {
      HIP_TRY(c, c->p_d_workkey.ensure((size_t)c->p_n * sizeof(int)));
      HIP_TRY(c, hipMemsetAsync(c->p_d_workkey.p, 0, c->p_d_workkey.cap, c->stream));
    }
    c->p_b.work_key = c->p_d_workkey.as<int>();
  } else c->p_b.order = nullptr;
  EventPair ep{}; prof_begin(c, PLSVO_K_POSEOPT, &ep);
  HIP_TRY(c, launch_pose_opt(c->p_b, c->p_d_poses.as<double>(), threads, c->stream));
  c->p_run_seq = ++c->run_seq;
  prof_end(c, PLSVO_K_POSEOPT, &ep);
  if (reorder) {
    DevBuf& ob = c->p_d_order[c->p_order_next];
    HIP_TRY(c, ob.ensure((size_t)c->p_n * sizeof(int)));
    HIP_TRY(c, launch_align_reorder(c->p_b.work_key, c->p_n, ob.as<int>(), c->p_key_shift, c->stream));
    c->p_b.order = ob.as<int>();
    c->p_order_next ^= 1;
  }
  return PLSVO_OK;
}

extern "C" int plsvo_poseopt_fetch(plsvo_ctx* c, int n, plsvo_poseopt_out* out) {
  CTX_CHECK(c);
  if (!c->p_staged) return fail(c, PLSVO_E_STATE, "poseopt_fetch: no staged batch");
  if (n != c->p_n || !out) return fail(c, PLSVO_E_INVALID, "poseopt_fetch: n does not match the staged batch");
  HIP_TRY(c, hipSetDevice(c->device));
  std::vector<uint8_t> big;
  const size_t rb[3] = { (size_t)n * sizeof(PoseStateDev), (size_t)std::max(c->p_total_pt, 0), (size_t)std::max(c->p_total_seg, 0) };
  const void* const rs[3] = { c->p_d_state.p, c->p_d_ptkeep.p, c->p_d_segkeep.p };
  const uint8_t* rh[3] = { nullptr, nullptr, nullptr };
  { const int rc_d = download_ranges(c, 3, rs, rb, big, rh); if (rc_d) return rc_d; }
  const PoseStateDev* const st = reinterpret_cast<const PoseStateDev*>(rh[0]);
  const uint8_t* const pk = rh[1]; const uint8_t* const sk = rh[2];
  for (int j = 0; j < n; ++j) {
    const PoseStateDev& s = st[(size_t)j];
    const PoseJobDev& J = c->p_jobs[(size_t)j];
    plsvo_poseopt_out& o = out[j];
    uint8_t* pko = o.pt_keep; uint8_t* sko = o.seg_keep;
    memset(&o, 0, sizeof(o));
    o.pt_keep = pko; o.seg_keep = sko;
    for (int k = 0; k < 7; ++k) o.T_f_w[k] = s.T[k];
    for (int k = 0; k < 36; ++k) o.cov[k] = s.cov[k];
    o.estimated_scale = s.estimated_scale; o.error_init = s.error_init; o.error_final = s.error_final;
    o.num_obs_pt = s.num_obs_pt; o.num_obs_ls = s.num_obs_ls;
    o.iters = s.iters; o.iters_ref = s.iters_ref; o.status = s.status;
    if (pko && J.n_pts > 0) memcpy(pko, pk + J.pt_off, (size_t)J.n_pts);
    if (sko && J.n_seg > 0) memcpy(sko, sk + J.seg_off, (size_t)J.n_seg);
  }
  return PLSVO_OK;
}

extern "C" int plsvo_pose_optimize_batch(plsvo_ctx* c, int n, const plsvo_poseopt_in* in, plsvo_poseopt_out* out) {
  int rc = plsvo_poseopt_stage(c, n, in); if (rc) return rc;
  c->p_one_shot = true;
  rc = plsvo_poseopt_run(c);
  c->p_one_shot = false;
  if (rc) return rc;
  return plsvo_poseopt_fetch(c, n, out);
}
// ... 633 lines not shown
```

pl-svo_amd/csrc/plsvo_dev.hpp:

```cpp
#pragma once
#include <stdint.h>

#include "../../include/plsvo_hip.h"

namespace plsvo_hip {

#if defined(__HIPCC__)
__host__ __device__
#endif
inline unsigned int pyr_level_offset(int width, int height, int level) {
  unsigned long long off = 0;
  for (int l = 0; l < level; ++l) off += (((unsigned long long)(width >> l) * (unsigned long long)(height >> l) + 64) + 255) & ~255ull;
  return (unsigned int)off;
}

#if defined(__HIPCC__)
__host__ __device__
#endif
inline unsigned int pyr_tiled_level_offset(int width, int height, int level) {
  unsigned long long off = 0;
  for (int l = 0; l < level; ++l) {
    const unsigned long long tiles = (unsigned long long)(((width >> l) + 15) >> 4) * (unsigned long long)(((height >> l) + 7) >> 3);
    off += (tiles * 128 + 255) & ~255ull;
  }
  return (unsigned int)off;
}
#if defined(__HIPCC__)
__device__ __forceinline__ int tiled_row_offset(int tiles_x, int y) { return (((y >> 3) * tiles_x) << 7) + ((y & 7) << 4); }
__device__ __forceinline__ int tiled_col_offset(int x) { return ((x >> 4) << 7) + (x & 15); }
#endif

constexpr int kQuadMinThreads = 256;

struct PyrDesc {
  const uint8_t* base;
  unsigned long long slot_bytes;
  const uint8_t* tbase;
  unsigned long long tslot_bytes;
  int n_slots, n_levels;
  int w[PLSVO_MAX_LEVELS], h[PLSVO_MAX_LEVELS];
  unsigned int off[PLSVO_MAX_LEVELS];
};

struct AlignJobDev {
  int ref_slot, cur_slot;
  double fx, fy, cx, cy;
  int width, height;
  int max_level, min_level, n_iter, skip;
  double eps;
  int pt_off, n_pts, seg_off, n_seg;
  int patch_off, patch_cap;
  int n_slots[PLSVO_MAX_LEVELS];
  int long_mask;
  int ldlt_flavour;
};

struct AlignStateDev {
  double T[7];
  double chi2;
  unsigned long long n_meas;
  double H[36];
  int stop;
  int log_count;
  int iters[PLSVO_MAX_LEVELS];
  unsigned long long patch_levels, patch_iters;
  unsigned long long patch_iters_pt;
  int error;
  int chi2_ties;
  int chi2_unarmed;
  int reserved2;
  unsigned long long phase_ticks[8];
};

struct AlignBatchDev {
  const AlignJobDev* jobs;
  AlignStateDev* state;
  const double* T0;
  const double* pt_px;
  const double* pt_xyz;
  const double* seg_spx;
  const double* seg_epx;
  const double* seg_len;
  const double* seg_p;
  const double* seg_q;
  const uint8_t* seg_alive_in;
  uint8_t* seg_alive;
  const int* seg_slot;
  int slot_level0, slot_stride;
  double* patch_xyz;
  float* patch_uvref;
  float* cache_ref;
  float* chi_terms;
  unsigned long long chi_plane;
  int chi_lds_pts;
  int reserved_lds;
  double* poses;
  PyrDesc pyr;
  plsvo_align_iterlog* log;
  int log_cap;
  int n_jobs;
  const int* order;
  int* work_key;
  int pair;
  unsigned int xseq0;
  unsigned long long* xbuf;
};

struct PoseJobDev {
  double T0[7];
  double fx, reproj_thresh;
  int n_iter, n_iter_ref;
  int pt_off, n_pts, seg_off, n_seg;
  int ldlt_flavour, reserved0;
};

struct PoseStateDev {
  double T[7];
  double cov[36];
  double estimated_scale, error_init, error_final;
  unsigned long long num_obs_pt, num_obs_ls;
  int iters, iters_ref, status, log_count;
  unsigned long long pt_iters, seg_iters;
  unsigned long long phase_ticks[8];
};

struct PoseBatchDev {
  const PoseJobDev* jobs;
  PoseStateDev* state;
  const double* pt_f;
  const double* pt_pos;
  const int* pt_level;
  const double* seg_line;
  const double* seg_spos;
  const double* seg_epos;
  const int* seg_level;
  uint8_t* pt_keep;
  uint8_t* seg_keep;
  float* scratch_f32;
  double* scratch_f64;
  plsvo_poseopt_iterlog* log;
  int log_cap;
  int n_jobs;
  const int* order;
  int* work_key;
};

struct StructBatchDev {
  const double* frame_T;
  const double* pt_pos; const int* pt_obs_off; const int* pt_obs_frame; const double* pt_obs_f;
  const double* seg_spos; const double* seg_epos; const int* seg_obs_off; const int* seg_obs_frame;
  const double* seg_obs_sf; const double* seg_obs_ef;
  double* pt_pos_out; double* seg_spos_out; double* seg_epos_out; int* pt_iters; int* seg_iters;
  int n_pts, n_seg, n_iter_pts, n_iter_segs;
};

struct MatchBatchDev {
  const uint8_t* pyr_base; unsigned long long slot_bytes;
  int width, height;
  double fx, fy, cx, cy; int cam_width, cam_height;
  int n, n_pyr_levels, align_max_iter;
  const double* frame_T; const int* frame_slot; const int* cur_frame; const int* ref_frame;
  const double* ref_px; const double* ref_f; const int* ref_level; const uint8_t* ref_type; const double* ref_grad;
  const double* pos; const double* px_cur;
  double* px_out; uint8_t* found; int* search_level; int* n_iter;
  const uint8_t* active;
};

struct SeedsBatchDev {
  const uint8_t* pyr_base; unsigned long long slot_bytes;
  int width, height;
  double fx, fy, cx, cy; int cam_width, cam_height;
  int n_pyr_levels, align_max_iter, max_epi_search_steps, edgelet_filtering;
  double edgelet_max_angle, px_error_angle, convergence_sigma2_thresh;
  int n_pt, n_seg;
  const double* frame_T; const int* frame_slot;
  const int* pt_ref_frame; const int* pt_cur_frame; const double* pt_px; const double* pt_f; const int* pt_level; const uint8_t* pt_type;
  const double* pt_grad; const float* pt_a; const float* pt_b; const float* pt_mu; const float* pt_z_range; const float* pt_sigma2;
  const int* seg_ref_frame; const int* seg_cur_frame; const double* seg_px; const double* seg_f; const double* seg_sf; const double* seg_ef;
  const int* seg_level; const float* seg_a; const float* seg_b; const float* seg_mu_s; const float* seg_mu_e; const float* seg_z_range_s;
  const float* seg_z_range_e; const float* seg_sigma2_s; const float* seg_sigma2_e;
  int* o_pt_status; float* o_pt_a; float* o_pt_b; float* o_pt_mu; float* o_pt_sigma2; double* o_pt_xyz; double* o_pt_px; double* o_pt_depth;
  int* o_seg_status; float* o_seg_a; float* o_seg_b; float* o_seg_mu_s; float* o_seg_mu_e; float* o_seg_sigma2_s; float* o_seg_sigma2_e;
  double* o_seg_xyz_s; double* o_seg_xyz_e; double* o_seg_depth_s; double* o_seg_depth_e;
};

struct ChainJobDev {
  double T_prev[7], T_kf[7];
  int kf_slot, cur_slot;
  int cand_off, n_pt, n_seg;
  int po_pt_off, po_seg_off;
  int reserved0;
};
struct ChainBatchDev {
  const ChainJobDev* jobs; int n_jobs, n_cand;
  const double* align_poses;
  double* frame_T; int* frame_slot;
  const int* cand_job; const double* pos; const uint8_t* active_in;
  const int* cell; uint8_t* active;
  const double* m_px; const uint8_t* found; const int* search_level;
  double fx, fy, cx, cy;
  int n_cells, cell_rule, max_fts; const int* cell_order;
  const double* proj_px;
  int seg_cell_size, seg_n_cols, seg_n_cells, max_fts_segs; const int* seg_cell_order;
  PoseJobDev* po_jobs; double* pt_f; double* pt_pos; int* pt_level; double* seg_line; double* seg_spos; double* seg_epos; int* seg_level;
  int* sel_pt; int* sel_seg; int* n_sel;
  double reproj_thresh; int po_n_iter, ldlt_flavour;
};

struct ReprojBatchDev {
  double fx, fy, cx, cy; int cam_width, cam_height;
  int n, cell_size, grid_n_cols, boundary;
  const double* frame_T; const int* frame; const double* pos;
  double* px; int* cell;
};

constexpr int kDetTileW = 64, kDetTileH = 32;
constexpr int kDetImgX0 = 8, kDetImgY0 = 5;
constexpr int kDetImgW = kDetTileW + 16, kDetImgH = kDetTileH + 10;
constexpr int kDetScoreW = 68, kDetScoreH = kDetTileH + 2;
constexpr int kDetCellCap = 128;
constexpr int kDetThreads = 256;

struct DetectLaunch {
  const uint8_t* pyr;
  unsigned long long slot_bytes;
  int n_lv;
  int level[PLSVO_MAX_LEVELS], w[PLSVO_MAX_LEVELS], h[PLSVO_MAX_LEVELS], tiles_x[PLSVO_MAX_LEVELS];
  unsigned int off[PLSVO_MAX_LEVELS];
  int tile_begin[PLSVO_MAX_LEVELS + 1];
  int fast_b;
  float thr;
  int cell, cols, n_cells;
  const uint8_t* occupancy;
  unsigned long long* keys;
  uint8_t* stage_score;
  uint8_t* stage_survives;
};

inline int detect_tiles(int w, int h, int* tiles_x) {
  *tiles_x = (w + kDetTileW - 1) / kDetTileW;
  return *tiles_x * ((h + kDetTileH - 1) / kDetTileH);
}


}
```

pl-svo_amd/csrc/plsvo_wave.hpp:

```cpp
#pragma once
#include <hip/hip_runtime.h>

#include "plsvo_math.hpp"

namespace plsvo_hip {

template <int CTRL>
__device__ __forceinline__ double dpp_mov_f64(double v) {
  int lo = __double2loint(v), hi = __double2hiint(v);
  lo = __builtin_amdgcn_update_dpp(0, lo, CTRL, 0xf, 0xf, true);
  hi = __builtin_amdgcn_update_dpp(0, hi, CTRL, 0xf, 0xf, true);
  return __hiloint2double(hi, lo);
}
template <int CTRL>
__device__ __forceinline__ float dpp_mov_f32(float v) {
  return __int_as_float(__builtin_amdgcn_update_dpp(0, __float_as_int(v), CTRL, 0xf, 0xf, true));
}
template <int CTRL, int ROW_MASK>
__device__ __forceinline__ double dpp_bcast_f64(double v) {
  int lo = __double2loint(v), hi = __double2hiint(v);
  lo = __builtin_amdgcn_update_dpp(0, lo, CTRL, ROW_MASK, 0xf, false);
  hi = __builtin_amdgcn_update_dpp(0, hi, CTRL, ROW_MASK, 0xf, false);
  return __hiloint2double(hi, lo);
}
// ... 112 lines not shown

__device__ __forceinline__ void wave_solve6_core(double m, double* x, int flavour = 320, bool allow_static_order = true);

__device__ __forceinline__ void wave_solve6(const double* tot, double* x) {
  const int lane = threadIdx.x & 63;
  const int i = lane >> 3, j = lane & 7;
  double m = 0.0;
  if (i < 6 && j < 6) m = tot[sym6_index(i, j)];
  else if (i < 6 && j == 6) m = tot[21 + i];
  wave_solve6_core(m, x);
}

__device__ __forceinline__ void wave_solve6_reg(double tot_lane, double* x, int flavour = 320, bool allow_static_order = true) {
  const int lane = threadIdx.x & 63;
  const int i = lane >> 3, j = lane & 7;
  const int src = (i < 6 && j < 6) ? sym6_index(i, j) : ((i < 6 && j == 6) ? 21 + i : 0);
  double m = __shfl(tot_lane, src, 64);
  if (!(i < 6 && j <= 6)) m = 0.0;
  wave_solve6_core(m, x, flavour, allow_static_order);
}

__device__ __forceinline__ double bpermute_f64(int byte_addr, double v) {
  const int lo = __builtin_amdgcn_ds_bpermute(byte_addr, __double2loint(v));
  const int hi = __builtin_amdgcn_ds_bpermute(byte_addr, __double2hiint(v));
  return __hiloint2double(hi, lo);
}
__device__ __forceinline__ double wave_max_to_lane63(double v) {
  v = fmax(v, dpp_mov_f64<DPP_QUAD_XOR1>(v));
  v = fmax(v, dpp_mov_f64<DPP_QUAD_XOR2>(v));
  v = fmax(v, dpp_mov_f64<DPP_ROW_HALF_MIRROR>(v));
  v = fmax(v, dpp_mov_f64<DPP_ROW_MIRROR>(v));
  v = fmax(v, dpp_bcast_f64<DPP_ROW_BCAST15, 0xA>(v));
  v = fmax(v, dpp_bcast_f64<DPP_ROW_BCAST31, 0xC>(v));
  return v;
}

__device__ __forceinline__ void wave_solve6_core(double m, double* x, int flavour, bool allow_static_order) {
  const int lane = threadIdx.x & 63;
  const int i = lane >> 3, j = lane & 7;
  const int addr_row = 4 * j, addr_col = 4 * 8 * i;
  bool diag_active = (i == j) && (i < 6);
  const bool in_system = (i < 6) && (j <= 6);
  const double key0 = fabs(m);
  unsigned zero_piv = 0u;
  double cutoff = 0.0;
  int last_p = 0;
  const bool in66 = (i < 6) && (j < 6);
  const double k_i = bpermute_f64(4 * 9 * (i < 6 ? i : 0), key0), k_j = bpermute_f64(4 * 9 * (j < 6 ? j : 0), key0);
  const unsigned long long larger = __ballot(in66 && k_j > k_i);
  const unsigned long long odd = __ballot(in66 && ((i != j && k_j == k_i) || k_i != k_i));
  if (allow_static_order && odd == 0ull) {
    int ord[6] = { 0, 0, 0, 0, 0, 0 };
#pragma unroll
    for (int a = 0; a < 6; ++a) {
      const int rank = __popcll(larger & (0x3full << (8 * a)));
#pragma unroll
      for (int s_ = 0; s_ < 6; ++s_) if (rank == s_) ord[s_] = a;
    }
    const double kmax0 = readlane_f64(key0, 9 * ord[0]);
    cutoff = flavour == 330 ? 0.0 : fabs(2.220446049250313e-16 * kmax0);
#pragma unroll
    for (int step = 0; step < 6; ++step) {
      const int p = ord[step];
      const double kmax = readlane_f64(key0, 9 * p);
      const double piv = readlane_f64(m, 9 * p);
      if (!(kmax < cutoff) && fabs(piv) > cutoff) {
        const double mp_j = bpermute_f64(addr_row + 32 * p, m);
        const double mi_p = bpermute_f64(addr_col + 4 * p, m);
        const double rinv = fast_rcp(piv);
        if (in_system && i != p) m = fma(-(mi_p * mp_j), rinv, m);
      } else {
        zero_piv |= 1u << p;
      }
      last_p = p;
    }
  } else {
  int pos = diag_active ? i : 64;
#pragma unroll
  for (int step = 0; step < 6; ++step) {
    const double key = diag_active ? key0 : -1.0;
    const double kmax = readlane_f64(wave_max_to_lane63(key), 63);
    unsigned long long cand = __ballot(diag_active && key == kmax);
    if (cand == 0ull) cand = __ballot(diag_active);
    int plane = __builtin_ctzll(cand);
    if (cand & (cand - 1ull)) {
      int best = 64;
      for (unsigned long long c = cand; c; c &= c - 1ull) {
        const int l = __builtin_ctzll(c);
        const int ps = __builtin_amdgcn_readlane(pos, l);
        if (ps < best) { best = ps; plane = l; }
      }
    }
    const int p = (plane * 57) >> 9;
    const double piv = readlane_f64(m, plane);
    const int pos_p = __builtin_amdgcn_readlane(pos, plane);
    if (pos == step) pos = pos_p;
    if (step == 0) cutoff = flavour == 330 ? 0.0 : fabs(2.220446049250313e-16 * kmax);
    if (!(kmax < cutoff) && fabs(piv) > cutoff) {
      const double mp_j = bpermute_f64(addr_row + 32 * p, m);
      const double mi_p = bpermute_f64(addr_col + 4 * p, m);
      const double rinv = fast_rcp(piv);
      if (in_system && i != p) m = fma(-(mi_p * mp_j), rinv, m);
    } else {
      zero_piv |= 1u << p;
    }
    diag_active = diag_active && (i != p);
    last_p = p;
  }
  }
  const double dgi = bpermute_f64(addr_col + 4 * i, m);
  const double tolerance = 1.0 / 1.7976931348623157e308;
  double xi = (((zero_piv >> i) & 1u) || !(fabs(dgi) > tolerance)) ? ((dgi != dgi || m != m) ? (m + dgi) : 0.0) : m / dgi;
  if (cutoff > 1.7976931348623157e308) xi = (i == last_p || fabs(dgi) <= 1.7976931348623157e308) ? 0.0 : __builtin_nan("");
#pragma unroll
  for (int r = 0; r < 6; ++r) x[r] = readlane_f64(xi, 8 * r + 6);
}

__device__ __forceinline__ void granule_store(unsigned long long* p, unsigned long long v) {
#ifdef PLSVO_WAVE_EMU
  __atomic_store_n(p, v, __ATOMIC_RELEASE);
#else
  __hip_atomic_store(p, v, __ATOMIC_RELAXED, __HIP_MEMORY_SCOPE_AGENT);
#endif
}
__device__ __forceinline__ unsigned long long granule_load(const unsigned long long* p) {
#ifdef PLSVO_WAVE_EMU
  return __atomic_load_n(p, __ATOMIC_ACQUIRE);
#else
  return __hip_atomic_load(p, __ATOMIC_RELAXED, __HIP_MEMORY_SCOPE_AGENT);
#endif
}
constexpr unsigned kPairPollMax = 1u << 20;
__device__ __forceinline__ double pair_allgather32(unsigned long long* xb, int rank, unsigned seq, double mine, bool& lost) {
  const int lane = threadIdx.x & 63;
  const double v = __shfl(mine, lane >> 1, 64);
  const unsigned half = (lane & 1) ? (unsigned)__double2hiint(v) : (unsigned)__double2loint(v);
  unsigned long long* const own = xb + (((seq & 1u) * 2u + (unsigned)rank) * 64u + (unsigned)lane);
  const unsigned long long* const peer = xb + (((seq & 1u) * 2u + (unsigned)(rank ^ 1)) * 64u + (unsigned)lane);
  granule_store(own, ((unsigned long long)seq << 32) | (unsigned long long)half);
  unsigned long long g;
  for (unsigned polls = 0;; ++polls) {
    g = granule_load(peer);
    if (!__any((unsigned)(g >> 32) != seq)) break;
    if (polls >= kPairPollMax || lost) { lost = true; break; }
#ifdef PLSVO_WAVE_EMU
    wave_emu_yield_thread();
#else
    __builtin_amdgcn_s_sleep(2);
#endif
  }
  const int k = lane & 31;
  const unsigned lo = (unsigned)__shfl((int)(unsigned)g, 2 * k, 64), hi = (unsigned)__shfl((int)(unsigned)g, 2 * k + 1, 64);
  return __hiloint2double((int)hi, (int)lo);
}

__device__ __forceinline__ Quat quat_normalized_fast(const Quat& a) {
  const double inv = fast_rcp(fast_sqrt(a.x * a.x + a.y * a.y + a.z * a.z + a.w * a.w));
  Quat r = { a.x * inv, a.y * inv, a.z * inv, a.w * inv };
  return r;
}

__device__ __forceinline__ SE3d se3_exp_dev(const double* u) {
  SE3d r;
  const double ox = u[3], oy = u[4], oz = u[5];
  const double z = ox * ox + oy * oy + oz * oz;
  double real_factor, imag_factor, a, b;
  if (z <= 0.01) {
    real_factor = 1.0 / 3715891200.0;
    real_factor = fma(real_factor, -z, 1.0 / 10321920.0);
    real_factor = fma(real_factor, -z, 1.0 / 46080.0);
    real_factor = fma(real_factor, -z, 1.0 / 384.0);
    real_factor = fma(real_factor, -z, 1.0 / 8.0);
    real_factor = fma(real_factor, -z, 1.0);
    imag_factor = 1.0 / 81749606400.0;
    imag_factor = fma(imag_factor, -z, 1.0 / 185794560.0);
    imag_factor = fma(imag_factor, -z, 1.0 / 645120.0);
    imag_factor = fma(imag_factor, -z, 1.0 / 3840.0);
    imag_factor = fma(imag_factor, -z, 1.0 / 48.0);
    imag_factor = fma(imag_factor, -z, 0.5);
    a = 1.0 / 479001600.0;
    a = fma(a, -z, 1.0 / 3628800.0);
    a = fma(a, -z, 1.0 / 40320.0);
    a = fma(a, -z, 1.0 / 720.0);
    a = fma(a, -z, 1.0 / 24.0);
    a = fma(a, -z, 0.5);
    b = 1.0 / 6227020800.0;
    b = fma(b, -z, 1.0 / 39916800.0);
    b = fma(b, -z, 1.0 / 362880.0);
    b = fma(b, -z, 1.0 / 5040.0);
    b = fma(b, -z, 1.0 / 120.0);
    b = fma(b, -z, 1.0 / 6.0);
  } else {
    const double theta = sqrt(z);
    real_factor = cos(0.5 * theta);
    imag_factor = sin(0.5 * theta) / theta;
    a = (1 - cos(theta)) / z;
    b = (theta - sin(theta)) / (z * theta);
  }
  Quat q = { imag_factor * ox, imag_factor * oy, imag_factor * oz, real_factor };
  r.q = quat_normalized_fast(q);
  const double O2_00 = -(oy * oy + oz * oz), O2_11 = -(ox * ox + oz * oz), O2_22 = -(ox * ox + oy * oy);
  const double O2_01 = ox * oy, O2_02 = ox * oz, O2_12 = oy * oz;
  double V[9];
  V[0] = 1.0 + b * O2_00;      V[1] = a * -oz + b * O2_01;  V[2] = a * oy + b * O2_02;
  V[3] = a * oz + b * O2_01;   V[4] = 1.0 + b * O2_11;      V[5] = a * -ox + b * O2_12;
  V[6] = a * -oy + b * O2_02;  V[7] = a * ox + b * O2_12;   V[8] = 1.0 + b * O2_22;
  for (int i = 0; i < 3; ++i) r.t[i] = V[i * 3 + 0] * u[0] + V[i * 3 + 1] * u[1] + V[i * 3 + 2] * u[2];
  return r;
}

__device__ __forceinline__ SE3d se3_mul_dev(const SE3d& A, const SE3d& B) {
  SE3d r; double rt[3];
  quat_rotate(A.q, B.t, rt);
  r.t[0] = A.t[0] + rt[0]; r.t[1] = A.t[1] + rt[1]; r.t[2] = A.t[2] + rt[2];
  r.q = quat_normalized_fast(quat_mul(A.q, B.q));
  return r;
}


}
```

Before: 2.215 million.

## Split the last-starting alignment frames into coarse and fine workgroups with device hand-off

After: 2.259 million (median of 6 runs). +2.0%, better.

```diff
diff --git a/include/plsvo_hip.h b/include/plsvo_hip.h
--- a/include/plsvo_hip.h
+++ b/include/plsvo_hip.h
@@ -36,6 +36,7 @@
 #define PLSVO_OPT_POSEOPT_THREADS 3
 #define PLSVO_OPT_ALIGN_REORDER 4
 #define PLSVO_OPT_POSEOPT_REORDER 5
+#define PLSVO_OPT_ALIGN_TAIL_SPLIT 6
 int plsvo_hip_set_option(plsvo_ctx* ctx, int option, int value);
 const char* plsvo_hip_last_error(const plsvo_ctx* ctx);
 void* plsvo_hip_stream(plsvo_ctx* ctx);
@@ -149,6 +150,7 @@
 
 int plsvo_align_work(plsvo_ctx* ctx, uint64_t* patch_levels, uint64_t* patch_iters);
 int plsvo_align_launch_order(plsvo_ctx* ctx, int n, int32_t* order);
+int plsvo_align_tail_frames(plsvo_ctx* ctx, int* tail_frames);
 int plsvo_align_work_points(plsvo_ctx* ctx, uint64_t* point_patch_iters);
 
 int plsvo_align_chi2_ties(plsvo_ctx* ctx, uint64_t* iterations, uint64_t* ties, uint64_t* near_ties_without_terms);
diff --git a/pl-svo_amd/capi.py b/pl-svo_amd/capi.py
--- a/pl-svo_amd/capi.py
+++ b/pl-svo_amd/capi.py
@@ -16,7 +16,7 @@
     "plsvo_rectify_map", "plsvo_hip_config_rectify", "plsvo_hip_rectify_build_pyramid", "plsvo_hip_rectify_build_pyramids_dev",
     "plsvo_detect_grid", "plsvo_detect_cell", "plsvo_hip_detect_fast", "plsvo_hip_detect_fast_dev", "plsvo_hip_detect_stages",
     "plsvo_sparse_align", "plsvo_sparse_align_batch", "plsvo_align_stage", "plsvo_align_run", "plsvo_align_fetch",
-    "plsvo_align_set_trace", "plsvo_align_fetch_trace", "plsvo_align_poses_dev", "plsvo_align_copy_poses", "plsvo_align_work", "plsvo_align_work_points", "plsvo_align_chi2_ties", "plsvo_align_launch_order",
+    "plsvo_align_set_trace", "plsvo_align_fetch_trace", "plsvo_align_poses_dev", "plsvo_align_copy_poses", "plsvo_align_work", "plsvo_align_work_points", "plsvo_align_chi2_ties", "plsvo_align_launch_order", "plsvo_align_tail_frames",
     "plsvo_pose_optimize", "plsvo_pose_optimize_batch", "plsvo_poseopt_stage", "plsvo_poseopt_run", "plsvo_poseopt_fetch",
     "plsvo_poseopt_set_trace", "plsvo_poseopt_fetch_trace", "plsvo_poseopt_poses_dev", "plsvo_poseopt_copy_poses", "plsvo_poseopt_work",
     "plsvo_structure_optimize", "plsvo_match_direct", "plsvo_reproject", "plsvo_trajectory_record", "plsvo_update_seeds",
@@ -110,6 +110,7 @@
         "plsvo_align_chi2_ties": (C.c_int, [ctxp, C.POINTER(C.c_uint64), C.POINTER(C.c_uint64), C.POINTER(C.c_uint64)]),
         "plsvo_align_work_points": (C.c_int, [ctxp, C.POINTER(C.c_uint64)]),
         "plsvo_align_launch_order": (C.c_int, [ctxp, C.c_int, C.POINTER(C.c_int32)]),
+        "plsvo_align_tail_frames": (C.c_int, [ctxp, C.POINTER(C.c_int)]),
         "plsvo_pose_optimize": (C.c_int, [ctxp, C.POINTER(abi.PoseOptIn), C.POINTER(abi.PoseOptOut)]),
         "plsvo_pose_optimize_batch": (C.c_int, [ctxp, C.c_int, C.POINTER(abi.PoseOptIn), C.POINTER(abi.PoseOptOut)]),
         "plsvo_poseopt_stage": (C.c_int, [ctxp, C.c_int, C.POINTER(abi.PoseOptIn)]),
@@ -180,6 +181,9 @@
         if poseopt is not None:
             self._chk(self.L.plsvo_hip_set_option(self.h, 5, 1 if poseopt else 0))
 
+    def set_align_tail_split(self, on):
+        self._chk(self.L.plsvo_hip_set_option(self.h, 6, 1 if on else 0))
+
     def close(self):
         if getattr(self, "h", None):
             self.L.plsvo_hip_destroy(self.h)
@@ -349,6 +353,11 @@
         out = np.zeros(n, dtype=np.int32)
         self._chk(self.L.plsvo_align_launch_order(self.h, n, out.ctypes.data_as(C.POINTER(C.c_int32))))
         return out
+
+    def align_tail_frames(self):
+        n = C.c_int(0)
+        self._chk(self.L.plsvo_align_tail_frames(self.h, C.byref(n)))
+        return n.value
 
     def align_chi2_ties(self):
         a = C.c_uint64(0)
diff --git a/pl-svo_amd/csrc/align_kernels.hip b/pl-svo_amd/csrc/align_kernels.hip
--- a/pl-svo_amd/csrc/align_kernels.hip
+++ b/pl-svo_amd/csrc/align_kernels.hip
@@ -1,5 +1,6 @@
 #include <hip/hip_runtime.h>
 
+#include <cstddef>
 #include <type_traits>
 
 #include "plsvo_dev.hpp"
@@ -227,7 +228,13 @@
 __global__ __launch_bounds__(T, kMinWavesPerSimd) void align_fused_kernel(AlignBatchDev b, int cap, int scap, int level_hi, int level_lo, int do_init) {
   const bool pair = T >= kQuadMinThreads && b.pair != 0;
   const int rank = pair ? (int)((blockIdx.x >> 3) & 1u) : 0;
-  const int wg_index = pair ? (int)((blockIdx.x >> 4) * 8u + (blockIdx.x & 7u)) : (int)blockIdx.x;
+  int wg_index = pair ? (int)((blockIdx.x >> 4) * 8u + (blockIdx.x & 7u)) : (int)blockIdx.x;
+  constexpr bool kTail = T == 64;
+  int part = 0;
+  if (kTail && b.tail_n > 0) {
+    if (wg_index < b.tail_n) { part = 1; wg_index += b.n_jobs - b.tail_n; }
+    else { if (wg_index >= b.n_jobs) part = 2; wg_index -= b.tail_n; }
+  }
   if (wg_index >= b.n_jobs) return;
   const bool lead = rank == 0;
   const bool own_pts = !pair || rank == 0, own_segs = !pair || rank == 1;
@@ -257,18 +264,36 @@
   __shared__ unsigned long long s_tlast;
   if (tid == 0) { for (int k = 0; k < 8; ++k) s_time[k] = 0; s_tlast = __builtin_amdgcn_s_memtime(); }
 #endif
-  const int lv_first = min(job.max_level, level_hi), lv_last = max(job.min_level, level_lo);
+  int lv_first = min(job.max_level, level_hi), lv_last = max(job.min_level, level_lo);
   const bool nothing = job.skip || lv_first < lv_last;
+  if (part == 1) lv_last += 1;
+  else if (part == 2) lv_first = lv_last;
+  if (part == 2) do_init = 0;
+  unsigned* const tail_flag = kTail && part ? b.tail_flag + (wg_index - (b.n_jobs - b.tail_n)) : nullptr;
+  if (part == 2 && !nothing) {
+    if (!tail_wait(tail_flag)) { if (tid == 0) st->error = 2; return; }
+    if (handoff_load_i32(&st->error)) return;
+    if (lane < 8) {
+      const double v = handoff_load_f64(&st->T[lane]);
+      if (lane < 7) { s_pose[12 + lane] = v; s_pose[19 + lane] = v; } else s_pose[26] = v;
+    }
+    if (lane == 8) s_ctl[1] = handoff_load_i32(&st->stop);
+  }
   if (do_init && own_segs) {
     for (int s = tid; s < job.n_seg; s += T)
-      b.seg_alive[job.seg_off + s] = b.seg_alive_in ? (b.seg_alive_in[job.seg_off + s] != 0) : 1;
-  }
+      ((kTail && part == 1) ? b.seg_alive_tail : b.seg_alive)[job.seg_off + s] = b.seg_alive_in ? (b.seg_alive_in[job.seg_off + s] != 0) : 1;
+  }
+  if (kTail && tid == 0) {
+    s_ctl[11] = part; s_ctl[12] = wg_index - (b.n_jobs - b.tail_n);
+    for (int k = 0; k < PLSVO_MAX_LEVELS; ++k) s_ctl[16 + k] = 0;
+  }
+  auto seg_flags = [&]() -> uint8_t* { return (kTail && s_ctl[11] == 1) ? b.seg_alive_tail : b.seg_alive; };
   if (tid == 0) {
     double T_in[7], chi_in = 1e10; int stop_in = 0;
     if (do_init) {
 #pragma unroll
       for (int k = 0; k < 7; ++k) T_in[k] = b.T0[7 * job_id + k];
-      if (lead) {
+      if (lead && !(kTail && part == 1 && !nothing)) {
 #pragma unroll
       for (int k = 0; k < 7; ++k) st->T[k] = T_in[k];
       st->chi2 = 1e10; st->n_meas = 0; st->stop = 0; st->log_count = 0; st->error = 0;
@@ -279,21 +304,24 @@
       if (nothing && b.poses) for (int k = 0; k < 7; ++k) b.poses[7 * job_id + k] = T_in[k];
       if (nothing && b.work_key) b.work_key[job_id] = 0;
       }
-    } else if (!nothing) {
+    } else if (!nothing && part != 2) {
 #pragma unroll
       for (int k = 0; k < 7; ++k) T_in[k] = st->T[k];
       chi_in = st->chi2; stop_in = st->stop;
     }
     if (!nothing) {
+      if (part != 2) {
 #pragma unroll
       for (int k = 0; k < 7; ++k) { s_pose[12 + k] = T_in[k]; s_pose[19 + k] = T_in[k]; }
-      s_pose[26] = chi_in; s_pose[28] = 0.0; s_pose[29] = 0.0; s_pose[31] = 0.0;
+      s_pose[26] = chi_in; s_ctl[1] = stop_in;
+      }
+      s_pose[28] = 0.0; s_pose[29] = 0.0; s_pose[31] = 0.0;
       for (int k = 0; k < 32; ++k) s_tot[k] = 0.0;
-      s_ctl[1] = stop_in; s_ctl[3] = 0; s_ctl[6] = 0; s_ctl[9] = 0;
+      s_ctl[3] = 0; s_ctl[6] = 0; s_ctl[9] = 0;
       s_ctl[10] = 0;
     }
   }
-  if (nothing) return;
+  if (nothing) { if (kTail && part == 1) tail_publish(tail_flag); return; }
   block_sync<T>();
   if (b.chi_lds_pts > 0) {
     const int tail0 = job.n_pts * 16, tail1 = ((job.n_pts + 3) & ~3) * 16;
@@ -321,6 +349,7 @@
     for (int l = 0; l < PLSVO_MAX_LEVELS; ++l) if (l == level) { n_slots = job.n_slots[l]; long_lines = ((job.long_mask >> l) & 1) != 0; }
     if (n_slots > cap || n_slots > job.patch_cap) {
       if (tid == 0 && lead) { st->error = 1; if (b.work_key) b.work_key[job_id] = 0; }
+      if (kTail && s_ctl[11] == 1) { if (tid == 0) handoff_store(&st->error, 1); tail_publish(b.tail_flag + s_ctl[12]); }
       return;
     }
     const int slot_lo = (pair && rank == 1) ? min(line0, n_slots) : 0, slot_hi = (pair && rank == 0) ? min(line0, n_slots) : n_slots;
@@ -364,7 +393,7 @@
           for (int c = 0; c < 3; ++c) { g_p[c] = b.seg_p[3 * s + c]; g_q[c] = b.seg_q[3 * s + c]; }
         }
         const int code = b.seg_slot[(size_t)(level - b.slot_level0) * b.slot_stride + s];
-        if (code >= 0 && b.seg_alive[s]) {
+        if (code >= 0 && seg_flags()[s]) {
           const int p0 = code & 0xfffff, N = code >> 20;
           const double sx = kQuad ? g_s[0] : b.seg_spx[2 * s], sy = kQuad ? g_s[1] : b.seg_spx[2 * s + 1];
           double inc2x = ((kQuad ? g_e[0] : b.seg_epx[2 * s]) - sx) * scale / (double)(N - 1);
@@ -548,7 +577,7 @@
                 }
               } else if (p == first) {
                 s_dead[-1 - meta.x] = iter + 1;
-                b.seg_alive[job.seg_off + (-1 - meta.x)] = 0;
+                seg_flags()[job.seg_off + (-1 - meta.x)] = 0;
               }
             }
           }
@@ -826,7 +855,7 @@
                 }
               } else if (p == first) {
                 s_dead[-1 - meta.x] = iter + 1;
-                b.seg_alive[job.seg_off + (-1 - meta.x)] = 0;
+                seg_flags()[job.seg_off + (-1 - meta.x)] = 0;
               }
             }
           }
@@ -987,25 +1016,61 @@
     }
 
     if (tid == 0) {
-      if (lead) st->iters[level] = s_ctl[2];
+      if (kTail && s_ctl[11] == 1) s_ctl[16 + level] = s_ctl[2];
+      else if (lead) st->iters[level] = s_ctl[2];
       s_pose[28] += pair ? s_tot[31] : (double)s_ctl[5];
       s_pose[29] += s_pose[27];
+      for (int k = 0; k < 7; ++k) s_pose[19 + k] = s_pose[12 + k];
     }
   }
 
   block_sync<T>();
+  const int part_end = kTail ? s_ctl[11] : 0;
+  if (part_end == 1) {
+    constexpr int kWords = (int)(sizeof(AlignStateDev) / sizeof(unsigned long long));
+    static_assert(sizeof(AlignStateDev) % sizeof(unsigned long long) == 0 && kWords <= 64 && sizeof(AlignStateDev) <= ROWS * 32 * sizeof(double), "one word per lane, in s_red");
+    unsigned long long* const img = reinterpret_cast<unsigned long long*>(s_red);
+    if (tid < kWords) img[tid] = 0ull;
+    block_sync<T>();
+    if (tid == 0) {
+      AlignStateDev* const im = reinterpret_cast<AlignStateDev*>(s_red);
+      for (int k = 0; k < 7; ++k) im->T[k] = s_pose[12 + k];
+      im->chi2 = s_pose[26]; im->stop = s_ctl[1]; im->error = s_ctl[3];
+      for (int k = 0; k < PLSVO_MAX_LEVELS; ++k) im->iters[k] = s_ctl[16 + k];
+      im->patch_levels = (unsigned long long)(s_pose[28] + 0.5); im->patch_iters = (unsigned long long)(s_pose[29] + 0.5);
+      im->patch_iters_pt = (unsigned long long)(s_pose[31] + 0.5);
+      im->chi2_ties = s_ctl[6]; im->chi2_unarmed = s_ctl[9];
+#ifdef PLSVO_TIMING
+      for (int k = 0; k < 8; ++k) im->phase_ticks[k] = s_time[k];
+#endif
+      if (b.work_key) handoff_store(&b.work_key[job_id], (int)fmin(s_pose[29] + 0.5, 2147483647.0));
+    }
+    block_sync<T>();
+    if (tid < kWords) handoff_store(reinterpret_cast<unsigned long long*>(st) + tid, img[tid]);
+    for (int sg = tid; sg < job.n_seg; sg += T) handoff_store(&b.seg_alive[job.seg_off + sg], b.seg_alive_tail[job.seg_off + sg]);
+    tail_publish(b.tail_flag + s_ctl[12]);
+    return;
+  }
   if (tid == 0 && lead) {
     for (int k = 0; k < 7; ++k) st->T[k] = s_pose[12 + k];
     if (b.poses) for (int k = 0; k < 7; ++k) b.poses[7 * job_id + k] = s_pose[12 + k];
     st->chi2 = s_pose[26];
-    st->patch_levels += (unsigned long long)(s_pose[28] + 0.5);
-    st->patch_iters += (unsigned long long)(s_pose[29] + 0.5);
-    if (b.work_key) b.work_key[job_id] = (int)fmin(s_pose[29] + 0.5, 2147483647.0);
-    st->patch_iters_pt += (unsigned long long)(s_pose[31] + 0.5);
+    unsigned long long w_lv = 0, w_it = 0, w_pt = 0; int w_ties = 0, w_unarmed = 0; double w_key = 0.0;
+    if (part_end == 2) {
+      w_lv = handoff_load_u64(&st->patch_levels); w_it = handoff_load_u64(&st->patch_iters); w_pt = handoff_load_u64(&st->patch_iters_pt);
+      w_ties = handoff_load_i32(&st->chi2_ties); w_unarmed = handoff_load_i32(&st->chi2_unarmed);
+      if (b.work_key) w_key = (double)handoff_load_i32(&b.work_key[job_id]);
+    } else {
+      w_lv = st->patch_levels; w_it = st->patch_iters; w_pt = st->patch_iters_pt; w_ties = st->chi2_ties; w_unarmed = st->chi2_unarmed;
+    }
+    st->patch_levels = w_lv + (unsigned long long)(s_pose[28] + 0.5);
+    st->patch_iters = w_it + (unsigned long long)(s_pose[29] + 0.5);
+    if (b.work_key) b.work_key[job_id] = (int)fmin(w_key + s_pose[29] + 0.5, 2147483647.0);
+    st->patch_iters_pt = w_pt + (unsigned long long)(s_pose[31] + 0.5);
     st->stop = s_ctl[1];
     if (s_ctl[3]) st->error = s_ctl[3];
-    st->chi2_ties += s_ctl[6];
-    st->chi2_unarmed += s_ctl[9];
+    st->chi2_ties = w_ties + s_ctl[6];
+    st->chi2_unarmed = w_unarmed + s_ctl[9];
     st->n_meas = (unsigned long long)(s_tot[28] + 0.5);
     for (int i = 0; i < 6; ++i) for (int jj = 0; jj < 6; ++jj) st->H[i * 6 + jj] = s_tot[sym6_index(i, jj)];
 #ifdef PLSVO_TIMING
@@ -1018,6 +1083,9 @@
 size_t align_level_lds_bytes(int threads, int cap, int scap, int chi_lds_pts) { return align_lds_used(threads, cap, scap, chi_lds_pts); }
 
 }
+#ifdef PLSVO_WAVE_EMU
+extern "C" void plsvo_emu_set_tail_flag_value(unsigned v) { plsvo_hip::wave_emu_tail_flag_value() = v; }
+#endif
 extern "C" const char* plsvo_hip_build_flags(void) { return ""; }
 namespace plsvo_hip {
 
@@ -1025,7 +1093,7 @@
 static hipError_t launch_fused_T(const AlignBatchDev& b, int cap, int scap, int level_hi, int level_lo, int do_init, size_t lds, hipStream_t stream) {
   hipError_t e = hipFuncSetAttribute(reinterpret_cast<const void*>(align_fused_kernel<T>), hipFuncAttributeMaxDynamicSharedMemorySize, (int)lds);
   if (e != hipSuccess) return e;
-  const unsigned grid = (T >= kQuadMinThreads && b.pair) ? (unsigned)((b.n_jobs + 7) / 8) * 16u : (unsigned)b.n_jobs;
+  const unsigned grid = (T >= kQuadMinThreads && b.pair) ? (unsigned)((b.n_jobs + 7) / 8) * 16u : (unsigned)(b.n_jobs + (T == 64 ? b.tail_n : 0));
 #ifdef PLSVO_WAVE_EMU
   wave_emu::pair_stride() = (T >= kQuadMinThreads && b.pair) ? 8 : 0;
 #endif
diff --git a/pl-svo_amd/csrc/plsvo_capi.hip b/pl-svo_amd/csrc/plsvo_capi.hip
--- a/pl-svo_amd/csrc/plsvo_capi.hip
+++ b/pl-svo_amd/csrc/plsvo_capi.hip
@@ -116,6 +116,10 @@
   const int* a_stage_order = nullptr;
   bool a_one_shot = false, p_one_shot = false;
   int env_align_reorder_min = 0;
+  bool opt_align_tail_split = true;
+  int env_align_tail_min = 0, env_align_tail_k = 0, env_align_tail_frames = 0;
+  DevBuf a_d_tailflag;
+  DevBuf a_d_alive_tail;
   DevBuf a_d_xbuf;
   unsigned int x_launch = 0;
   bool env_align_no_pair = false;
@@ -250,6 +254,10 @@
   c->env_align_no_pair = env_flag("PLSVO_ALIGN_NO_PAIR");
   c->env_align_no_reorder = env_flag("PLSVO_ALIGN_NO_REORDER");
   if (const char* s = getenv("PLSVO_ALIGN_REORDER_MIN")) c->env_align_reorder_min = atoi(s);
+  if (const char* s = getenv("PLSVO_ALIGN_TAIL_SPLIT")) c->opt_align_tail_split = atoi(s) != 0;
+  if (const char* s = getenv("PLSVO_ALIGN_TAIL_MIN")) c->env_align_tail_min = atoi(s);
+  if (const char* s = getenv("PLSVO_ALIGN_TAIL_K")) c->env_align_tail_k = atoi(s);
+  if (const char* s = getenv("PLSVO_ALIGN_TAIL_FRAMES")) c->env_align_tail_frames = atoi(s);
   c->env_poseopt_no_reorder = env_flag("PLSVO_POSEOPT_NO_REORDER");
   if (const char* s = getenv("PLSVO_POSEOPT_REORDER_MIN")) c->env_poseopt_reorder_min = atoi(s);
   c->env_host_timing = getenv("PLSVO_HOST_TIMING") != nullptr;
@@ -263,7 +271,7 @@
   (void)hipStreamSynchronize(c->stream);
   prof_collect(c);
   for (auto& ep : c->ev_pool) { (void)hipEventDestroy(ep.a); (void)hipEventDestroy(ep.b); }
-  c->a_d_xbuf.release(); c->a_d_order[0].release(); c->a_d_order[1].release(); c->a_d_workkey.release(); c->p_d_workkey.release(); c->p_d_order[0].release(); c->p_d_order[1].release();
+  c->a_d_tailflag.release(); c->a_d_alive_tail.release(); c->a_d_xbuf.release(); c->a_d_order[0].release(); c->a_d_order[1].release(); c->a_d_workkey.release(); c->p_d_workkey.release(); c->p_d_order[0].release(); c->p_d_order[1].release();
   DevBuf* bufs[] = { &c->pyr_slab, &c->pyr_tiled, &c->pyr_upload, &c->a_d_blob, &c->a_d_state, &c->a_d_alive, &c->a_d_pxyz, &c->a_d_puv, &c->a_d_cref,
                      &c->a_d_chi, &c->a_d_log, &c->a_d_poses, &c->p_d_blob, &c->p_d_state, &c->p_d_ptkeep, &c->p_d_segkeep, &c->p_d_s32, &c->p_d_s64,
                      &c->p_d_log, &c->p_d_poses, &c->s_d_in, &c->s_d_out, &c->ch_d_blob, &c->ch_d_work, &c->ch_d_po, &c->ch_d_state,
@@ -304,6 +312,11 @@
     } else {
       c->env_poseopt_no_reorder = value == 0;
     }
+    return PLSVO_OK;
+  }
+  if (option == PLSVO_OPT_ALIGN_TAIL_SPLIT) {
+    if (value != 0 && value != 1) return fail(c, PLSVO_E_INVALID, "set_option: the alignment's tail split is 0 (one workgroup per frame throughout) or 1 (the frames that start last run as a coarse and a fine part)");
+    c->opt_align_tail_split = value != 0;
     return PLSVO_OK;
   }
   return fail(c, PLSVO_E_INVALID, "set_option: unknown option");
@@ -1002,7 +1015,7 @@
   b.log = c->a_trace_cap > 0 ? c->a_d_log.as<plsvo_align_iterlog>() : nullptr;
   b.log_cap = c->a_trace_cap;
   b.n_jobs = n;
-  b.pair = 0; b.xseq0 = 0; b.xbuf = nullptr; b.work_key = nullptr;
+  b.pair = 0; b.xseq0 = 0; b.xbuf = nullptr; b.work_key = nullptr; b.tail_n = 0; b.reserved_tail = 0; b.tail_flag = nullptr; b.seg_alive_tail = nullptr;
   b.order = reinterpret_cast<const int*>(base + o_order);
   c->a_stage_order = b.order;
   c->a_jobs.swap(jobs);
@@ -1049,6 +1062,7 @@
 };
 }
 
+constexpr int kAlignTailRounds = 2;
 extern "C" int plsvo_align_run(plsvo_ctx* c) {
   CTX_CHECK(c);
   RoctxRange range("sparse_img_align");
@@ -1105,6 +1119,20 @@
       HIP_TRY(c, hipMemsetAsync(c->a_d_workkey.p, 0, c->a_d_workkey.cap, c->stream));
     }
     c->a_b.work_key = c->a_d_workkey.as<int>();
+  }
+  c->a_b.tail_n = 0; c->a_b.tail_flag = nullptr; c->a_b.seg_alive_tail = nullptr;
+  if (c->opt_align_tail_split && threads == 64 && have_levels && c->a_gmax > c->a_gmin && !pair && !per_level && c->a_trace_cap == 0) {
+    const int resident = cus_run * 512 / threads;
+    const int min_n = c->env_align_tail_min > 0 ? c->env_align_tail_min : 4 * resident;
+    const int want = c->env_align_tail_frames > 0 ? c->env_align_tail_frames : (c->env_align_tail_k > 0 ? c->env_align_tail_k : kAlignTailRounds) * resident;
+    if (c->a_n >= min_n) {
+      const int tail_n = std::min(c->a_n, want);
+      const size_t fbytes = (((size_t)tail_n * sizeof(unsigned int)) + 15) & ~(size_t)15;
+      HIP_TRY(c, c->a_d_tailflag.ensure(fbytes));
+      HIP_TRY(c, hipMemsetAsync(c->a_d_tailflag.p, 0, fbytes, c->stream));
+      HIP_TRY(c, c->a_d_alive_tail.ensure((size_t)std::max(c->a_total_seg, 1)));
+      c->a_b.tail_n = tail_n; c->a_b.tail_flag = c->a_d_tailflag.as<unsigned int>(); c->a_b.seg_alive_tail = c->a_d_alive_tail.as<uint8_t>();
+    }
   }
   if (!per_level || !have_levels) {
     EventPair ep{}; prof_begin(c, PLSVO_K_ALIGN_LEVEL, &ep);
@@ -1157,6 +1185,7 @@
       memcpy(alive_out, alive + c->a_jobs[(size_t)j].seg_off, (size_t)c->a_jobs[(size_t)j].n_seg);
     if (s.error) dev_err = s.error;
   }
+  if (dev_err == 2) return fail(c, PLSVO_E_HIP, "align: a workgroup timed out waiting for the workgroup it shares a frame with (device-side hand-off, code 2)");
   if (dev_err) return fail(c, PLSVO_E_CAPACITY, "align: device-side capacity check failed (code " + std::to_string(dev_err) + ")");
   return PLSVO_OK;
 }
@@ -1276,6 +1305,14 @@
   if (!c->a_b.order) { for (int j = 0; j < n; ++j) order[j] = j; return PLSVO_OK; }
   HIP_TRY(c, hipMemcpyAsync(order, c->a_b.order, (size_t)n * sizeof(int32_t), hipMemcpyDeviceToHost, c->stream));
   HIP_TRY(c, hipStreamSynchronize(c->stream));
+  return PLSVO_OK;
+}
+
+extern "C" int plsvo_align_tail_frames(plsvo_ctx* c, int* tail_frames) {
+  CTX_CHECK(c);
+  if (!c->a_staged) return fail(c, PLSVO_E_STATE, "align_tail_frames: no staged batch");
+  if (!tail_frames) return fail(c, PLSVO_E_INVALID, "align_tail_frames: NULL output");
+  *tail_frames = c->a_b.tail_n;
   return PLSVO_OK;
 }
 
diff --git a/pl-svo_amd/csrc/plsvo_dev.hpp b/pl-svo_amd/csrc/plsvo_dev.hpp
--- a/pl-svo_amd/csrc/plsvo_dev.hpp
+++ b/pl-svo_amd/csrc/plsvo_dev.hpp
@@ -104,6 +104,10 @@
   int pair;
   unsigned int xseq0;
   unsigned long long* xbuf;
+  int tail_n;
+  int reserved_tail;
+  unsigned int* tail_flag;
+  uint8_t* seg_alive_tail;
 };
 
 struct PoseJobDev {
diff --git a/pl-svo_amd/csrc/plsvo_wave.hpp b/pl-svo_amd/csrc/plsvo_wave.hpp
--- a/pl-svo_amd/csrc/plsvo_wave.hpp
+++ b/pl-svo_amd/csrc/plsvo_wave.hpp
@@ -288,6 +288,60 @@
   const int k = lane & 31;
   const unsigned lo = (unsigned)__shfl((int)(unsigned)g, 2 * k, 64), hi = (unsigned)__shfl((int)(unsigned)g, 2 * k + 1, 64);
   return __hiloint2double((int)hi, (int)lo);
+}
+
+#ifdef PLSVO_WAVE_EMU
+constexpr unsigned kTailPollMax = 1u << 10;
+inline unsigned& wave_emu_tail_flag_value() { static unsigned v = 1u; return v; }
+#else
+constexpr unsigned kTailPollMax = kPairPollMax;
+#endif
+__device__ __forceinline__ unsigned long long handoff_load_u64(const void* p) {
+#ifdef PLSVO_WAVE_EMU
+  return __atomic_load_n(reinterpret_cast<const unsigned long long*>(p), __ATOMIC_ACQUIRE);
+#else
+  return __hip_atomic_load(reinterpret_cast<const unsigned long long*>(p), __ATOMIC_RELAXED, __HIP_MEMORY_SCOPE_AGENT);
+#endif
+}
+__device__ __forceinline__ double handoff_load_f64(const double* p) { return __longlong_as_double((long long)handoff_load_u64(p)); }
+__device__ __forceinline__ int handoff_load_i32(const void* p) {
+#ifdef PLSVO_WAVE_EMU
+  return __atomic_load_n(reinterpret_cast<const int*>(p), __ATOMIC_ACQUIRE);
+#else
+  return __hip_atomic_load(reinterpret_cast<const int*>(p), __ATOMIC_RELAXED, __HIP_MEMORY_SCOPE_AGENT);
+#endif
+}
+template <typename V>
+__device__ __forceinline__ void handoff_store(V* p, V v) {
+#ifdef PLSVO_WAVE_EMU
+  __atomic_store_n(p, v, __ATOMIC_RELEASE);
+#else
+  __hip_atomic_store(p, v, __ATOMIC_RELAXED, __HIP_MEMORY_SCOPE_AGENT);
+#endif
+}
+__device__ __forceinline__ void handoff_store_f64(double* p, double v) { handoff_store(reinterpret_cast<unsigned long long*>(p), (unsigned long long)__double_as_longlong(v)); }
+__device__ __forceinline__ void tail_publish(unsigned* flag) {
+#ifdef PLSVO_WAVE_EMU
+  if ((threadIdx.x & 63) == 0) __atomic_store_n(flag, wave_emu_tail_flag_value(), __ATOMIC_RELEASE);
+#else
+  asm volatile("s_waitcnt vmcnt(0)" ::: "memory");
+  if ((threadIdx.x & 63) == 0) __hip_atomic_store(flag, 1u, __ATOMIC_RELAXED, __HIP_MEMORY_SCOPE_AGENT);
+#endif
+}
+__device__ __forceinline__ bool tail_wait(const unsigned* flag) {
+  for (unsigned polls = 0;; ++polls) {
+    if ((unsigned)handoff_load_i32(flag) == 1u) break;
+    if (polls >= kTailPollMax) return false;
+#ifdef PLSVO_WAVE_EMU
+    wave_emu_yield_thread();
+#else
+    __builtin_amdgcn_s_sleep(8);
+#endif
+  }
+#ifndef PLSVO_WAVE_EMU
+  __builtin_amdgcn_fence(__ATOMIC_ACQUIRE, "agent");
+#endif
+  return true;
 }
 
 __device__ __forceinline__ Quat quat_normalized_fast(const Quat& a) {
```
